# KerkDovan/univer-ocr

Measured on AMD Instinct MI355X. Metric: document-images/sec (fwd+bwd) on 256x512 synthetic pages, higher is better.
Workload: dtype f32; 1 GPU; BASELINE configs[2]: my_model train step (fwd+loss+bwd+L2+SGD) of Monochrome+Paragraph+Line on (32,256,512,1) pages and Char on (32,32,64,1) line strips per GPU; batch_per_gpu=32, global_batch=32, optimizer=sgd, parallelism=dp1, h2d_inclusive=False, input_grads=True, hip_graphs=True, pipelined_lanes=True, hw_queues=4

## Files before the change

### include/univer_hip.h

```cpp
#ifndef UNIVER_HIP_H
#define UNIVER_HIP_H

#include <stddef.h>
#include <stdint.h>

#ifdef __cplusplus
extern "C" {
#endif

#define UOCR_ABI_VERSION 4

typedef struct uocr_ctx uocr_ctx;

enum { UOCR_F32 = 0, UOCR_F64 = 1, UOCR_F16 = 2 };
#define UOCR_F16_SCALED(k) (UOCR_F16 | ((k) << 8))
#define UOCR_DTYPE_BASE(dtype) ((dtype) & 0xff)
#define UOCR_DTYPE_GRAD_SCALE_LOG2(dtype) (((dtype) >> 8) & 0xff)
enum { UOCR_ACT_NONE = 0, UOCR_ACT_RELU = 1, UOCR_ACT_LEAKY = 2, UOCR_ACT_SIGMOID = 3 };
enum { UOCR_LOSS_DICE = 0, UOCR_LOSS_JACCARD = 1 };
enum {
    UOCR_OK = 0,
    UOCR_ERR_ARG = -1,
    UOCR_ERR_DTYPE = -2,
    UOCR_ERR_HIP = -3,
    UOCR_ERR_WORKSPACE = -4,
    UOCR_ERR_UNSUPPORTED = -5,
    UOCR_ERR_RCCL = -6
};

int uocr_abi_version(void);
int uocr_ctx_create(int device, size_t workspace_bytes, uocr_ctx** out);
int uocr_ctx_create_cu_mask(int device, size_t workspace_bytes, const uint32_t* cu_mask, int mask_words, uocr_ctx** out);
int uocr_ctx_destroy(uocr_ctx* ctx);
int uocr_ctx_set_stream(uocr_ctx* ctx, void* hip_stream);
void* uocr_ctx_get_stream(uocr_ctx* ctx);
int uocr_ctx_set_option(uocr_ctx* ctx, const char* key, int value);
int uocr_ctx_last_split(uocr_ctx* ctx, int* blocks, long long* items);
int uocr_ctx_last_gemm(uocr_ctx* ctx, int* bm, int* gm, int* gn, int* nsplit);
int uocr_ctx_last_gemm_group(uocr_ctx* ctx, int* problems, int* split_problems);
int uocr_ctx_last_pair(uocr_ctx* ctx, int* kernel, int* g, int* mode, int* pf, int* nw, int* blocks_x, int* bands,
                       int* band_h);
enum {
    UOCR_CONV_NONE = 0,
    UOCR_CONV_GENERIC = 1,
    UOCR_CONV_MFMA = 2,
    UOCR_CONV_H16 = 3,
    UOCR_CONV_H16_WGRAD = 4,
    UOCR_CONV_H16_WGRAD_S2 = 5,
    UOCR_CONV_T32 = 6,
    UOCR_CONV_T32_WGRAD = 7,
    UOCR_CONV_H3 = 8,
    UOCR_CONV_TILED = 9,
    UOCR_CONV_C16_EXPAND = 10,
    UOCR_CONV_C16_REDUCE = 11,
    UOCR_CONV_C16_WGRAD = 12,
    UOCR_CONV_DGRAD_S2 = 13,
    UOCR_CONV_DGRAD_C64S2 = 14,
    UOCR_CONV_WGRAD_T542 = 15,
    UOCR_CONV_WGRAD_S2_TILED = 16,
    UOCR_CONV_TABLE_FAST = 17,
    UOCR_CONV_TABLE_PX = 18
};
int uocr_ctx_last_conv(uocr_ctx* ctx, int* entry, int* kernel);
int uocr_ctx_reserve_workspace(uocr_ctx* ctx, size_t bytes);
const char* uocr_last_error(uocr_ctx* ctx);
int uocr_malloc(uocr_ctx* ctx, size_t bytes, void** out);
int uocr_free(uocr_ctx* ctx, void* ptr);
int uocr_memset_zero(uocr_ctx* ctx, void* ptr, size_t bytes);
int uocr_h2d(uocr_ctx* ctx, void* dst, const void* src_host, size_t bytes);
int uocr_d2h_sync(uocr_ctx* ctx, void* dst_host, const void* src, size_t bytes);
int uocr_d2d(uocr_ctx* ctx, void* dst, const void* src, size_t bytes);
int uocr_stream_sync(uocr_ctx* ctx);
int uocr_event_create(void** out_event);
int uocr_event_destroy(void* event);
int uocr_event_record(uocr_ctx* ctx, void* event);
int uocr_stream_wait_event(uocr_ctx* ctx, void* event);
int uocr_event_elapsed_ms_sync(void* start, void* stop, float* out_ms);
int uocr_event_synchronize(void* event);
int uocr_graph_begin_capture(uocr_ctx* ctx);
int uocr_graph_end_capture(uocr_ctx* ctx, void** out_graph_exec);
int uocr_graph_launch(uocr_ctx* ctx, void* graph_exec);
int uocr_graph_destroy(void* graph_exec);
int uocr_ctx_set_loss_snapshot(uocr_ctx* ctx, const double* slots, int count, double* ring, int ring_len,
                               unsigned* counter);
int uocr_wgrad_defer_begin(uocr_ctx* ctx);
int uocr_wgrad_defer_flush(uocr_ctx* ctx, int keep_open);
int uocr_device_info(uocr_ctx* ctx, char* name_out, size_t name_cap, int* cu_count, size_t* hbm_bytes);

int uocr_conv2d_fwd(uocr_ctx* ctx, int dtype, const void* x, const void* w, const void* b, void* y,
                    int n, int h, int wd, int cin, int cout, int kh, int kw, int sh, int sw,
                    int ph, int pw, int oh, int ow, double pad_value, int use_bias,
                    int act, double act_alpha);
int uocr_conv2d_bwd_data(uocr_ctx* ctx, int dtype, const void* dy, const void* w, void* dx,
                         int n, int h, int wd, int cin, int cout, int kh, int kw, int sh, int sw,
                         int ph, int pw, int oh, int ow,
                         const void* x_act, int act, double act_alpha);
int uocr_conv2d_bwd_weight(uocr_ctx* ctx, int dtype, const void* x, const void* dy, void* dw, void* db,
                           int n, int h, int wd, int cin, int cout, int kh, int kw, int sh, int sw,
                           int ph, int pw, int oh, int ow, double pad_value, int use_bias,
                           int accumulate);

int uocr_conv_pair_fwd(uocr_ctx* ctx, int dtype, const void* x, const void* w1, const void* b1,
                       const void* w2, const void* b2, void* y, int n, int h, int wd, int cmid,
                       double pad_value1, int use_bias1, int use_bias2, double alpha1, int act2);
int uocr_conv_pair_bwd(uocr_ctx* ctx, int dtype, const void* x, const void* y, const void* dy,
                       const void* w1, const void* b1, const void* w2, void* dw1, void* db1, void* dw2,
                       void* db2, void* dx, int n, int h, int wd, int cmid, double pad_value1,
                       int use_bias1, int use_bias2, double alpha1, int act2, int accumulate);

int uocr_upconv2x_fwd(uocr_ctx* ctx, int dtype, const void* x_low, const void* w, const void* b, void* y,
                      int n, int hl, int wl, int cin, int cout, int kh, int kw, int ph, int pw,
                      int use_bias, int act, double act_alpha, void* weff);
int uocr_upconv2x_bwd_data(uocr_ctx* ctx, int dtype, const void* dy, const void* w, void* dx_low,
                           int n, int hl, int wl, int cin, int cout, int kh, int kw, int ph, int pw,
                           const void* x_act, int act, double act_alpha, const void* weff);
int uocr_upconv2x_bwd_weight(uocr_ctx* ctx, int dtype, const void* x_low, const void* dy, void* dw, void* db,
                             int n, int hl, int wl, int cin, int cout, int kh, int kw, int ph, int pw,
                             int use_bias, int accumulate);

int uocr_maxpool2d_fwd(uocr_ctx* ctx, int dtype, const void* x, void* y, uint8_t* mask,
                       int n, int h, int wd, int c, int kh, int kw, int sh, int sw, int ph, int pw,
                       int oh, int ow);
int uocr_maxpool2d_bwd(uocr_ctx* ctx, int dtype, const void* dy, const uint8_t* mask, void* dx,
                       int n, int h, int wd, int c, int kh, int kw, int sh, int sw, int ph, int pw,
                       int oh, int ow);

int uocr_upsample2d_fwd(uocr_ctx* ctx, int dtype, const void* x, void* y,
                        int n, int h, int wd, int c, int sy, int sx);
int uocr_upsample2d_bwd(uocr_ctx* ctx, int dtype, const void* dy, void* dx,
                        int n, int h, int wd, int c, int sy, int sx);

int uocr_act_fwd(uocr_ctx* ctx, int dtype, int kind, double alpha, const void* x, void* y, size_t count);
int uocr_act_bwd(uocr_ctx* ctx, int dtype, int kind, double alpha, const void* x, const void* dy,
                 void* dx, size_t count);

int uocr_act_bwd_from_output(uocr_ctx* ctx, int dtype, int kind, double alpha, const void* y, const void* dy,
                             void* dx, size_t count);

int uocr_dense_fwd(uocr_ctx* ctx, int dtype, const void* x, const void* w, void* y,
                   int m, int n_in, int n_out);
int uocr_dense_bwd(uocr_ctx* ctx, int dtype, const void* x, const void* w, const void* dy,
                   void* dx, void* dw, int m, int n_in, int n_out, int accumulate);
int uocr_dense_fwd_act(uocr_ctx* ctx, int dtype, const void* x, const void* w, void* y,
                       int m, int n_in, int n_out, int act, double act_alpha);
int uocr_dense_bwd_act(uocr_ctx* ctx, int dtype, const void* x, const void* w, const void* dy,
                       void* dx, void* dw, int m, int n_in, int n_out, int accumulate,
// ... 118 lines not shown
```

### univer-ocr_amd/csrc/conv_api.hip

```cpp
#include "conv_dims.h"

namespace {

int check_dims(uocr_ctx* ctx, const ConvDims& d) {
    UOCR_REQUIRE(ctx, d.n > 0 && d.h > 0 && d.w > 0 && d.cin > 0 && d.cout > 0);
    UOCR_REQUIRE(ctx, d.kh > 0 && d.kw > 0 && d.sh > 0 && d.sw > 0 && d.ph >= 0 && d.pw >= 0);
    UOCR_REQUIRE(ctx, d.oh > 0 && d.ow > 0);
    UOCR_REQUIRE(ctx, (d.oh - 1) * d.sh + d.kh <= d.h + 2 * d.ph);
    UOCR_REQUIRE(ctx, (d.ow - 1) * d.sw + d.kw <= d.w + 2 * d.pw);
    return UOCR_OK;
}

constexpr ConvRow<ConvFwd> FWD_ROWS[] = {
    {UOCR_CONV_H16, uocr_conv_h16_takes, uocr_conv_h16_run},
    {UOCR_CONV_T32, uocr_conv_t32_takes, uocr_conv_t32_run},
    {UOCR_CONV_H3, uocr_conv_h3_takes, uocr_conv_h3_run},
    {UOCR_CONV_TILED, uocr_conv_tiled_takes, uocr_conv_tiled_run},
    {CONV_NOT_NOTED, uocr_conv_fast_takes, uocr_conv_fast_run},
    {UOCR_CONV_MFMA, uocr_conv_mfma_takes, uocr_conv_mfma_run},
    {UOCR_CONV_GENERIC, uocr_conv_any_takes, uocr_conv_generic_run},
};
constexpr ConvRow<ConvDgrad> DGRAD_ROWS[] = {
    {UOCR_CONV_H16, uocr_conv_h16_takes, uocr_conv_h16_run},
    {UOCR_CONV_T32, uocr_conv_t32_takes, uocr_conv_t32_run},
    {CONV_NOT_NOTED, uocr_conv_fast_takes, uocr_conv_fast_run},
    {UOCR_CONV_MFMA, uocr_conv_mfma_takes, uocr_conv_mfma_run},
    {UOCR_CONV_GENERIC, uocr_conv_any_takes, uocr_conv_generic_run},
};
constexpr ConvRow<ConvWgrad> WGRAD_ROWS[] = {
    {UOCR_CONV_H16_WGRAD, uocr_conv_h16_takes, uocr_conv_h16_run},
    {UOCR_CONV_T32_WGRAD, uocr_conv_t32_takes, uocr_conv_t32_run},
    {UOCR_CONV_H16_WGRAD_S2, uocr_conv_h16_s2_takes, uocr_conv_h16_s2_run},
    {CONV_NOT_NOTED, uocr_conv_fast_takes, uocr_conv_fast_run},
    {UOCR_CONV_MFMA, uocr_conv_mfma_takes, uocr_conv_mfma_run},
    {UOCR_CONV_GENERIC, uocr_conv_any_takes, uocr_conv_generic_run},
};

}

extern "C" {

int uocr_conv2d_fwd(uocr_ctx* ctx, int dtype, const void* x, const void* w, const void* b, void* y, int n, int h,
                    int wd, int cin, int cout, int kh, int kw, int sh, int sw, int ph, int pw, int oh, int ow,
                    double pad_value, int use_bias, int act, double act_alpha) {
    UOCR_CHECK_CTX(ctx);
    const ConvDims d{n, h, wd, cin, cout, kh, kw, sh, sw, ph, pw, oh, ow};
    int rc = check_dims(ctx, d);
    if (rc) return rc;
    UOCR_REQUIRE(ctx, x && w && y && (b || !use_bias));
    UOCR_REQUIRE(ctx, act >= UOCR_ACT_NONE && act <= UOCR_ACT_SIGMOID);
    return uocr_conv_dispatch(ctx, 0, FWD_ROWS, ConvFwd{dtype, d, x, w, b, y, pad_value, use_bias, act, act_alpha});
}

int uocr_conv2d_bwd_data(uocr_ctx* ctx, int dtype, const void* dy, const void* w, void* dx, int n, int h, int wd,
                         int cin, int cout, int kh, int kw, int sh, int sw, int ph, int pw, int oh, int ow,
                         const void* x_act, int act, double act_alpha) {
    UOCR_CHECK_CTX(ctx);
    const ConvDims d{n, h, wd, cin, cout, kh, kw, sh, sw, ph, pw, oh, ow};
    int rc = check_dims(ctx, d);
    if (rc) return rc;
    UOCR_REQUIRE(ctx, dy && w && dx);
    UOCR_REQUIRE(ctx, act == UOCR_ACT_NONE || (x_act && (act == UOCR_ACT_SIGMOID || (act == UOCR_ACT_LEAKY && act_alpha > 0))));
    const ActMask mask{act == UOCR_ACT_NONE ? nullptr : x_act, act, act_alpha};
    return uocr_conv_dispatch(ctx, 1, DGRAD_ROWS, ConvDgrad{dtype, d, dy, w, dx, mask});
}

int uocr_conv2d_bwd_weight(uocr_ctx* ctx, int dtype, const void* x, const void* dy, void* dw, void* db, int n, int h,
                           int wd, int cin, int cout, int kh, int kw, int sh, int sw, int ph, int pw, int oh, int ow,
                           double pad_value, int use_bias, int accumulate) {
    UOCR_CHECK_CTX(ctx);
    const ConvDims d{n, h, wd, cin, cout, kh, kw, sh, sw, ph, pw, oh, ow};
    int rc = check_dims(ctx, d);
    if (rc) return rc;
    UOCR_REQUIRE(ctx, x && dy && dw && db);
    return uocr_conv_dispatch(ctx, 2, WGRAD_ROWS, ConvWgrad{dtype, d, x, dy, dw, db, pad_value, use_bias, accumulate});
}

}
```

### univer-ocr_amd/csrc/conv_dims.h

```cpp
#pragma once
#include "uocr_common.h"

struct ConvDims { int n, h, w, cin, cout, kh, kw, sh, sw, ph, pw, oh, ow; };

inline bool conv_is5x5_pad2(const ConvDims& d, int stride) {
    return d.kh == 5 && d.kw == 5 && d.sh == stride && d.sw == stride && d.ph == 2 && d.pw == 2 &&
           d.oh == (d.h + stride - 1) / stride && d.ow == (d.w + stride - 1) / stride;
}

struct ActMask { const void* y; int act; double alpha; };

struct ConvFwd { int dtype; ConvDims d; const void *x, *w, *b; void* y; double pad_value; int use_bias, act; double act_alpha; };
struct ConvDgrad { int dtype; ConvDims d; const void *dy, *w; void* dx; ActMask mask; };
struct ConvWgrad { int dtype; ConvDims d; const void *x, *dy; void *dw, *db; double pad_value; int use_bias, accumulate; };

template <class Call>
struct ConvRow { int kernel; bool (*takes)(uocr_ctx*, const Call&); int (*run)(uocr_ctx*, const Call&); };
constexpr int CONV_NOT_NOTED = UOCR_CONV_NONE;
template <class Call> bool uocr_conv_any_takes(uocr_ctx*, const Call&) { return true; }

template <class Call, size_t N>
int uocr_conv_dispatch(uocr_ctx* ctx, int entry, const ConvRow<Call> (&rows)[N], const Call& c) {
    for (const ConvRow<Call>& r : rows)
        if (r.takes(ctx, c))
            return r.kernel == CONV_NOT_NOTED ? r.run(ctx, c) : uocr_noted_conv(ctx, entry, r.kernel, r.run(ctx, c));
    UOCR_FAIL(ctx, UOCR_ERR_UNSUPPORTED, "no conv kernel takes this call");
}

bool uocr_conv_mfma_takes(uocr_ctx*, const ConvFwd&);       int uocr_conv_mfma_run(uocr_ctx*, const ConvFwd&);
bool uocr_conv_mfma_takes(uocr_ctx*, const ConvDgrad&);     int uocr_conv_mfma_run(uocr_ctx*, const ConvDgrad&);
bool uocr_conv_mfma_takes(uocr_ctx*, const ConvWgrad&);     int uocr_conv_mfma_run(uocr_ctx*, const ConvWgrad&);
bool uocr_conv_h16_takes(uocr_ctx*, const ConvFwd&);        int uocr_conv_h16_run(uocr_ctx*, const ConvFwd&);
bool uocr_conv_h16_takes(uocr_ctx*, const ConvDgrad&);      int uocr_conv_h16_run(uocr_ctx*, const ConvDgrad&);
bool uocr_conv_h16_takes(uocr_ctx*, const ConvWgrad&);      int uocr_conv_h16_run(uocr_ctx*, const ConvWgrad&);
bool uocr_conv_h16_s2_takes(uocr_ctx*, const ConvWgrad&);   int uocr_conv_h16_s2_run(uocr_ctx*, const ConvWgrad&);
bool uocr_upconv_h16_takes(uocr_ctx*, const ConvFwd&);      int uocr_upconv_h16_run(uocr_ctx*, const ConvFwd&);
bool uocr_upconv_h16_takes(uocr_ctx*, const ConvDgrad&);    int uocr_upconv_h16_run(uocr_ctx*, const ConvDgrad&);
bool uocr_upconv_wgrad_h16_takes(uocr_ctx*, const ConvWgrad&);
int uocr_upconv_wgrad_h16(uocr_ctx* ctx, const ConvWgrad& c, float* partial, size_t partial_floats, int* nblocks);
bool uocr_conv_t32_takes(uocr_ctx*, const ConvFwd&);        int uocr_conv_t32_run(uocr_ctx*, const ConvFwd&);
bool uocr_conv_t32_takes(uocr_ctx*, const ConvDgrad&);      int uocr_conv_t32_run(uocr_ctx*, const ConvDgrad&);
bool uocr_conv_t32_takes(uocr_ctx*, const ConvWgrad&);      int uocr_conv_t32_run(uocr_ctx*, const ConvWgrad&);
bool uocr_upconv_t32_takes(uocr_ctx*, const ConvDgrad&);    int uocr_upconv_t32_run(uocr_ctx*, const ConvDgrad&);
bool uocr_conv_h3_takes(uocr_ctx*, const ConvFwd&);         int uocr_conv_h3_run(uocr_ctx*, const ConvFwd&);
bool uocr_conv_tiled_takes(uocr_ctx*, const ConvFwd&);      int uocr_conv_tiled_run(uocr_ctx*, const ConvFwd&);
bool uocr_conv_fast_takes(uocr_ctx*, const ConvFwd&);       int uocr_conv_fast_run(uocr_ctx*, const ConvFwd&);
bool uocr_conv_fast_takes(uocr_ctx*, const ConvDgrad&);     int uocr_conv_fast_run(uocr_ctx*, const ConvDgrad&);
bool uocr_conv_fast_takes(uocr_ctx*, const ConvWgrad&);     int uocr_conv_fast_run(uocr_ctx*, const ConvWgrad&);
int uocr_conv_generic_run(uocr_ctx*, const ConvFwd&);       int uocr_conv_generic_run(uocr_ctx*, const ConvDgrad&);
int uocr_conv_generic_run(uocr_ctx*, const ConvWgrad&);
```

### univer-ocr_amd/csrc/conv_fast.hip

```cpp
#include "finish_group.h"
#include "conv_dims.h"

namespace {

template <int C, typename TA>
__device__ __forceinline__ void load_vec(const TA* __restrict__ p, float (&v)[C]) {
    if constexpr (C == 1) {
        v[0] = ld1(p);
    } else if constexpr (C == 2) {
        const float2 t = ld2(p);
        v[0] = t.x;
        v[1] = t.y;
    } else {
        static_assert(C % 4 == 0, "channel count must be 1, 2 or a multiple of 4");
#pragma unroll
        for (int q = 0; q < C / 4; ++q) {
            const float4 t = ld4(p + 4 * q);
            v[4 * q] = t.x;
            v[4 * q + 1] = t.y;
            v[4 * q + 2] = t.z;
            v[4 * q + 3] = t.w;
        }
    }
}

template <int C, typename TA>
__device__ __forceinline__ void store_vec(TA* __restrict__ p, const float (&v)[C]) {
    if constexpr (C == 1) {
        st1(p, v[0]);
    } else if constexpr (C == 2) {
        st2(p, make_float2(v[0], v[1]));
    } else {
#pragma unroll
        for (int q = 0; q < C / 4; ++q) st4(p + 4 * q, make_float4(v[4 * q], v[4 * q + 1], v[4 * q + 2], v[4 * q + 3]));
    }
}

struct FastDims {
    int n, h, w, oh, ow, ph, pw;
};

inline bool is_c16_same(const ConvDims& d, int cin, int cout) {
    return d.kh == 3 && d.kw == 3 && d.cin == cin && d.cout == cout && d.sh == 1 && d.sw == 1 && d.oh == d.h &&
           d.ow == d.w;
}
inline bool is_5x5_s2_pad2(const ConvDims& d) {
    return d.kh == 5 && d.kw == 5 && d.sh == 2 && d.sw == 2 && d.ph == 2 && d.pw == 2;
}
inline bool is_5x5_s1_pad2(const ConvDims& d) {
    return d.kh == 5 && d.kw == 5 && d.sh == 1 && d.sw == 1 && d.ph == 2 && d.pw == 2;
}

template <int C, typename TA>
__device__ __forceinline__ void apply_mask(float (&v)[C], const TA* __restrict__ mask_y, size_t off, int act,
                                           float alpha) {
    if (act == UOCR_ACT_NONE) return;
    float m[C];
    load_vec<C>(mask_y + off, m);
#pragma unroll
    for (int c = 0; c < C; ++c) v[c] *= act_grad_from_output<float>(m[c], act, alpha);
}

template <int KH, int KW, int CIN, int COUT, int SH, int SW, int COB, int PY, typename TA>
__global__ __launch_bounds__(256) void conv_fwd_fast(const TA* __restrict__ x, const float* __restrict__ w,
                                                     const float* __restrict__ bias, TA* __restrict__ y,
                                                     FastDims d, float pad, int use_bias, int act, float alpha) {
    constexpr int NQ = COUT / COB;
    constexpr int PXW = 64 / NQ;
    constexpr int ROWS = (PY - 1) * SH + KH;
    const int ox = blockIdx.x * PXW + threadIdx.x / NQ;
    const int oy0 = (blockIdx.y * 4 + threadIdx.y) * PY;
    const int oc0 = (threadIdx.x % NQ) * COB;
    const int b = blockIdx.z;
    const float* __restrict__ wl = w;
    const bool valid = ox < d.ow && oy0 < d.oh;
    if (!valid) return;
    float acc[PY][COB];
#pragma unroll
    for (int p = 0; p < PY; ++p)
#pragma unroll
        for (int o = 0; o < COB; ++o) acc[p][o] = 0.f;
    const int iy0 = oy0 * SH - d.ph, ix0 = ox * SW - d.pw;
    const TA* xb = x + (size_t)b * d.h * d.w * CIN;
#pragma unroll
// ... 35 lines not shown
        }
        store_vec<COB>(y + (((size_t)b * d.oh + oy0 + p) * d.ow + ox) * COUT + oc0, out);
    }
}

template <int KH, int KW, int CIN, int COUT, int SH, int SW, int PY, typename TA>
__global__ __launch_bounds__(256) void conv_dgrad_fast(const TA* __restrict__ dy, const float* __restrict__ w,
                                                       TA* __restrict__ dx, FastDims d,
                                                       const TA* __restrict__ mask_y, int mask_act, float mask_alpha) {
    static_assert(PY == 1 || (SH == 1 && SW == 1), "row tiling of dgrad needs stride 1");
    const int ix = blockIdx.x * 64 + threadIdx.x;
    const int iy0 = (blockIdx.y * 4 + threadIdx.y) * PY;
    const int b = blockIdx.z;
    const float* __restrict__ wl = w;
    const bool valid = ix < d.w && iy0 < d.h;
    if (!valid) return;
    float acc[PY][CIN];
#pragma unroll
    for (int p = 0; p < PY; ++p)
#pragma unroll
        for (int c = 0; c < CIN; ++c) acc[p][c] = 0.f;
    const TA* gb = dy + (size_t)b * d.oh * d.ow * COUT;
    if constexpr (SH == 1 && SW == 1) {
        constexpr int ROWS = PY + KH - 1;
        const int gy0 = iy0 + d.ph - (KH - 1);
#pragma unroll
        for (int r = 0; r < ROWS; ++r) {
            const int gy = gy0 + r;
            const bool row_ok = gy >= 0 && gy < d.oh;
            const int gyc = min(max(gy, 0), d.oh - 1);
#pragma unroll
            for (int kx = KW - 1; kx >= 0; --kx) {
                const int gx = ix + d.pw - kx;
                float g[COUT];
                load_vec<COUT>(gb + ((size_t)gyc * d.ow + min(max(gx, 0), d.ow - 1)) * COUT, g);
                if (!(row_ok && gx >= 0 && gx < d.ow)) {
#pragma unroll
                    for (int o = 0; o < COUT; ++o) g[o] = 0.f;
                }
#pragma unroll
                for (int p = 0; p < PY; ++p) {
                    const int ky = p + (KH - 1) - r;
                    if (ky >= 0 && ky < KH) {
#pragma unroll
                        for (int c = 0; c < CIN; ++c)
#pragma unroll
                            for (int o = 0; o < COUT; ++o)
                                acc[p][c] += g[o] * wl[((ky * KW + kx) * CIN + c) * COUT + o];
                    }
                }
            }
        }
    } else {
#pragma unroll
        for (int ky = KH - 1; ky >= 0; --ky) {
            const int ty = iy0 + d.ph - ky;
            const int gy = ty / SH;
            const bool row_ok = ty >= 0 && gy < d.oh && gy * SH == ty;
#pragma unroll
            for (int kx = KW - 1; kx >= 0; --kx) {
                const int tx = ix + d.pw - kx;
                const int gx = tx / SW;
                if (row_ok && tx >= 0 && gx < d.ow && gx * SW == tx) {
                    float g[COUT];
                    load_vec<COUT>(gb + ((size_t)gy * d.ow + gx) * COUT, g);
#pragma unroll
                    for (int c = 0; c < CIN; ++c)
#pragma unroll
                        for (int o = 0; o < COUT; ++o) acc[0][c] += g[o] * wl[((ky * KW + kx) * CIN + c) * COUT + o];
                }
            }
        }
    }
#pragma unroll
    for (int p = 0; p < PY; ++p) {
        if (!valid || iy0 + p >= d.h) break;
        const size_t off = (((size_t)b * d.h + iy0 + p) * d.w + ix) * CIN;
        apply_mask<CIN>(acc[p], mask_y, off, mask_act, mask_alpha);
        store_vec<CIN>(dx + off, acc[p]);
    }
}

template <int CIN, int COUT, typename TA, class K>
__global__ __launch_bounds__(256) void conv_dgrad_s2(const TA* __restrict__ dy, const float* __restrict__ w,
                                                     TA* __restrict__ dx, FastDims d,
                                                     const TA* __restrict__ mask_y, int mask_act,
                                                     float mask_alpha) {
    mask_act = act_kind<K::mask>(mask_act);
    const int i = blockIdx.x * 64 + threadIdx.x, j = blockIdx.y * 4 + threadIdx.y, b = blockIdx.z;
    if (2 * i >= d.w || 2 * j >= d.h) return;
    const TA* gb = dy + (size_t)b * d.oh * d.ow * COUT;
    float g[3][3][COUT];
#pragma unroll
    for (int r = 0; r < 3; ++r) {
        const int gy = j - 1 + r;
        const bool row_ok = gy >= 0 && gy < d.oh;
        const int gyc = min(max(gy, 0), d.oh - 1);
#pragma unroll
        for (int c = 0; c < 3; ++c) {
            const int gx = i - 1 + c;
            load_vec<COUT>(gb + ((size_t)gyc * d.ow + min(max(gx, 0), d.ow - 1)) * COUT, g[r][c]);
            if (!(row_ok && gx >= 0 && gx < d.ow)) {
#pragma unroll
                for (int o = 0; o < COUT; ++o) g[r][c][o] = 0.f;
            }
        }
    }
    float out[2][2][CIN];
#pragma unroll
    for (int q = 0; q < 4; ++q)
#pragma unroll
        for (int ci = 0; ci < CIN; ++ci) out[q >> 1][q & 1][ci] = 0.f;
#pragma unroll
    for (int ky = 0; ky < 5; ++ky)
#pragma unroll
        for (int kx = 0; kx < 5; ++kx) {
            const int py = ky & 1, px = kx & 1;
            const int r = (py ? (3 - ky) / 2 : 1 - ky / 2) + 1, c = (px ? (3 - kx) / 2 : 1 - kx / 2) + 1;
#pragma unroll
            for (int ci = 0; ci < CIN; ++ci)
#pragma unroll
                for (int o = 0; o < COUT; ++o)
                    out[py][px][ci] += g[r][c][o] * w[((ky * 5 + kx) * CIN + ci) * COUT + o];
        }
#pragma unroll
    for (int py = 0; py < 2; ++py) {
        const int y = 2 * j + py;
        if (y >= d.h) break;
        const size_t off = (((size_t)b * d.h + y) * d.w + 2 * i) * CIN;
        if (CIN == 1 && (d.w & 1) == 0) {
            float v[2] = {out[py][0][0], out[py][1][0]};
            apply_mask<2>(v, mask_y, off, mask_act, mask_alpha);
            store_vec<2>(dx + off, v);
        } else {
#pragma unroll
            for (int px = 0; px < 2; ++px) {
                if (2 * i + px >= d.w) break;
                apply_mask<CIN>(out[py][px], mask_y, off + px * CIN, mask_act, mask_alpha);
                store_vec<CIN>(dx + off + px * CIN, out[py][px]);
            }
        }
    }
}

__global__ __launch_bounds__(256) void conv_dgrad_c64s2(const float* __restrict__ dy, const float* __restrict__ w,
                                                        float* __restrict__ dx, int n, int h, int wd, int oh, int ow,
                                                        const float* __restrict__ mask_y, int mask_act,
                                                        float mask_alpha) {
    constexpr int KH = 5, KW = 3, CO = 64;
    const int q = threadIdx.x & 15;
    const int b = blockIdx.z, y = blockIdx.y;
    const bool live = (int)(blockIdx.x * 16 + (threadIdx.x >> 4)) < wd;
    const int x = live ? blockIdx.x * 16 + (threadIdx.x >> 4) : wd - 1;
    const size_t pix = ((size_t)b * h + y) * wd + x;
    const float* gb = dy + (size_t)b * oh * ow * CO + 4 * q;
    float acc = 0.f;
#pragma unroll
    for (int t = 0; t < 3; ++t) {
        const int ky = (y & 1) + 2 * t, gy = (y - ky) / 2;
        if (ky >= KH || y - ky < 0 || gy >= oh) continue;
#pragma unroll
        for (int kx = 0; kx < KW; ++kx) {
            const int gx = x + 1 - kx;
            if (gx < 0 || gx >= ow) continue;
            const float4 g = *reinterpret_cast<const float4*>(gb + ((size_t)gy * ow + gx) * CO);
            const float4 wv = *reinterpret_cast<const float4*>(w + (ky * KW + kx) * CO + 4 * q);
            acc += g.x * wv.x + g.y * wv.y + g.z * wv.z + g.w * wv.w;
        }
    }
    acc += __shfl_xor(acc, 8, 64);
    acc += __shfl_xor(acc, 4, 64);
    acc += __shfl_xor(acc, 2, 64);
    acc += __shfl_xor(acc, 1, 64);
    if (!live || q != 0) return;
    if (mask_act != UOCR_ACT_NONE) acc *= act_grad_from_output<float>(mask_y[pix], mask_act, mask_alpha);
    dx[pix] = acc;
}

template <int N, int OFFS, typename TA>
__device__ __forceinline__ void load_row_c1(const TA* __restrict__ row, int a4, int width, bool row_ok,
                                            float fill, float (&seg)[N][1]) {
    constexpr int NV4 = (OFFS + N + 3) / 4;
    float buf[NV4 * 4];
#pragma unroll
    for (int k = 0; k < NV4; ++k) {
        const int col = a4 + 4 * k;
        float4 v = ld4(row + min(max(col, 0), width - 4));
        if (!(row_ok && col >= 0 && col < width)) v = make_float4(fill, fill, fill, fill);
        buf[4 * k] = v.x;
        buf[4 * k + 1] = v.y;
        buf[4 * k + 2] = v.z;
        buf[4 * k + 3] = v.w;
    }
#pragma unroll
    for (int j = 0; j < N; ++j) seg[j][0] = buf[OFFS + j];
}

template <int KH, int KW, int CIN, int COUT, int SH, int SW, int PX, typename TA, class K>
__global__ __launch_bounds__(256) void conv_fwd_px(const TA* __restrict__ x, const float* __restrict__ w,
                                                   const float* __restrict__ bias, TA* __restrict__ y,
                                                   FastDims d, float pad, int use_bias, int act, float alpha) {
    act = act_kind<K::act>(act);
    constexpr int NXV = (PX - 1) * SW + KW;
    const int ox0 = (blockIdx.x * 64 + threadIdx.x) * PX;
    const int oy = blockIdx.y * 4 + threadIdx.y;
    const int b = blockIdx.z;
    if (ox0 >= d.ow || oy >= d.oh) return;
    float acc[PX][COUT];
#pragma unroll
    for (int p = 0; p < PX; ++p)
#pragma unroll
        for (int o = 0; o < COUT; ++o) acc[p][o] = 0.f;
    const int ix0 = ox0 * SW - d.pw;
    const TA* xb = x + (size_t)b * d.h * d.w * CIN;
#pragma unroll 1
    for (int ky = 0; ky < KH; ++ky) {
        const int iy = oy * SH - d.ph + ky;
        const bool row_ok = iy >= 0 && iy < d.h;
        const TA* xr = xb + (size_t)min(max(iy, 0), d.h - 1) * d.w * CIN;
        const float* wr = w + ky * (KW * CIN * COUT);
        float xv[NXV][CIN];
        bool vec_done = false;
        if constexpr (CIN == 1 && PX % 4 == 0) {
            constexpr int PWC = KW / 2, OFFS = (4 - PWC % 4) % 4;
            if (d.pw == PWC && d.w % 4 == 0) {
                load_row_c1<NXV, OFFS>(xr, ix0 - OFFS, d.w, row_ok, pad, xv);
                vec_done = true;
            }
        }
        if (!vec_done) {
#pragma unroll
            for (int j = 0; j < NXV; ++j) {
                const int ix = ix0 + j;
                load_vec<CIN>(xr + (size_t)min(max(ix, 0), d.w - 1) * CIN, xv[j]);
                if (!(row_ok && ix >= 0 && ix < d.w)) {
#pragma unroll
                    for (int c = 0; c < CIN; ++c) xv[j][c] = pad;
                }
            }
        }
#pragma unroll
        for (int kx = 0; kx < KW; ++kx)
#pragma unroll
            for (int c = 0; c < CIN; ++c)
#pragma unroll
                for (int o = 0; o < COUT; ++o) {
                    const float wv = wr[(kx * CIN + c) * COUT + o];
#pragma unroll
                    for (int p = 0; p < PX; ++p) acc[p][o] += xv[p * SW + kx][c] * wv;
                }
    }
    if constexpr (COUT == 1 && PX % 4 == 0) {
        if (d.ow % PX == 0) {
            float out[PX];
#pragma unroll
            for (int p = 0; p < PX; ++p) out[p] = act_apply(acc[p][0] + (use_bias ? bias[0] : 0.f), act, alpha);
            store_vec<PX>(y + ((size_t)b * d.oh + oy) * d.ow + ox0, out);
            return;
        }
    }
#pragma unroll
    for (int p = 0; p < PX; ++p) {
        if (ox0 + p >= d.ow) break;
        float out[COUT];
#pragma unroll
        for (int o = 0; o < COUT; ++o) {
            float v = acc[p][o];
            if (use_bias) v += bias[o];
            out[o] = act_apply(v, act, alpha);
        }
        store_vec<COUT>(y + (((size_t)b * d.oh + oy) * d.ow + ox0 + p) * COUT, out);
    }
}

template <int KH, int KW, int CIN, int COUT, int PX, typename TA>
__global__ __launch_bounds__(256) void conv_dgrad_px(const TA* __restrict__ dy, const float* __restrict__ w,
                                                     TA* __restrict__ dx, FastDims d,
                                                     const TA* __restrict__ mask_y, int mask_act, float mask_alpha) {
    constexpr int NG = PX + KW - 1;
    const int ix0 = (blockIdx.x * 64 + threadIdx.x) * PX;
    const int iy = blockIdx.y * 4 + threadIdx.y;
    const int b = blockIdx.z;
    if (ix0 >= d.w || iy >= d.h) return;
    float acc[PX][CIN];
#pragma unroll
    for (int p = 0; p < PX; ++p)
#pragma unroll
        for (int c = 0; c < CIN; ++c) acc[p][c] = 0.f;
    const TA* gb = dy + (size_t)b * d.oh * d.ow * COUT;
    const int gx0 = ix0 + d.pw - (KW - 1);
#pragma unroll 1
    for (int ky = KH - 1; ky >= 0; --ky) {
        const int gy = iy + d.ph - ky;
        const bool row_ok = gy >= 0 && gy < d.oh;
        const TA* gr = gb + (size_t)min(max(gy, 0), d.oh - 1) * d.ow * COUT;
        const float* wr = w + ky * (KW * CIN * COUT);
        float g[NG][COUT];
        bool vec_done = false;
        if constexpr (COUT == 1 && PX % 4 == 0) {
            constexpr int PWC = KW / 2, OFFS = (((KW - 1 - PWC) % 4) + 4) % 4;
            if (d.pw == PWC && d.ow % 4 == 0) {
                load_row_c1<NG, OFFS>(gr, gx0 - OFFS, d.ow, row_ok, 0.f, g);
                vec_done = true;
            }
        }
        if (!vec_done) {
#pragma unroll
            for (int j = 0; j < NG; ++j) {
                const int gx = gx0 + j;
                load_vec<COUT>(gr + (size_t)min(max(gx, 0), d.ow - 1) * COUT, g[j]);
                if (!(row_ok && gx >= 0 && gx < d.ow)) {
#pragma unroll
                    for (int o = 0; o < COUT; ++o) g[j][o] = 0.f;
                }
            }
        }
#pragma unroll
        for (int kx = 0; kx < KW; ++kx)
#pragma unroll
            for (int c = 0; c < CIN; ++c)
#pragma unroll
                for (int o = 0; o < COUT; ++o) {
                    const float wv = wr[(kx * CIN + c) * COUT + o];
#pragma unroll
                    for (int p = 0; p < PX; ++p) acc[p][c] += g[p + (KW - 1) - kx][o] * wv;
                }
    }
    if constexpr (CIN == 1 && PX % 4 == 0) {
        if (d.w % PX == 0) {
            float out[PX];
#pragma unroll
            for (int p = 0; p < PX; ++p) out[p] = acc[p][0];
            const size_t off = ((size_t)b * d.h + iy) * d.w + ix0;
            apply_mask<PX>(out, mask_y, off, mask_act, mask_alpha);
            store_vec<PX>(dx + off, out);
            return;
        }
    }
#pragma unroll
    for (int p = 0; p < PX; ++p) {
        if (ix0 + p >= d.w) break;
        const size_t off = (((size_t)b * d.h + iy) * d.w + ix0 + p) * CIN;
        apply_mask<CIN>(acc[p], mask_y, off, mask_act, mask_alpha);
        store_vec<CIN>(dx + off, acc[p]);
    }
}

template <int KH, int KW, int PY, bool FLIP>
__global__ __launch_bounds__(256) void conv_c16_reduce(const float* __restrict__ src, const float* __restrict__ w,
                                                       const float* __restrict__ bias, float* __restrict__ dst,
                                                       int n, int h, int wd, int ph, int pw, float pad, int use_bias,
                                                       int act, float alpha, const float* __restrict__ mask_y,
                                                       int mask_act, float mask_alpha) {
    constexpr int C = 16, ROWS = PY + KH - 1;
    const int q = threadIdx.x & 3;
    const int ox = blockIdx.x * 16 + (threadIdx.x >> 2);
    const int oy0 = (blockIdx.y * 4 + threadIdx.y) * PY;
    const int b = blockIdx.z;
    float wreg[KH][KW][4];
#pragma unroll
    for (int ky = 0; ky < KH; ++ky)
#pragma unroll
        for (int kx = 0; kx < KW; ++kx) {
            const int sky = FLIP ? KH - 1 - ky : ky, skx = FLIP ? KW - 1 - kx : kx;
            const float4 t = *reinterpret_cast<const float4*>(w + (sky * KW + skx) * C + q * 4);
            wreg[ky][kx][0] = t.x;
            wreg[ky][kx][1] = t.y;
            wreg[ky][kx][2] = t.z;
            wreg[ky][kx][3] = t.w;
        }
    const int PH = FLIP ? KH - 1 - ph : ph, PW = FLIP ? KW - 1 - pw : pw;
    float acc[PY];
#pragma unroll
    for (int p = 0; p < PY; ++p) acc[p] = 0.f;
    const float* sb = src + (size_t)b * h * wd * C + q * 4;
    const int oxc = min(ox, wd - 1);
#pragma unroll
    for (int r = 0; r < ROWS; ++r) {
        const int iy = oy0 - PH + r;
        const bool row_ok = iy >= 0 && iy < h;
        const float* sr = sb + (size_t)min(max(iy, 0), h - 1) * wd * C;
#pragma unroll
        for (int kx = 0; kx < KW; ++kx) {
            const int ix = oxc - PW + kx;
            float4 v = *reinterpret_cast<const float4*>(sr + (size_t)min(max(ix, 0), wd - 1) * C);
            if (!(row_ok && ix >= 0 && ix < wd)) v = make_float4(pad, pad, pad, pad);
#pragma unroll
            for (int p = 0; p < PY; ++p) {
                const int ky = r - p;
                if (ky >= 0 && ky < KH)
                    acc[p] += v.x * wreg[ky][kx][0] + v.y * wreg[ky][kx][1] + v.z * wreg[ky][kx][2] +
                              v.w * wreg[ky][kx][3];
            }
        }
    }
#pragma unroll
    for (int p = 0; p < PY; ++p) {
        float v = acc[p];
        v += __shfl_xor(v, 1, 64);
        v += __shfl_xor(v, 2, 64);
        if (q == 0 && ox < wd && oy0 + p < h) {
            if (use_bias) v += bias[0];
            const size_t off = ((size_t)b * h + oy0 + p) * wd + ox;
            v = act_apply(v, act, alpha);
            if (mask_act != UOCR_ACT_NONE) v *= act_grad_from_output<float>(mask_y[off], mask_act, mask_alpha);
            dst[off] = v;
        }
    }
}

template <int KH, int KW, int PY, bool FLIP>
__global__ __launch_bounds__(256) void conv_c16_expand(const float* __restrict__ src, const float* __restrict__ w,
                                                       const float* __restrict__ bias, float* __restrict__ dst,
                                                       int n, int h, int wd, int ph, int pw, float pad, int use_bias,
                                                       int act, float alpha, const float* __restrict__ mask_y,
                                                       int mask_act, float mask_alpha) {
    constexpr int C = 16, ROWS = PY + KH - 1;
    const int q = threadIdx.x & 3;
    const int ox = blockIdx.x * 16 + (threadIdx.x >> 2);
    const int oy0 = (blockIdx.y * 4 + threadIdx.y) * PY;
    const int b = blockIdx.z;
    float wreg[KH][KW][4];
#pragma unroll
    for (int ky = 0; ky < KH; ++ky)
#pragma unroll
        for (int kx = 0; kx < KW; ++kx) {
            const int sky = FLIP ? KH - 1 - ky : ky, skx = FLIP ? KW - 1 - kx : kx;
            const float4 t = *reinterpret_cast<const float4*>(w + (sky * KW + skx) * C + q * 4);
            wreg[ky][kx][0] = t.x;
// ... 92 lines not shown
        for (int kx = 0; kx < KW; ++kx)
#pragma unroll
            for (int j = 0; j < 4; ++j) {
                float t = acc[ky][kx][j];
#pragma unroll
                for (int m = 4; m < 64; m <<= 1) t += __shfl_xor(t, m, 64);
                acc[ky][kx][j] = t;
            }
#pragma unroll
    for (int m = 4; m < 64; m <<= 1) accb += __shfl_xor(accb, m, 64);
    if (pl == 0) {
#pragma unroll
        for (int ky = 0; ky < KH; ++ky)
#pragma unroll
            for (int kx = 0; kx < KW; ++kx)
#pragma unroll
                for (int j = 0; j < 4; ++j) red[wv][q][(ky * KW + kx) * 4 + j] = acc[ky][kx][j];
        red[wv][q][NA - 1] = accb;
    }
    __syncthreads();
    const int tid = wv * 64 + threadIdx.x;
    float* out = partial + (size_t)blockIdx.x * 4 * NA;
    for (int a = tid; a < 4 * NA; a += 256) {
        const int qq = a / NA, i = a % NA;
        out[a] = red[0][qq][i] + red[1][qq][i] + red[2][qq][i] + red[3][qq][i];
    }
}

template <int KH, int KW>
__global__ __launch_bounds__(256) void conv_c16_wgrad_finish(const float* __restrict__ partial, float* __restrict__ dw,
                                                             float* __restrict__ db, int nblocks, int use_bias,
                                                             int accumulate) {
    constexpr int NA = KH * KW * 4 + 1;
    __shared__ double smem[16];
    const int i = blockIdx.x, q = blockIdx.y;
    double s = 0.0;
    for (int blk = threadIdx.x; blk < nblocks; blk += blockDim.x) s += (double)partial[((size_t)blk * 4 + q) * NA + i];
    s = block_reduce_sum(s, smem);
    if (threadIdx.x != 0) return;
    float* dst;
    if (i < NA - 1) {
        dst = dw + (i / 4) * 16 + q * 4 + (i % 4);
    } else {
        if (q != 0) return;
        dst = db;
        if (!use_bias) s = 0.0;
    }
    *dst = accumulate ? (float)((double)*dst + s) : (float)s;
}

template <int NP, int S>
__device__ __forceinline__ void reduce_scatter_step(float (&acc)[NP], int lane) {
    constexpr int bit = 32 >> S;
    constexpr int half = NP >> (S + 1);
    const bool up = lane & bit;
#pragma unroll
    for (int i = 0; i < half; ++i) {
        const float send = up ? acc[i] : acc[i + half];
        const float keep = up ? acc[i + half] : acc[i];
        acc[i] = keep + __shfl_xor(send, bit, 64);
    }
}

template <int NP>
__device__ __forceinline__ void lane_reduce_scatter(float (&acc)[NP], int lane) {
    reduce_scatter_step<NP, 0>(acc, lane);
    reduce_scatter_step<NP, 1>(acc, lane);
    reduce_scatter_step<NP, 2>(acc, lane);
    reduce_scatter_step<NP, 3>(acc, lane);
    reduce_scatter_step<NP, 4>(acc, lane);
    reduce_scatter_step<NP, 5>(acc, lane);
}

template <int KH, int KW, int CIN, int COUT, int SH, int SW, int KYR, int COB>
struct WgradCfg {
    static constexpr int NW = KYR * KW * CIN * COB;
    static constexpr int NACC = NW + COB;
    static constexpr int NP = ((NACC + 63) / 64) * 64;
    static constexpr int KYG = KH / KYR;
    static constexpr int OCG = COUT / COB;
};

template <int KH, int KW, int CIN, int COUT, int SH, int SW, int KYR, int COB, int PX, bool CLAMP, typename TA>
__global__ __launch_bounds__(256) void conv_wgrad_fast(const TA* __restrict__ x, const TA* __restrict__ dy,
                                                       float* __restrict__ partial, FastDims d, float pad,
                                                       int rows_per_block, int nbands) {
    using C = WgradCfg<KH, KW, CIN, COUT, SH, SW, KYR, COB>;
    constexpr int NXV = (PX - 1) * SW + KW;
    __shared__ float red[4][C::NP];
    const int lane = threadIdx.x, wv = threadIdx.y;
    const int band = blockIdx.x % nbands, b = blockIdx.x / nbands;
    const int kyg = blockIdx.y / C::OCG, ocg = blockIdx.y % C::OCG;
    const int ky0 = kyg * KYR, oc0 = ocg * COB;
    const int row0 = band * rows_per_block;
    const int row1 = min(d.oh, row0 + rows_per_block);
    float acc[C::NP];
#pragma unroll
    for (int a = 0; a < C::NP; ++a) acc[a] = 0.f;
    const TA* xb = x + (size_t)b * d.h * d.w * CIN;
    const TA* gb = dy + (size_t)b * d.oh * d.ow * COUT + oc0;
    for (int oy = row0 + wv; oy < row1; oy += 4) {
        for (int ox0 = lane * PX; ox0 < d.ow; ox0 += 64 * PX) {
            float g[PX][COB];
#pragma unroll
            for (int p = 0; p < PX; ++p) {
                if (ox0 + p < d.ow) {
                    load_vec<COB>(gb + ((size_t)oy * d.ow + ox0 + p) * COUT, g[p]);
                } else {
#pragma unroll
                    for (int o = 0; o < COB; ++o) g[p][o] = 0.f;
                }
                if (kyg == 0) {
#pragma unroll
                    for (int o = 0; o < COB; ++o) acc[C::NW + o] += g[p][o];
                }
            }
            const int iy0 = oy * SH - d.ph + ky0, ix0 = ox0 * SW - d.pw;
#pragma unroll
            for (int kyl = 0; kyl < KYR; ++kyl) {
                const int iy = iy0 + kyl;
                const bool row_ok = iy >= 0 && iy < d.h;
                const int iyc = min(max(iy, 0), d.h - 1);
                float xv[NXV][CIN];
                bool vec_done = false;
                if constexpr (CIN == 1 && PX % 4 == 0) {
                    constexpr int PWC = KW / 2, OFFS = (4 - PWC % 4) % 4;
                    if (d.pw == PWC && d.w % 4 == 0) {
                        load_row_c1<NXV, OFFS>(xb + (size_t)iyc * d.w, ix0 - OFFS, d.w, row_ok, pad, xv);
                        vec_done = true;
                    }
                }
                if (!vec_done) {
#pragma unroll
                    for (int j = 0; j < NXV; ++j) {
                        const int ix = ix0 + j;
                        if constexpr (CLAMP) {
                            load_vec<CIN>(xb + ((size_t)iyc * d.w + min(max(ix, 0), d.w - 1)) * CIN, xv[j]);
                            if (!(row_ok && ix >= 0 && ix < d.w)) {
#pragma unroll
                                for (int c = 0; c < CIN; ++c) xv[j][c] = pad;
                            }
                        } else {
                            if (row_ok && ix >= 0 && ix < d.w) {
                                load_vec<CIN>(xb + ((size_t)iy * d.w + ix) * CIN, xv[j]);
                            } else {
#pragma unroll
                                for (int c = 0; c < CIN; ++c) xv[j][c] = pad;
                            }
                        }
                    }
                }
#pragma unroll
                for (int kx = 0; kx < KW; ++kx)
#pragma unroll
                    for (int c = 0; c < CIN; ++c)
#pragma unroll
                        for (int o = 0; o < COB; ++o)
#pragma unroll
                            for (int p = 0; p < PX; ++p)
                                acc[((kyl * KW + kx) * CIN + c) * COB + o] += xv[p * SW + kx][c] * g[p][o];
            }
        }
    }
    lane_reduce_scatter<C::NP>(acc, lane);
    int base = 0;
#pragma unroll
    for (int s = 0; s < 6; ++s)
        if (lane & (32 >> s)) base += C::NP >> (s + 1);
#pragma unroll
    for (int r = 0; r < C::NP / 64; ++r) red[wv][base + r] = acc[r];
    __syncthreads();
    const int tid = wv * 64 + lane;
    float* out = partial + ((size_t)blockIdx.y * gridDim.x + blockIdx.x) * C::NP;
    for (int a = tid; a < C::NP; a += 256) out[a] = red[0][a] + red[1][a] + red[2][a] + red[3][a];
}

template <int KH, int KW, int CIN, int COUT, int KYR, int COB, int NW, int NP>
__global__ __launch_bounds__(256) void conv_wgrad_fast_finish(const float* __restrict__ partial, float* __restrict__ dw,
                                                              float* __restrict__ db, int nblocks, int use_bias,
                                                              int accumulate, float unscale) {
    __shared__ double smem[16];
    const int a = blockIdx.x, grp = blockIdx.y;
    constexpr int OCG = COUT / COB;
    const int kyg = grp / OCG, ocg = grp % OCG;
    const float* src = partial + (size_t)grp * nblocks * NP + a;
    double s = 0.0;
    for (int i = threadIdx.x; i < nblocks; i += blockDim.x) s += (double)src[(size_t)i * NP];
    s = block_reduce_sum(s, smem);
    if (threadIdx.x != 0) return;
    float* dst;
    if (a < NW) {
        const int o = a % COB, t = a / COB;
        const int c = t % CIN, tap = t / CIN;
        const int kx = tap % KW, kyl = tap / KW;
        dst = dw + (((size_t)(kyg * KYR + kyl) * KW + kx) * CIN + c) * COUT + ocg * COB + o;
    } else {
        if (kyg != 0) return;
        dst = db + ocg * COB + (a - NW);
        if (!use_bias) s = 0.0;
    }
    s *= (double)unscale;
    *dst = accumulate ? (float)((double)*dst + s) : (float)s;
}

namespace t542 {
constexpr int TH = 16, TW = 64, WH = TH + 4, WW = TW + 4, NW = 40, NB = 2, NACC = NW + NB, NP = 64;
__device__ __forceinline__ int swz(int row, int c) { return row * WW + (c & 3) * (WW / 4) + (c >> 2); }
struct Taprows {
    static constexpr int TH = t542::TH, TW = t542::TW, NW = t542::NW, NB = t542::NB, ROW = NACC;
};
}

template <typename TA>
__global__ __launch_bounds__(320) void conv_wgrad_t542(const TA* __restrict__ x, const TA* __restrict__ dy,
                                                       float* __restrict__ partial, int h, int wd, float pad,
                                                       int tiles_per_block) {
    using namespace t542;
    __shared__ float4 xs[WH * WW];
    __shared__ float2 gs[TH * TW];
    const int tid = threadIdx.x, lane = tid & 63, ky = tid >> 6;
    const int x0 = blockIdx.x * TW, b = blockIdx.z;
    const int tile0 = blockIdx.y * tiles_per_block, tiles_y = (h + TH - 1) / TH;
    const TA* xb = x + (size_t)b * h * wd * 4;
    const TA* gb = dy + (size_t)b * h * wd * 2;
    float acc[NP];
#pragma unroll
    for (int a = 0; a < NP; ++a) acc[a] = 0.f;
    const int cg = lane & 15, rsub = lane >> 4;
    const int t_end = min(tiles_y, tile0 + tiles_per_block);
    for (int t = tile0; t < t_end; ++t) {
        const int y0 = t * TH;
        __syncthreads();
        for (int e = tid; e < WH * WW; e += 320) {
            const int r = e / WW, c = e - r * WW;
            const int gy = y0 - 2 + r, gx = x0 - 2 + c;
            float4 v = ld4(xb + ((size_t)min(max(gy, 0), h - 1) * wd + min(max(gx, 0), wd - 1)) * 4);
            if (gy < 0 || gy >= h || gx < 0 || gx >= wd) v = make_float4(pad, pad, pad, pad);
            xs[swz(r, c)] = v;
        }
        for (int e = tid; e < TH * TW; e += 320) {
            const int r = e / TW, c = e - r * TW;
            const int gy = y0 + r, gx = x0 + c;
            float2 v = ld2(gb + ((size_t)min(gy, h - 1) * wd + min(gx, wd - 1)) * 2);
            if (gy >= h || gx >= wd) v = make_float2(0.f, 0.f);
            gs[e] = v;
        }
        __syncthreads();
#pragma unroll 1
        for (int it = 0; it < TH / 4; ++it) {
            const int r = it * 4 + rsub;
            float g[4][2];
            {
                const float4* gp = reinterpret_cast<const float4*>(gs + r * TW + 4 * cg);
                const float4 g01 = gp[0], g23 = gp[1];
                g[0][0] = g01.x, g[0][1] = g01.y, g[1][0] = g01.z, g[1][1] = g01.w;
                g[2][0] = g23.x, g[2][1] = g23.y, g[3][0] = g23.z, g[3][1] = g23.w;
            }
            float xv[8][4];
// ... 82 lines not shown
            float v[COUT];
            load_vec<COUT>(gb + ((size_t)min(gy, oh - 1) * ow + min(gx, ow - 1)) * COUT, v);
            const bool in = gy < oh && gx < ow;
#pragma unroll
            for (int co = 0; co < COUT; ++co) gs[e * COUT + co] = in ? v[co] : 0.f;
        }
        __syncthreads();
#pragma unroll 1
        for (int it = 0; it < C::TH * C::TW / 64; ++it) {
            const int e = it * 64 + lane, r = e / C::TW, c = e - r * C::TW;
            float g[COUT];
#pragma unroll
            for (int co = 0; co < COUT; ++co) g[co] = gs[e * COUT + co];
            const float* xr = xs + ((2 * r + ky) * C::WW + 2 * c) * CIN;
#pragma unroll
            for (int kx = 0; kx < 5; ++kx)
#pragma unroll
                for (int ci = 0; ci < CIN; ++ci) {
                    const float xv = xr[kx * CIN + ci];
#pragma unroll
                    for (int co = 0; co < COUT; ++co) acc[(kx * CIN + ci) * COUT + co] += xv * g[co];
                }
            if (ky == 0) {
#pragma unroll
                for (int co = 0; co < COUT; ++co) acc[C::NW + co] += g[co];
            }
        }
    }
    lane_reduce_scatter<C::NP>(acc, lane);
    int base = 0;
#pragma unroll
    for (int sft = 0; sft < 6; ++sft)
        if (lane & (32 >> sft)) base += C::NP >> (sft + 1);
    const size_t blk = ((size_t)blockIdx.z * gridDim.y + blockIdx.y) * gridDim.x + blockIdx.x;
    float* out = partial + (blk * 5 + ky) * C::NP;
#pragma unroll
    for (int q = 0; q < C::NP / 64; ++q) out[base + q] = acc[q];
}

template <int ROW, int NW>
__global__ __launch_bounds__(256) void conv_wgrad_taprows_finish(const float* __restrict__ partial, float* __restrict__ dw,
                                                                 float* __restrict__ db, int nblocks, int use_bias,
                                                                 int accumulate, float unscale) {
    __shared__ double smem[16];
    const int a = blockIdx.x, ndw = 5 * NW;
    const int ky = a < ndw ? a / NW : 0, idx = a < ndw ? a % NW : NW + (a - ndw);
    double s = 0.0;
    for (int i = threadIdx.x; i < nblocks; i += blockDim.x) s += (double)partial[((size_t)i * 5 + ky) * ROW + idx];
    s = block_reduce_sum(s, smem);
    if (threadIdx.x != 0) return;
    float* dst = a < ndw ? dw + a : db + (a - ndw);
    if (a >= ndw && !use_bias) s = 0.0;
    s *= (double)unscale;
    *dst = accumulate ? (float)((double)*dst + s) : (float)s;
}

template <class C, class Producer>
int launch_wgrad_taprows(uocr_ctx* ctx, const ConvWgrad& c, int kernel_id, int rows, int cols, Producer&& producer) {
    const int n = c.d.n;
    const int tiles_x = (cols + C::TW - 1) / C::TW, tiles_y = (rows + C::TH - 1) / C::TH;
    const int per_block = uocr_tiles_per_block(tiles_x, tiles_y, n, uocr_budget(ctx, 1024));
    const dim3 grid(tiles_x, (tiles_y + per_block - 1) / per_block, n);
    const int nblocks = (int)(grid.x * grid.y * grid.z);
    uocr_note_split(ctx, nblocks, (long long)tiles_x * tiles_y * n);
    int rc = UOCR_OK;
    float* partial = uocr_partial_buffer(ctx, (size_t)nblocks * 5 * C::ROW * sizeof(float), &rc);
    if (rc) return rc;
    UOCR_DISPATCH_TA(ctx, c.dtype, { producer(TA{}, grid, partial, per_block); });
    UOCR_LAUNCH_CHECK(ctx);
    const float unscale = (float)uocr_grad_unscale(c.dtype);
    const FinishDesc fd = finish_taprows(partial, nblocks, C::ROW, C::NW, C::NB, (float*)c.dw, (float*)c.db, c.use_bias,
                                         c.accumulate, unscale);
    return uocr_noted_conv(ctx, 2, kernel_id, uocr_finish(ctx, fd, [&] {
        hipLaunchKernelGGL((conv_wgrad_taprows_finish<C::ROW, C::NW>), dim3(5 * C::NW + C::NB), dim3(256), 0, ctx->stream,
                           (const float*)partial, (float*)c.dw, (float*)c.db, nblocks, c.use_bias, c.accumulate, unscale);
    }));
}

struct FastRow {
    int kh, kw, cin, cout, sh, sw;
    struct Fwd { int px = 0, cob = 0, py = 0; } fwd;
    struct Dx { int px = 0, py = 0; } dx;
    struct Dw { int kyr = 0, cob = 0, px = 0; } dw;
};

constexpr FastRow FAST_CONVS[] = {
    {.kh = 3, .kw = 3, .cin = 1, .cout = 16, .sh = 1, .sw = 1,
     .fwd = {.cob = 4, .py = 2}, .dx = {.px = 4}, .dw = {.kyr = 3, .cob = 16, .px = 1}},
    {.kh = 3, .kw = 3, .cin = 16, .cout = 1, .sh = 1, .sw = 1,
     .fwd = {.px = 4}, .dx = {.px = 2}, .dw = {.kyr = 1, .cob = 1, .px = 1}},
    {.kh = 5, .kw = 5, .cin = 1, .cout = 1, .sh = 2, .sw = 2,
     .fwd = {.px = 4}, .dx = {.py = 1}, .dw = {.kyr = 5, .cob = 1, .px = 4}},
    {.kh = 5, .kw = 5, .cin = 1, .cout = 1, .sh = 1, .sw = 1,
     .fwd = {.px = 4}, .dx = {.px = 8}, .dw = {.kyr = 5, .cob = 1, .px = 8}},
    {.kh = 5, .kw = 5, .cin = 1, .cout = 4, .sh = 2, .sw = 2,
     .fwd = {.px = 4}, .dx = {.py = 1}, .dw = {.kyr = 5, .cob = 4, .px = 1}},
    {.kh = 5, .kw = 5, .cin = 4, .cout = 4, .sh = 2, .sw = 2,
     .fwd = {.px = 4}, .dx = {.py = 1}, .dw = {.kyr = 1, .cob = 4, .px = 2}},
    {.kh = 5, .kw = 5, .cin = 4, .cout = 4, .sh = 1, .sw = 1,
     .fwd = {.px = 4}, .dx = {.px = 4}, .dw = {.kyr = 1, .cob = 4, .px = 4}},
    {.kh = 5, .kw = 5, .cin = 4, .cout = 2, .sh = 1, .sw = 1,
     .fwd = {.px = 4}, .dx = {.px = 4}, .dw = {.kyr = 1, .cob = 2, .px = 4}},
    {.kh = 5, .kw = 3, .cin = 1, .cout = 64, .sh = 2, .sw = 1,
     .fwd = {.cob = 4, .py = 1}, .dx = {.py = 1}, .dw = {.kyr = 5, .cob = 8, .px = 1}},
};

template <int I>
struct FastConv {
    static constexpr FastRow R = FAST_CONVS[I];
    static constexpr int KH = R.kh, KW = R.kw, CIN = R.cin, COUT = R.cout, SH = R.sh, SW = R.sw;
    static_assert(R.fwd.px > 0 ? !R.fwd.cob && !R.fwd.py : R.fwd.cob > 0 && R.fwd.py > 0, "forward: px, or cob and py");
    static_assert(R.dx.px > 0 ? !R.dx.py && SH == 1 && SW == 1 : R.dx.py > 0, "dx: px (stride 1 only), or py");
    static_assert(R.dw.kyr > 0 && R.dw.cob > 0 && R.dw.px > 0, "dw: kyr, cob and px");
    static constexpr int FWD_KERNEL = R.fwd.px > 0 ? UOCR_CONV_TABLE_PX : UOCR_CONV_TABLE_FAST;
    static constexpr int DX_KERNEL = R.dx.px > 0 ? UOCR_CONV_TABLE_PX : UOCR_CONV_TABLE_FAST;

    static bool match(const ConvDims& d) {
        return d.kh == KH && d.kw == KW && d.cin == CIN && d.cout == COUT && d.sh == SH && d.sw == SW;
    }
    static FastDims dims(const ConvDims& d) { return FastDims{d.n, d.h, d.w, d.oh, d.ow, d.ph, d.pw}; }

    static int run(uocr_ctx* ctx, const ConvFwd& c) {
        const ConvDims& d = c.d;
        return uocr_act_tags<0>(ctx, c.act, UOCR_ACT_NONE, [&](auto kinds) -> int {
        using K = ActKindsIf<COUT == 4, decltype(kinds)>;
        UOCR_DISPATCH_TA(ctx, c.dtype, {
            if constexpr (R.fwd.px > 0) {
                const int groups = (d.ow + R.fwd.px - 1) / R.fwd.px;
                const dim3 grid((groups + 63) / 64, (d.oh + 3) / 4, d.n), block(64, 4);
                hipLaunchKernelGGL((conv_fwd_px<KH, KW, CIN, COUT, SH, SW, R.fwd.px, TA, K>), grid, block, 0, ctx->stream,
                                   (const TA*)c.x, (const float*)c.w, (const float*)c.b, (TA*)c.y, dims(d),
                                   (float)c.pad_value, c.use_bias, c.act, (float)c.act_alpha);
            } else {
                constexpr int PXW = 64 / (COUT / R.fwd.cob);
                const dim3 grid((d.ow + PXW - 1) / PXW, (d.oh + 4 * R.fwd.py - 1) / (4 * R.fwd.py), d.n), block(64, 4);
                hipLaunchKernelGGL((conv_fwd_fast<KH, KW, CIN, COUT, SH, SW, R.fwd.cob, R.fwd.py, TA>), grid, block, 0, ctx->stream,
                                   (const TA*)c.x, (const float*)c.w, (const float*)c.b, (TA*)c.y, dims(d),
                                   (float)c.pad_value, c.use_bias, c.act, (float)c.act_alpha);
            }
        });
        UOCR_LAUNCH_CHECK(ctx);
        return UOCR_OK;
        });
    }

    static int run(uocr_ctx* ctx, const ConvDgrad& c) {
        const ConvDims& d = c.d;
        UOCR_DISPATCH_TA(ctx, c.dtype, {
            if constexpr (R.dx.px > 0) {
                const int groups = (d.w + R.dx.px - 1) / R.dx.px;
                const dim3 grid((groups + 63) / 64, (d.h + 3) / 4, d.n), block(64, 4);
                hipLaunchKernelGGL((conv_dgrad_px<KH, KW, CIN, COUT, R.dx.px, TA>), grid, block, 0, ctx->stream,
                                   (const TA*)c.dy, (const float*)c.w, (TA*)c.dx, dims(d), (const TA*)c.mask.y,
                                   c.mask.act, (float)c.mask.alpha);
            } else {
                const dim3 grid((d.w + 63) / 64, (d.h + 4 * R.dx.py - 1) / (4 * R.dx.py), d.n), block(64, 4);
                hipLaunchKernelGGL((conv_dgrad_fast<KH, KW, CIN, COUT, SH, SW, R.dx.py, TA>), grid, block, 0, ctx->stream,
                                   (const TA*)c.dy, (const float*)c.w, (TA*)c.dx, dims(d), (const TA*)c.mask.y,
                                   c.mask.act, (float)c.mask.alpha);
            }
        });
        UOCR_LAUNCH_CHECK(ctx);
        return UOCR_OK;
    }

    static int run(uocr_ctx* ctx, const ConvWgrad& c) {
        const ConvDims& d = c.d;
        using C = WgradCfg<KH, KW, CIN, COUT, SH, SW, R.dw.kyr, R.dw.cob>;
        constexpr int RQ = 4;
        const int bands = ctx->opt_wgrad_bands > 0 ? ctx->opt_wgrad_bands : (C::NP >= 128 ? 64 : 512);
        int rows = (d.n * d.oh + bands - 1) / bands;
        rows = ((rows + RQ - 1) / RQ) * RQ;
        if (rows > d.oh) rows = ((d.oh + RQ - 1) / RQ) * RQ;
        const int nbands = (d.oh + rows - 1) / rows;
        const int nblocks = nbands * d.n, ngroups = C::KYG * C::OCG;
        const size_t bytes = (size_t)nblocks * ngroups * C::NP * sizeof(float);
        int rc = UOCR_OK;
        float* partial = uocr_partial_buffer(ctx, bytes, &rc);
        if (rc) return rc;
        UOCR_DISPATCH_TA(ctx, c.dtype, {
            hipLaunchKernelGGL((conv_wgrad_fast<KH, KW, CIN, COUT, SH, SW, R.dw.kyr, R.dw.cob, R.dw.px, (CIN >= 4), TA>),
                               dim3(nblocks, ngroups), dim3(64, 4), 0, ctx->stream, (const TA*)c.x, (const TA*)c.dy,
                               partial, dims(d), (float)c.pad_value, rows, nbands);
        });
        UOCR_LAUNCH_CHECK(ctx);
        const float unscale = (float)uocr_grad_unscale(c.dtype);
        const FinishDesc fd = finish_fast(partial, nblocks, ngroups, {C::NP, C::NW, KW, CIN, COUT, R.dw.kyr, R.dw.cob},
                                          (float*)c.dw, (float*)c.db, c.use_bias, c.accumulate, unscale);
        return uocr_finish(ctx, fd, [&] {
            hipLaunchKernelGGL((conv_wgrad_fast_finish<KH, KW, CIN, COUT, R.dw.kyr, R.dw.cob, C::NW, C::NP>),
                               dim3(C::NACC, ngroups), dim3(256), 0, ctx->stream, (const float*)partial, (float*)c.dw,
                               (float*)c.db, nblocks, c.use_bias, c.accumulate, unscale);
        });
    }
};

template <class F>
bool with_fast_conv(const ConvDims& d, F&& f) {
    return [&]<size_t... I>(std::index_sequence<I...>) {
        return ((FastConv<I>::match(d) && (f(FastConv<I>{}), true)) || ...);
    }(std::make_index_sequence<std::size(FAST_CONVS)>{});
}

struct C16Args { const void *src, *w, *bias; void* dst; float pad; int use_bias, act; float alpha; ActMask mask; };
template <class Kernel>
int launch_c16(uocr_ctx* ctx, Kernel kernel, int py, const C16Args& a, const ConvDims& d, int entry, int kernel_id) {
    const dim3 grid((d.w + 15) / 16, (d.h + 4 * py - 1) / (4 * py), d.n), block(64, 4);
    hipLaunchKernelGGL(kernel, grid, block, 0, ctx->stream, (const float*)a.src, (const float*)a.w, (const float*)a.bias,
                       (float*)a.dst, d.n, d.h, d.w, d.ph, d.pw, a.pad, a.use_bias, a.act, a.alpha,
                       (const float*)a.mask.y, a.mask.act, (float)a.mask.alpha);
    UOCR_LAUNCH_CHECK(ctx);
    uocr_note_conv(ctx, entry, kernel_id);
    return UOCR_OK;
}

bool fast_takes(uocr_ctx* ctx, int dtype, const ConvDims& d, const void* p0, const void* p1, const void* p2) {
    const int base = UOCR_DTYPE_BASE(dtype);
    if ((base != UOCR_F32 && base != UOCR_F16) || !ctx->opt_fast) return false;
    if (!uocr_aligned_act(p0, dtype) || !uocr_aligned_act(p1, dtype) || !uocr_aligned_act(p2, UOCR_F32)) return false;
    return with_fast_conv(d, [](auto) {});
}

}

bool uocr_conv_fast_takes(uocr_ctx* ctx, const ConvFwd& c) { return fast_takes(ctx, c.dtype, c.d, c.x, c.y, c.w); }
bool uocr_conv_fast_takes(uocr_ctx* ctx, const ConvDgrad& c) { return fast_takes(ctx, c.dtype, c.d, c.dy, c.dx, c.w); }
bool uocr_conv_fast_takes(uocr_ctx* ctx, const ConvWgrad& c) { return fast_takes(ctx, c.dtype, c.d, c.x, c.dy, c.dw); }

int uocr_conv_fast_run(uocr_ctx* ctx, const ConvFwd& c) {
    const ConvDims& d = c.d;
    const bool f32 = UOCR_DTYPE_BASE(c.dtype) == UOCR_F32;
    const C16Args c16{c.x, c.w, c.b, c.y, (float)c.pad_value, c.use_bias, c.act, (float)c.act_alpha, ActMask{nullptr, UOCR_ACT_NONE, 0.0}};
    if (f32 && is_c16_same(d, 1, 16))
        return launch_c16(ctx, conv_c16_expand<3, 3, 2, false>, 2, c16, d, 0, UOCR_CONV_C16_EXPAND);
    if (f32 && is_c16_same(d, 16, 1))
        return launch_c16(ctx, conv_c16_reduce<3, 3, 4, false>, 4, c16, d, 0, UOCR_CONV_C16_REDUCE);
    int rc = UOCR_OK;
    if (with_fast_conv(d, [&](auto fc) { rc = uocr_noted_conv(ctx, 0, fc.FWD_KERNEL, fc.run(ctx, c)); })) return rc;
    UOCR_FAIL(ctx, UOCR_ERR_UNSUPPORTED, "no fast conv kernel for this shape");
}

int uocr_conv_fast_run(uocr_ctx* ctx, const ConvDgrad& c) {
    const ConvDims& d = c.d;
    const bool f32 = UOCR_DTYPE_BASE(c.dtype) == UOCR_F32;
    const C16Args c16{c.dy, c.w, nullptr, c.dx, 0.f, 0, UOCR_ACT_NONE, 0.f, c.mask};
    if (f32 && is_c16_same(d, 16, 1))
        return launch_c16(ctx, conv_c16_expand<3, 3, 2, true>, 2, c16, d, 1, UOCR_CONV_C16_EXPAND);
    if (f32 && is_c16_same(d, 1, 16))
        return launch_c16(ctx, conv_c16_reduce<3, 3, 4, true>, 4, c16, d, 1, UOCR_CONV_C16_REDUCE);
    if (f32 && d.kh == 5 && d.kw == 3 && d.sh == 2 && d.sw == 1 && d.ph == 0 && d.pw == 1 && d.cin == 1 && d.cout == 64 &&
        d.h <= 65535 && d.n <= 65535) {
        hipLaunchKernelGGL(conv_dgrad_c64s2, dim3((unsigned)((d.w + 15) / 16), d.h, d.n), dim3(256), 0, ctx->stream,
                           (const float*)c.dy, (const float*)c.w, (float*)c.dx, d.n, d.h, d.w, d.oh, d.ow,
                           (const float*)c.mask.y, c.mask.act, (float)c.mask.alpha);
        UOCR_LAUNCH_CHECK(ctx);
        uocr_note_conv(ctx, 1, UOCR_CONV_DGRAD_C64S2);
        return UOCR_OK;
    }
    if (is_5x5_s2_pad2(d) && ((d.cin == 1 && (d.cout == 1 || d.cout == 4)) || (d.cin == 4 && d.cout == 4))) {
        const dim3 grid(((d.w + 1) / 2 + 63) / 64, ((d.h + 1) / 2 + 3) / 4, d.n), block(64, 4);
        const FastDims fd{d.n, d.h, d.w, d.oh, d.ow, d.ph, d.pw};
        const int rc = uocr_act_tags<1>(ctx, UOCR_ACT_NONE, c.mask.act, [&](auto kinds) -> int {
            using K = decltype(kinds);
            using D = ActKinds<UOCR_ACT_DYN, UOCR_ACT_DYN>;
            UOCR_DISPATCH_TA(ctx, c.dtype, {
                auto launch = [&](auto kernel) {
                    hipLaunchKernelGGL(kernel, grid, block, 0, ctx->stream, (const TA*)c.dy, (const float*)c.w, (TA*)c.dx, fd,
                                       (const TA*)c.mask.y, c.mask.act, (float)c.mask.alpha);
                };
                if (d.cin == 4) launch(conv_dgrad_s2<4, 4, TA, K>);
                else if (d.cout == 1) launch(conv_dgrad_s2<1, 1, TA, D>);
                else launch(conv_dgrad_s2<1, 4, TA, D>);
            });
            UOCR_LAUNCH_CHECK(ctx);
            return UOCR_OK;
        });
        if (rc != UOCR_OK) return rc;
        uocr_note_conv(ctx, 1, UOCR_CONV_DGRAD_S2);
        return UOCR_OK;
    }
    int rc = UOCR_OK;
    if (with_fast_conv(d, [&](auto fc) { rc = uocr_noted_conv(ctx, 1, fc.DX_KERNEL, fc.run(ctx, c)); })) return rc;
    UOCR_FAIL(ctx, UOCR_ERR_UNSUPPORTED, "no fast conv kernel for this shape");
}

int uocr_conv_fast_run(uocr_ctx* ctx, const ConvWgrad& c) {
    const ConvDims& d = c.d;
    const bool f32 = UOCR_DTYPE_BASE(c.dtype) == UOCR_F32;
    if (f32 && is_c16_same(d, 16, 1) && c.pad_value == 0.0) {
        constexpr int NA = 3 * 3 * 4 + 1;
        const long budget = uocr_budget(ctx, 2048);
        int rows = (int)((d.n * d.h + budget - 1) / budget);
        rows = ((rows + 3) / 4) * 4;
        if (rows > d.h) rows = ((d.h + 3) / 4) * 4;
        const int nbands = (d.h + rows - 1) / rows, nblocks = nbands * d.n;
        uocr_note_split(ctx, nblocks, (long long)((d.h + 3) / 4) * d.n);
        int rc = uocr_need_workspace(ctx, (size_t)nblocks * 4 * NA * sizeof(float));
        if (rc) return rc;
        float* partial = (float*)ctx->workspace;
        hipLaunchKernelGGL((conv_c16_wgrad<3, 3>), dim3(nblocks), dim3(64, 4), 0, ctx->stream, (const float*)c.x,
                           (const float*)c.dy, partial, d.h, d.w, d.ph, d.pw, rows, nbands);
        UOCR_LAUNCH_CHECK(ctx);
        hipLaunchKernelGGL((conv_c16_wgrad_finish<3, 3>), dim3(NA, 4), dim3(256), 0, ctx->stream,
                           (const float*)partial, (float*)c.dw, (float*)c.db, nblocks, c.use_bias, c.accumulate);
        UOCR_LAUNCH_CHECK(ctx);
        uocr_note_conv(ctx, 2, UOCR_CONV_C16_WGRAD);
        return UOCR_OK;
    }
    if (is_5x5_s2_pad2(d) && ctx->opt_tiled == 1 && d.cin == 1 && d.cout == 4)
        return launch_wgrad_taprows<S2Cfg<1, 4>>(
            ctx, c, UOCR_CONV_WGRAD_S2_TILED, d.oh, d.ow, [&](auto ta, dim3 grid, float* partial, int per_block) {
                using TA = decltype(ta);
                hipLaunchKernelGGL((conv_wgrad_s2_tiled<1, 4, TA>), grid, dim3(320), 0, ctx->stream, (const TA*)c.x,
                                   (const TA*)c.dy, partial, d.h, d.w, d.oh, d.ow, (float)c.pad_value, per_block);
            });
    if (is_5x5_s1_pad2(d) && d.cin == 4 && d.cout == 2)
        return launch_wgrad_taprows<t542::Taprows>(
            ctx, c, UOCR_CONV_WGRAD_T542, d.h, d.w, [&](auto ta, dim3 grid, float* partial, int per_block) {
                using TA = decltype(ta);
                hipLaunchKernelGGL((conv_wgrad_t542<TA>), grid, dim3(320), 0, ctx->stream, (const TA*)c.x, (const TA*)c.dy,
                                   partial, d.h, d.w, (float)c.pad_value, per_block);
            });
    int rc = UOCR_OK;
    if (with_fast_conv(d, [&](auto fc) { rc = uocr_noted_conv(ctx, 2, UOCR_CONV_TABLE_FAST, fc.run(ctx, c)); })) return rc;
    UOCR_FAIL(ctx, UOCR_ERR_UNSUPPORTED, "no fast conv kernel for this shape");
}
```

### univer-ocr_amd/csrc/conv_up.hip

```cpp
#include "up_phase.h"
#include "finish_group.h"
#include "conv_toeplitz.h"

namespace {

constexpr int CH = 4;
constexpr int RH = 16, RW = 32;
constexpr int XH = RH + 2, XW = RW + 2;
constexpr int XPLANE = 624;
constexpr int NWEFF = 9 * CH * 16;

__device__ __forceinline__ float weff_entry(const float* __restrict__ w, int i) {
    const int o = i & 3, phase = (i >> 2) & 3, c = (i >> 4) & 3, m = i >> 6;
    int ylo, yhi, xlo, xhi;
    tap_group(phase >> 1, m / 3, ylo, yhi);
    tap_group(phase & 1, m % 3, xlo, xhi);
    float v[2][2];
#pragma unroll
    for (int a = 0; a < 2; ++a)
#pragma unroll
        for (int b = 0; b < 2; ++b) v[a][b] = w[((min(ylo + a, 4) * 5 + min(xlo + b, 4)) * CH + c) * CH + o];
    float s = 0.f;
#pragma unroll
    for (int a = 0; a < 2; ++a)
#pragma unroll
        for (int b = 0; b < 2; ++b) s += (ylo + a < yhi && xlo + b < xhi) ? v[a][b] : 0.f;
    return s;
}
constexpr int NW = 25 * CH * CH;

__global__ __launch_bounds__(256) void upconv_weff_kernel(const float* __restrict__ w, float* __restrict__ weff) {
    for (int i = threadIdx.x; i < NWEFF; i += blockDim.x) weff[i] = weff_entry(w, i);
}

template <typename TA>
__device__ __forceinline__ void xl_tile_load(float4 (&v)[3], bool (&in)[3], const TA* __restrict__ xb, int ry, int rx,
                                             int hl, int wl, int tid) {
#pragma unroll
    for (int k = 0; k < 3; ++k) {
        const int i = min(tid + 256 * k, XH * XW - 1);
        const int r = i / XW, c = i - r * XW;
        const int gy = ry - 1 + r, gx = rx - 1 + c;
        in[k] = gy >= 0 && gy < hl && gx >= 0 && gx < wl;
        v[k] = ld4(xb + ((size_t)min(max(gy, 0), hl - 1) * wl + min(max(gx, 0), wl - 1)) * CH);
    }
}
__device__ __forceinline__ void xl_tile_put(float* __restrict__ xs, const float4 (&v)[3], const bool (&in)[3], int tid) {
#pragma unroll
    for (int k = 0; k < 3; ++k) {
        const int i = tid + 256 * k;
        if (i >= XH * XW) continue;
        const float4 u = in[k] ? v[k] : make_float4(0.f, 0.f, 0.f, 0.f);
        xs[i] = u.x;
        xs[XPLANE + i] = u.y;
        xs[2 * XPLANE + i] = u.z;
        xs[3 * XPLANE + i] = u.w;
    }
}

template <typename TA, class K>
__global__ __launch_bounds__(256, 8) void upconv_fwd_kernel(const TA* __restrict__ xl, const float* __restrict__ w,
                                                         const float* __restrict__ bias, TA* __restrict__ y,
                                                         int hl, int wl, int rows_per_block, int use_bias, int act,
                                                         float alpha, float* __restrict__ weff_out) {
    act = act_kind<K::act>(act);
    __shared__ float xs[CH * XPLANE];
    __shared__ float ws[512];
    const int tid = threadIdx.x, lane = tid & 63, wv = tid >> 6, n = lane & 15, kq = lane >> 4;
    const int rx = blockIdx.x * RW;
    const int row_begin = blockIdx.y * rows_per_block, row_end = min(hl, row_begin + rows_per_block);
    const TA* xb = xl + (size_t)blockIdx.z * hl * wl * CH;
    const int W = 2 * wl;
    TA* yb = y + (size_t)blockIdx.z * (2 * hl) * W * CH;
    float wr[2];
#pragma unroll
    for (int k = 0; k < 2; ++k) wr[k] = w[min(tid + 256 * k, NW - 1)];
    float4 xv[3];
    bool xin[3];
    xl_tile_load(xv, xin, xb, row_begin, rx, hl, wl, tid);
#pragma unroll
    for (int k = 0; k < 2; ++k) ws[tid + 256 * k] = wr[k];
    xl_tile_put(xs, xv, xin, tid);
    __syncthreads();
    if (weff_out && blockIdx.x == 0 && blockIdx.y == 0 && blockIdx.z == 0)
        for (int i = tid; i < NWEFF; i += 256) weff_out[i] = weff_entry(ws, i);
// ... 222 lines not shown
#pragma unroll
            for (int ch = 0; ch < 4; ++ch)
#pragma unroll
                for (int phase = 0; phase < 4; ++phase) {
                    const float* wv = wt + ch * 16 + phase * 4;
                    acc[p][ch] += wv[0] * g[phase].x + wv[1] * g[phase].y + wv[2] * g[phase].z + wv[3] * g[phase].w;
                }
        }
    }
#pragma unroll
    for (int p = 0; p < 2; ++p) {
        const int qy = ry + r0 + 8 * p, qx = rx + c;
        if (qy >= hl || qx >= wl) continue;
        const size_t off = (((size_t)blockIdx.z * hl + qy) * wl + qx) * CH;
        float4 out = make_float4(acc[p][0], acc[p][1], acc[p][2], acc[p][3]);
        if (mask_act != UOCR_ACT_NONE) {
            out.x *= act_grad_from_output<float>(yv[p].x, mask_act, mask_alpha);
            out.y *= act_grad_from_output<float>(yv[p].y, mask_act, mask_alpha);
            out.z *= act_grad_from_output<float>(yv[p].z, mask_act, mask_alpha);
            out.w *= act_grad_from_output<float>(yv[p].w, mask_act, mask_alpha);
        }
        st4(dxl + off, out);
    }
}

__device__ __forceinline__ void weff1_build(float (&we)[36], const float* __restrict__ w) {
#pragma unroll
    for (int m = 0; m < 9; ++m)
#pragma unroll
        for (int phase = 0; phase < 4; ++phase) {
            int ylo, yhi, xlo, xhi;
            tap_group(phase >> 1, m / 3, ylo, yhi);
            tap_group(phase & 1, m % 3, xlo, xhi);
            float s = 0.f;
            for (int ky = ylo; ky < yhi; ++ky)
                for (int kx = xlo; kx < xhi; ++kx) s += w[ky * 5 + kx];
            we[m * 4 + phase] = s;
        }
}

template <typename TA>
__global__ __launch_bounds__(256) void up1_fwd_kernel(const TA* __restrict__ xl, const float* __restrict__ w,
                                                      const float* __restrict__ bias, TA* __restrict__ y, int hl,
                                                      int wl, int use_bias, int act, float alpha) {
    __shared__ float xs[XH * XW];
    const int tid = threadIdx.x;
    const int rx = blockIdx.x * RW, ry = blockIdx.y * RH;
    const TA* xb = xl + (size_t)blockIdx.z * hl * wl;
    stage_batched<XH * XW, 256, 3, TA>(
        tid,
        [&](int i, bool& inside) {
            const int r = i / XW, c = i - r * XW;
            const int gy = ry - 1 + r, gx = rx - 1 + c;
            inside = gy >= 0 && gy < hl && gx >= 0 && gx < wl;
            return xb + (size_t)min(max(gy, 0), hl - 1) * wl + min(max(gx, 0), wl - 1);
        },
        [&](int i, TA v, bool inside) { xs[i] = inside ? (float)v : 0.f; });
    float we[36];
    weff1_build(we, w);
    const float b0 = use_bias ? bias[0] : 0.f;
    __syncthreads();
    const int c = tid & 31, r0 = tid >> 5;
    const int W = 2 * wl;
    TA* yb = y + (size_t)blockIdx.z * (2 * hl) * W;
#pragma unroll
    for (int p = 0; p < 2; ++p) {
        const int r = r0 + 8 * p, py = ry + r, pxl = rx + c;
        float acc[4] = {b0, b0, b0, b0};
#pragma unroll
        for (int m = 0; m < 9; ++m) {
            const float xv = xs[(r + m / 3) * XW + c + m % 3];
#pragma unroll
            for (int phase = 0; phase < 4; ++phase) acc[phase] += xv * we[m * 4 + phase];
        }
        if (py < hl && pxl < wl) {
            TA* o = yb + (size_t)(2 * py) * W + 2 * pxl;
            st2(o, make_float2(act_apply(acc[0], act, alpha), act_apply(acc[1], act, alpha)));
            st2(o + W, make_float2(act_apply(acc[2], act, alpha), act_apply(acc[3], act, alpha)));
        }
    }
}

template <typename TA>
__global__ __launch_bounds__(256) void up1_dgrad_kernel(const TA* __restrict__ dy, const float* __restrict__ w,
                                                        TA* __restrict__ dxl, int hl, int wl,
                                                        const TA* __restrict__ mask_y, int mask_act,
                                                        float mask_alpha) {
    __shared__ float gs[GH * GW];
    const int tid = threadIdx.x;
    const int rx = blockIdx.x * RW, ry = blockIdx.y * RH;
    const int H = 2 * hl, W = 2 * wl;
    const TA* gb = dy + (size_t)blockIdx.z * H * W;
    stage_batched<GH * GW, 256, 10, TA>(
        tid,
        [&](int i, bool& inside) {
            const int r = i / GW, c = i - r * GW;
            const int gy = 2 * (ry - 1) + r, gx = 2 * (rx - 1) + c;
            inside = gy >= 0 && gy < H && gx >= 0 && gx < W;
            return gb + (size_t)min(max(gy, 0), H - 1) * W + min(max(gx, 0), W - 1);
        },
        [&](int i, TA v, bool inside) { gs[i] = inside ? (float)v : 0.f; });
    float we[36];
    weff1_build(we, w);
    __syncthreads();
    const int c = tid & 31, r0 = tid >> 5;
#pragma unroll
    for (int p = 0; p < 2; ++p) {
        const int r = r0 + 8 * p;
        float acc = 0.f;
#pragma unroll
        for (int m = 0; m < 9; ++m) {
            const int my = m / 3 - 1, mx = m % 3 - 1;
            const float* g0 = gs + (2 * (r - my + 1)) * GW + 2 * (c - mx + 1);
            acc += we[m * 4] * g0[0] + we[m * 4 + 1] * g0[1] + we[m * 4 + 2] * g0[GW] + we[m * 4 + 3] * g0[GW + 1];
        }
        const int qy = ry + r, qx = rx + c;
        if (qy >= hl || qx >= wl) continue;
        const size_t off = ((size_t)blockIdx.z * hl + qy) * wl + qx;
        if (mask_act != UOCR_ACT_NONE) acc *= act_grad_from_output<float>(ld1(mask_y + off), mask_act, mask_alpha);
        st1(dxl + off, acc);
    }
}

template <typename TA>
__global__ __launch_bounds__(256) void up1_wgrad_kernel(const TA* __restrict__ xl, const TA* __restrict__ dy,
                                                        float* __restrict__ partial, int hl, int wl,
                                                        int rows_per_block) {
    __shared__ float xs[XH * XW];
    __shared__ float red[4][37];
    const int tid = threadIdx.x;
    const int rx = blockIdx.x * RW;
    const int row_begin = blockIdx.y * rows_per_block, row_end = min(hl, row_begin + rows_per_block);
    const TA* xb = xl + (size_t)blockIdx.z * hl * wl;
    const int W = 2 * wl;
    const TA* gb = dy + (size_t)blockIdx.z * (2 * hl) * W;
    const int c = tid & 31, r0 = tid >> 5;
    float acc[36], dbacc = 0.f;
#pragma unroll
    for (int i = 0; i < 36; ++i) acc[i] = 0.f;
    for (int ry = row_begin; ry < row_end; ry += RH) {
        __syncthreads();
        stage_batched<XH * XW, 256, 3, TA>(
            tid,
            [&](int i, bool& inside) {
                const int r = i / XW, cc = i - r * XW;
                const int gy = ry - 1 + r, gx = rx - 1 + cc;
                inside = gy >= 0 && gy < hl && gx >= 0 && gx < wl;
                return xb + (size_t)min(max(gy, 0), hl - 1) * wl + min(max(gx, 0), wl - 1);
            },
            [&](int i, TA v, bool inside) { xs[i] = inside ? (float)v : 0.f; });
        __syncthreads();
#pragma unroll
        for (int p = 0; p < 2; ++p) {
            const int r = r0 + 8 * p, py = ry + r, pxl = rx + c;
            if (py >= row_end || pxl >= wl) continue;
            const TA* g0 = gb + (size_t)(2 * py) * W + 2 * pxl;
            const float2 ga = ld2(g0), gbv = ld2(g0 + W);
            const float g[4] = {ga.x, ga.y, gbv.x, gbv.y};
            dbacc += (g[0] + g[1]) + (g[2] + g[3]);
#pragma unroll
            for (int m = 0; m < 9; ++m) {
                const float xv = xs[(r + m / 3) * XW + c + m % 3];
#pragma unroll
                for (int phase = 0; phase < 4; ++phase) acc[m * 4 + phase] += xv * g[phase];
            }
        }
    }
    const int lane = tid & 63, wv = tid >> 6;
#pragma unroll
    for (int i = 0; i < 36; ++i) {
        const float v = wave_reduce_sum(acc[i]);
        if (lane == 0) red[wv][i] = v;
    }
    dbacc = wave_reduce_sum(dbacc);
    if (lane == 0) red[wv][36] = dbacc;
    __syncthreads();
    const int blk = (blockIdx.z * gridDim.y + blockIdx.y) * gridDim.x + blockIdx.x;
    up1_write_row(partial + (size_t)blk * UP1_NOUT, [&](int i) { return red[0][i] + red[1][i] + red[2][i] + red[3][i]; }, tid);
}


int up_rows_per_block(int strips, int hl, int n, unsigned max_blocks = 2048u) {
    int rows = RH;
    while (rows < hl && (size_t)strips * ((hl + rows - 1) / rows) * n > max_blocks) rows += RH;
    return rows;
}

int check_up(uocr_ctx* ctx, int dtype, int n, int hl, int wl, int cin, int cout, int kh, int kw, int ph, int pw) {
    if (UOCR_DTYPE_BASE(dtype) != UOCR_F32 && UOCR_DTYPE_BASE(dtype) != UOCR_F16)
        UOCR_FAIL(ctx, UOCR_ERR_UNSUPPORTED, "upconv2x: float32 / float16 only");
    if (!((cin == CH && cout == CH) || (cin == 1 && cout == 1)) || kh != 5 || kw != 5 || ph != 2 || pw != 2)
        UOCR_FAIL(ctx, UOCR_ERR_UNSUPPORTED,
                  "upconv2x: 5x5 / padding 2 / 4 -> 4 or 1 -> 1 channels only (got %dx%d pad %d,%d %d -> %d)", kh, kw, ph,
                  pw, cin, cout);
    UOCR_REQUIRE(ctx, n > 0 && hl > 0 && wl > 0 && n <= 65535);
    return UOCR_OK;
}

ConvDims up_dims(int n, int hl, int wl, int cin, int cout) { return {n, hl, wl, cin, cout, 5, 5, 1, 1, 2, 2, 2 * hl, 2 * wl}; }
int up_ncols(const ConvWgrad& c) { return c.d.cin == 1 ? UP1_NOUT : UP4_NOUT; }

struct UpFwd { ConvFwd call; void* weff; };
struct UpDgrad { ConvDgrad call; const void* weff; };
template <class Up> bool up_h16_takes(uocr_ctx* ctx, const Up& u) { return uocr_upconv_h16_takes(ctx, u.call); }
template <class Up> int up_h16_run(uocr_ctx* ctx, const Up& u) { return uocr_upconv_h16_run(ctx, u.call); }
bool up_t32_takes(uocr_ctx* ctx, const UpDgrad& u) { return uocr_upconv_t32_takes(ctx, u.call); }
int up_t32_run(uocr_ctx* ctx, const UpDgrad& u) { return uocr_upconv_t32_run(ctx, u.call); }

int up_fwd_vector(uocr_ctx* ctx, const UpFwd& u) {
    const ConvFwd& c = u.call;
    const int n = c.d.n, hl = c.d.h, wl = c.d.w, cin = c.d.cin;
    const int strips = (wl + RW - 1) / RW, rows = up_rows_per_block(strips, hl, n, (unsigned)uocr_budget(ctx, 2048));
    if (cin != 1) uocr_note_split(ctx, (long long)strips * ((hl + rows - 1) / rows) * n, (long long)strips * ((hl + RH - 1) / RH) * n);
    return uocr_act_tags<0>(ctx, c.act, UOCR_ACT_NONE, [&](auto kinds) -> int {
    using K = decltype(kinds);
    UOCR_DISPATCH_TA(ctx, c.dtype, {
        if (cin == 1)
            hipLaunchKernelGGL((up1_fwd_kernel<TA>), dim3((wl + RW - 1) / RW, (hl + RH - 1) / RH, n), dim3(256), 0,
                               ctx->stream, (const TA*)c.x, (const float*)c.w, (const float*)c.b, (TA*)c.y, hl, wl,
                               c.use_bias, c.act, (float)c.act_alpha);
        else
            hipLaunchKernelGGL((upconv_fwd_kernel<TA, K>), dim3(strips, (hl + rows - 1) / rows, n), dim3(256), 0,
                               ctx->stream, (const TA*)c.x, (const float*)c.w, (const float*)c.b, (TA*)c.y, hl, wl, rows,
                               c.use_bias, c.act, (float)c.act_alpha, (float*)u.weff);
    });
    UOCR_LAUNCH_CHECK(ctx);
    return UOCR_OK;
    });
}

int up_dgrad_vector(uocr_ctx* ctx, const UpDgrad& u) {
    const ConvDgrad& c = u.call;
    const int n = c.d.n, hl = c.d.h, wl = c.d.w, cin = c.d.cin;
    const float* weff = (const float*)u.weff;
    if (cin != 1 && !weff) {
        const int rc = uocr_need_workspace(ctx, NWEFF * sizeof(float));
        if (rc != UOCR_OK) return rc;
        hipLaunchKernelGGL(upconv_weff_kernel, dim3(1), dim3(256), 0, ctx->stream, (const float*)c.w, (float*)ctx->workspace);
        weff = (const float*)ctx->workspace;
    }
    const dim3 grid((wl + RW - 1) / RW, (hl + RH - 1) / RH, n);
    return uocr_act_tags<1>(ctx, UOCR_ACT_NONE, c.mask.act, [&](auto kinds) -> int {
    using K = decltype(kinds);
    UOCR_DISPATCH_TA(ctx, c.dtype, {
        if (cin == 1)
            hipLaunchKernelGGL((up1_dgrad_kernel<TA>), grid, dim3(256), 0, ctx->stream, (const TA*)c.dy, (const float*)c.w,
                               (TA*)c.dx, hl, wl, (const TA*)c.mask.y, c.mask.act, (float)c.mask.alpha);
        else
            hipLaunchKernelGGL((upconv_dgrad_kernel<TA, K>), grid, dim3(256), 0, ctx->stream, (const TA*)c.dy,
                               weff, (TA*)c.dx, hl, wl, (const TA*)c.mask.y, c.mask.act, (float)c.mask.alpha);
    });
    UOCR_LAUNCH_CHECK(ctx);
    return UOCR_OK;
    });
}

int up_wgrad_finish(uocr_ctx* ctx, const ConvWgrad& c, const float* partial, int nblocks) {
    const float unscale = (float)uocr_grad_unscale(c.dtype);
    const int ncols = up_ncols(c), ndw = ncols - c.d.cin;
    const FinishDesc fd = finish_cols(partial, nblocks, ncols, ndw, (float*)c.dw, (float*)c.db, c.use_bias, c.accumulate, unscale);
    return uocr_finish(ctx, fd, [&] {
        hipLaunchKernelGGL(colsum_finish_kernel, dim3((ncols + 7) / 8), dim3(256), 0, ctx->stream, partial, nblocks,
                           ncols, ndw, (float*)c.dw, (float*)c.db, c.use_bias, c.accumulate, unscale);
    });
}

int up_wgrad_h16(uocr_ctx* ctx, const ConvWgrad& c) {
    const size_t floats = (size_t)ctx->cu_count * 8 * up_ncols(c);
    int rc = UOCR_OK, nblocks = 0;
    float* partial = uocr_partial_buffer(ctx, floats * sizeof(float), &rc);
    if (rc != UOCR_OK) return rc;
    rc = uocr_upconv_wgrad_h16(ctx, c, partial, floats, &nblocks);
    return rc != UOCR_OK ? rc : up_wgrad_finish(ctx, c, partial, nblocks);
}

int up_wgrad_vector(uocr_ctx* ctx, const ConvWgrad& c) {
    const int n = c.d.n, hl = c.d.h, wl = c.d.w, cin = c.d.cin;
    const int strips = (wl + RW - 1) / RW, rows = up_rows_per_block(strips, hl, n, (unsigned)uocr_budget(ctx, 1024));
    const int bands = (hl + rows - 1) / rows, nblocks = strips * bands * n;
    uocr_note_split(ctx, nblocks, (long long)strips * ((hl + RH - 1) / RH) * n);
    int rc = UOCR_OK;
    float* partial = uocr_partial_buffer(ctx, (size_t)nblocks * up_ncols(c) * sizeof(float), &rc);
    if (rc != UOCR_OK) return rc;
    UOCR_DISPATCH_TA(ctx, c.dtype, {
        if (cin == 1)
            hipLaunchKernelGGL((up1_wgrad_kernel<TA>), dim3(strips, bands, n), dim3(256), 0, ctx->stream,
                               (const TA*)c.x, (const TA*)c.dy, partial, hl, wl, rows);
        else
            hipLaunchKernelGGL((upconv_wgrad_kernel<TA>), dim3(strips, bands, n), dim3(256), 0, ctx->stream,
                               (const TA*)c.x, (const TA*)c.dy, partial, hl, wl, rows);
    });
    UOCR_LAUNCH_CHECK(ctx);
    return up_wgrad_finish(ctx, c, partial, nblocks);
}

constexpr ConvRow<UpFwd> UP_FWD_ROWS[] = {{CONV_NOT_NOTED, up_h16_takes, up_h16_run},
                                          {CONV_NOT_NOTED, uocr_conv_any_takes, up_fwd_vector}};
constexpr ConvRow<UpDgrad> UP_DGRAD_ROWS[] = {{CONV_NOT_NOTED, up_h16_takes, up_h16_run},
                                              {CONV_NOT_NOTED, up_t32_takes, up_t32_run},
                                              {CONV_NOT_NOTED, uocr_conv_any_takes, up_dgrad_vector}};
constexpr ConvRow<ConvWgrad> UP_WGRAD_ROWS[] = {{CONV_NOT_NOTED, uocr_upconv_wgrad_h16_takes, up_wgrad_h16},
                                                {CONV_NOT_NOTED, uocr_conv_any_takes, up_wgrad_vector}};

}

extern "C" int uocr_upconv2x_fwd(uocr_ctx* ctx, int dtype, const void* x_low, const void* w, const void* b, void* y,
                                 int n, int hl, int wl, int cin, int cout, int kh, int kw, int ph, int pw,
                                 int use_bias, int act, double act_alpha, void* weff) {
    UOCR_CHECK_CTX(ctx);
    UOCR_REQUIRE(ctx, x_low && w && b && y);
    int rc = check_up(ctx, dtype, n, hl, wl, cin, cout, kh, kw, ph, pw);
    if (rc != UOCR_OK) return rc;
    const ConvFwd call{dtype, up_dims(n, hl, wl, cin, cout), x_low, w, b, y, 0.0, use_bias, act, act_alpha};
    return uocr_conv_dispatch(ctx, 0, UP_FWD_ROWS, UpFwd{call, weff});
}

extern "C" int uocr_upconv2x_bwd_data(uocr_ctx* ctx, int dtype, const void* dy, const void* w, void* dx_low, int n,
                                      int hl, int wl, int cin, int cout, int kh, int kw, int ph, int pw,
                                      const void* x_act, int act, double act_alpha, const void* weff_in) {
    UOCR_CHECK_CTX(ctx);
    UOCR_REQUIRE(ctx, dy && w && dx_low);
    UOCR_REQUIRE(ctx, act == UOCR_ACT_NONE || x_act != nullptr);
    int rc = check_up(ctx, dtype, n, hl, wl, cin, cout, kh, kw, ph, pw);
    if (rc != UOCR_OK) return rc;
    const ActMask mask{act == UOCR_ACT_NONE ? nullptr : x_act, act, act_alpha};
    const ConvDgrad call{dtype, up_dims(n, hl, wl, cin, cout), dy, w, dx_low, mask};
    return uocr_conv_dispatch(ctx, 1, UP_DGRAD_ROWS, UpDgrad{call, weff_in});
}

extern "C" int uocr_upconv2x_bwd_weight(uocr_ctx* ctx, int dtype, const void* x_low, const void* dy, void* dw, void* db,
                                        int n, int hl, int wl, int cin, int cout, int kh, int kw, int ph, int pw,
                                        int use_bias, int accumulate) {
    UOCR_CHECK_CTX(ctx);
    UOCR_REQUIRE(ctx, x_low && dy && dw && db);
    int rc = check_up(ctx, dtype, n, hl, wl, cin, cout, kh, kw, ph, pw);
    if (rc != UOCR_OK) return rc;
    return uocr_conv_dispatch(ctx, 2, UP_WGRAD_ROWS,
                              ConvWgrad{dtype, up_dims(n, hl, wl, cin, cout), x_low, dy, dw, db, 0.0, use_bias, accumulate});
}
```

### univer-ocr_amd/csrc/ctx.hip

```cpp
#include <cstdlib>

#include "finish_group.h"
#include "gemm.h"
#include "uocr_common.h"

extern "C" {

int uocr_abi_version(void) { return UOCR_ABI_VERSION; }

int uocr_ctx_create(int device, size_t workspace_bytes, uocr_ctx** out) {
    if (!out || device < 0) return UOCR_ERR_ARG;
    *out = nullptr;
    int count = 0;
    if (hipGetDeviceCount(&count) != hipSuccess || device >= count) return UOCR_ERR_HIP;
    if (hipSetDevice(device) != hipSuccess) return UOCR_ERR_HIP;
    uocr_ctx* ctx = new uocr_ctx();
    ctx->device = device;
#ifdef UOCR_EXPERIMENTS
    if (const char* e = getenv("UOCR_H3")) ctx->opt_h3 = atoi(e);
#endif
    if (const char* e = getenv("UOCR_PAIR_PF")) ctx->opt_pair_pf = atoi(e);
    if (const char* e = getenv("UOCR_WGRAD_BANDS")) ctx->opt_wgrad_bands = atoi(e);
    if (hipStreamCreateWithFlags(&ctx->stream, hipStreamNonBlocking) != hipSuccess) {
        delete ctx;
// ... 8 lines not shown
            return UOCR_ERR_HIP;
        }
        ctx->workspace_bytes = workspace_bytes;
    }
    if (hipMalloc((void**)&ctx->sync, UOCR_SYNC_WORDS * sizeof(unsigned)) != hipSuccess ||
        hipMemsetAsync(ctx->sync, 0, UOCR_SYNC_WORDS * sizeof(unsigned), ctx->stream) != hipSuccess ||
        hipStreamSynchronize(ctx->stream) != hipSuccess) {
        if (ctx->sync) hipFree(ctx->sync);
        if (ctx->workspace) hipFree(ctx->workspace);
        hipStreamDestroy(ctx->stream);
        delete ctx;
        return UOCR_ERR_HIP;
    }
    *out = ctx;
    return UOCR_OK;
}

int uocr_ctx_create_cu_mask(int device, size_t workspace_bytes, const uint32_t* cu_mask, int mask_words, uocr_ctx** out) {
    if (!out || !cu_mask || mask_words <= 0) return UOCR_ERR_ARG;
    int rc = uocr_ctx_create(device, workspace_bytes, out);
    if (rc != UOCR_OK) return rc;
    uocr_ctx* ctx = *out;
    hipStream_t masked = nullptr;
    if (hipExtStreamCreateWithCUMask(&masked, (uint32_t)mask_words, cu_mask) != hipSuccess) {
        uocr_ctx_destroy(ctx);
        *out = nullptr;
        return UOCR_ERR_HIP;
    }
    hipStreamDestroy(ctx->stream);
    ctx->stream = masked;
    int cus = 0;
    for (int i = 0; i < mask_words; ++i) cus += __builtin_popcount(cu_mask[i]);
    if (cus > 0 && cus < ctx->cu_count) ctx->cu_count = cus;
    return UOCR_OK;
}

int uocr_ctx_destroy(uocr_ctx* ctx) {
    UOCR_CHECK_CTX(ctx);
    hipSetDevice(ctx->device);
    hipStreamSynchronize(ctx->stream);
    if (ctx->workspace) hipFree(ctx->workspace);
    if (ctx->sync) hipFree(ctx->sync);
    uocr_gemm_defer_free(ctx);
    uocr_finish_defer_free(ctx);
    if (ctx->owns_stream) hipStreamDestroy(ctx->stream);
    delete ctx;
    return UOCR_OK;
}

int uocr_ctx_set_stream(uocr_ctx* ctx, void* hip_stream) {
    UOCR_CHECK_CTX(ctx);
    if (ctx->owns_stream) {
        UOCR_HIP(ctx, hipStreamSynchronize(ctx->stream));
        UOCR_HIP(ctx, hipStreamDestroy(ctx->stream));
        ctx->owns_stream = false;
    }
    ctx->stream = (hipStream_t)hip_stream;
    return UOCR_OK;
}

int uocr_ctx_set_option(uocr_ctx* ctx, const char* key, int value) {
    UOCR_CHECK_CTX(ctx);
    UOCR_REQUIRE(ctx, key != nullptr);
    if (!strcmp(key, "mfma")) ctx->opt_mfma = value;
    else if (!strcmp(key, "fast_paths")) ctx->opt_fast = value;
    else if (!strcmp(key, "tiled")) ctx->opt_tiled = value;
    else if (!strcmp(key, "split_blocks")) ctx->opt_split = value;
    else if (!strcmp(key, "split_min")) ctx->opt_split_min = value;
    else if (!strcmp(key, "gemm_bm")) ctx->opt_bm = value;
    else if (!strcmp(key, "xcd_remap")) ctx->opt_xcd = value;
    else if (!strcmp(key, "h16")) ctx->opt_h16 = value;
    else if (!strcmp(key, "t32")) {
        if (value & ~UOCR_T32_BUILT)
            UOCR_FAIL(ctx, UOCR_ERR_UNSUPPORTED, "option t32 = %d asks for kernels this library was built without "
                      "(UOCR_BUILD_EXPERIMENTS=1 ./build.sh)", value);
        ctx->opt_t32 = value;
    }
    else if (!strcmp(key, "pair_band")) ctx->opt_pair_band = value;
    else if (!strcmp(key, "pair_g")) ctx->opt_pair_g = value;
    else if (!strcmp(key, "group_blocks")) ctx->opt_group_blocks = value;
    else if (!strcmp(key, "wgrad_bands") && value >= 0) ctx->opt_wgrad_bands = value;
    else if (!strcmp(key, "max_blocks") && value >= 0) ctx->opt_max_blocks = value;
    else if (!strcmp(key, "act_dispatch")) ctx->opt_act_dispatch = value != 0;
    else if (!strcmp(key, "h3")) {
#ifndef UOCR_EXPERIMENTS
        if (value) UOCR_FAIL(ctx, UOCR_ERR_UNSUPPORTED, "option h3: this library was built without conv_h3 "
                             "(UOCR_BUILD_EXPERIMENTS=1 ./build.sh)");
#endif
        ctx->opt_h3 = value;
    }
    else if (!strcmp(key, "pair_pf")) ctx->opt_pair_pf = value;
    else UOCR_FAIL(ctx, UOCR_ERR_ARG, "unknown option '%s'", key);
    return UOCR_OK;
}

int uocr_ctx_last_split(uocr_ctx* ctx, int* blocks, long long* items) {
    return uocr_report_read(ctx, UOCR_REPORT_SPLIT, blocks, items);
}

int uocr_ctx_last_gemm(uocr_ctx* ctx, int* bm, int* gm, int* gn, int* nsplit) {
    return uocr_report_read(ctx, UOCR_REPORT_GEMM, bm, gm, gn, nsplit);
}

int uocr_ctx_last_gemm_group(uocr_ctx* ctx, int* problems, int* split_problems) {
    return uocr_report_read(ctx, UOCR_REPORT_GEMM_GROUP, problems, split_problems);
}

int uocr_ctx_last_pair(uocr_ctx* ctx, int* kernel, int* g, int* mode, int* pf, int* nw, int* blocks_x, int* bands,
                       int* band_h) {
    return uocr_report_read(ctx, UOCR_REPORT_PAIR, kernel, g, mode, pf, nw, blocks_x, bands, band_h);
}

int uocr_ctx_last_conv(uocr_ctx* ctx, int* entry, int* kernel) {
    return uocr_report_read(ctx, UOCR_REPORT_CONV, entry, kernel);
}

void* uocr_ctx_get_stream(uocr_ctx* ctx) { return ctx ? (void*)ctx->stream : nullptr; }

int uocr_ctx_reserve_workspace(uocr_ctx* ctx, size_t bytes) {
    UOCR_CHECK_CTX(ctx);
    if (bytes <= ctx->workspace_bytes) return UOCR_OK;
    UOCR_HIP(ctx, hipSetDevice(ctx->device));
    UOCR_HIP(ctx, hipStreamSynchronize(ctx->stream));
    if (ctx->workspace) UOCR_HIP(ctx, hipFree(ctx->workspace));
    ctx->workspace = nullptr;
    ctx->workspace_bytes = 0;
    UOCR_HIP(ctx, hipMalloc(&ctx->workspace, bytes));
    ctx->workspace_bytes = bytes;
    return UOCR_OK;
}

const char* uocr_last_error(uocr_ctx* ctx) { return ctx ? ctx->err : "null context"; }

int uocr_malloc(uocr_ctx* ctx, size_t bytes, void** out) {
    UOCR_CHECK_CTX(ctx);
    UOCR_REQUIRE(ctx, out != nullptr);
    UOCR_HIP(ctx, hipSetDevice(ctx->device));
    UOCR_HIP(ctx, hipMalloc(out, bytes ? bytes : 1));
    return UOCR_OK;
}

int uocr_free(uocr_ctx* ctx, void* ptr) {
    UOCR_CHECK_CTX(ctx);
    if (ptr) UOCR_HIP(ctx, hipFree(ptr));
    return UOCR_OK;
}

int uocr_memset_zero(uocr_ctx* ctx, void* ptr, size_t bytes) {
    UOCR_CHECK_CTX(ctx);
    if (!bytes) return UOCR_OK;
    UOCR_REQUIRE(ctx, ptr != nullptr);
    UOCR_HIP(ctx, hipMemsetAsync(ptr, 0, bytes, ctx->stream));
    return UOCR_OK;
}

int uocr_h2d(uocr_ctx* ctx, void* dst, const void* src_host, size_t bytes) {
    UOCR_CHECK_CTX(ctx);
    if (!bytes) return UOCR_OK;
    UOCR_REQUIRE(ctx, dst && src_host);
    UOCR_HIP(ctx, hipMemcpyAsync(dst, src_host, bytes, hipMemcpyHostToDevice, ctx->stream));
    return UOCR_OK;
}

int uocr_d2h_sync(uocr_ctx* ctx, void* dst_host, const void* src, size_t bytes) {
    UOCR_CHECK_CTX(ctx);
    if (!bytes) return UOCR_OK;
    UOCR_REQUIRE(ctx, dst_host && src);
    UOCR_HIP(ctx, hipMemcpyAsync(dst_host, src, bytes, hipMemcpyDeviceToHost, ctx->stream));
    UOCR_HIP(ctx, hipStreamSynchronize(ctx->stream));
    return UOCR_OK;
}

int uocr_d2d(uocr_ctx* ctx, void* dst, const void* src, size_t bytes) {
    UOCR_CHECK_CTX(ctx);
    if (!bytes) return UOCR_OK;
    UOCR_REQUIRE(ctx, dst && src);
    UOCR_HIP(ctx, hipMemcpyAsync(dst, src, bytes, hipMemcpyDeviceToDevice, ctx->stream));
    return UOCR_OK;
}

int uocr_stream_sync(uocr_ctx* ctx) {
    UOCR_CHECK_CTX(ctx);
    UOCR_HIP(ctx, hipStreamSynchronize(ctx->stream));
    return UOCR_OK;
}

int uocr_event_create(void** out_event) {
    if (!out_event) return UOCR_ERR_ARG;
    hipEvent_t ev;
    if (hipEventCreate(&ev) != hipSuccess) return UOCR_ERR_HIP;
    *out_event = (void*)ev;
    return UOCR_OK;
}

int uocr_event_destroy(void* event) {
    if (!event) return UOCR_ERR_ARG;
    return hipEventDestroy((hipEvent_t)event) == hipSuccess ? UOCR_OK : UOCR_ERR_HIP;
// ... 75 lines not shown
```

### univer-ocr_amd/csrc/gemm_mfma.hip

```cpp
#include <array>
#include <type_traits>

#include "conv_dims.h"
#include "gemm.h"

namespace {

using f32x16 = __attribute__((ext_vector_type(16))) float;

constexpr int BN = 64;
constexpr int BD = 32;
constexpr int LDA = BD + 1;

struct alignas(16) F4 {
    float v[4];
};

__device__ __forceinline__ F4 f4_zero() { return F4{{0.f, 0.f, 0.f, 0.f}}; }
__device__ __forceinline__ F4 f4_fill(float x) { return F4{{x, x, x, x}}; }

enum : int { LD_KEEP = 0, LD_ZERO = 1, LD_E0 = 2, LD_PAD = 3 };

__device__ __forceinline__ F4 ld_resolve(F4 v, int code, float pad) {
    const float first = code == LD_PAD ? pad : (code == LD_E0 ? 1.f : 0.f);
    const float rest = code == LD_PAD ? pad : 0.f;
    F4 r;
    r.v[0] = code == LD_KEEP ? v.v[0] : first;
#pragma unroll
    for (int q = 1; q < 4; ++q) r.v[q] = code == LD_KEEP ? v.v[q] : rest;
    return r;
}

struct FastDiv {
    unsigned mul, shift;
    int d;
    FastDiv() = default;
    explicit FastDiv(int divisor) : mul(0), shift(0), d(divisor) {
        if (divisor > 1) {
            int lg = 0;
            while ((1ll << lg) < divisor) ++lg;
            const int p = 31 + lg;
            mul = (unsigned)(((1ull << p) + (unsigned)divisor - 1) / (unsigned)divisor);
            shift = (unsigned)(p - 32);
        }
    }
    __device__ __forceinline__ int div(int n) const { return d == 1 ? n : (int)(__umulhi((unsigned)n, mul) >> shift); }
};

struct Epilogue {
    float* c;
    long ldc;
    const float* bias;
    int act;
    float alpha;
    int accumulate;
    int split_row;
    float* c2;
    const float* mask_y;
    int mask_act;
    float mask_alpha;
};

__device__ __forceinline__ void epilogue_store(const Epilogue& e, int i, int j, float v) {
    if (e.bias) v += e.bias[j];
    v = act_apply(v, e.act, e.alpha);
    if (e.mask_act != UOCR_ACT_NONE) v *= act_grad_from_output<float>(e.mask_y[(long)i * e.ldc + j], e.mask_act, e.mask_alpha);
    float* dst = (e.split_row >= 0 && i >= e.split_row) ? e.c2 + j : e.c + (long)i * e.ldc + j;
    *dst = e.accumulate ? *dst + v : v;
}

struct BRowMajor {
    static constexpr bool DEPTH_CONTIG = false;
    const float* b;
    long ld;
    int rows, n;
    int vec_ok;
    __device__ __forceinline__ F4 load(int d, int j, int& code) const {
        const bool in = d < rows && j < n;
        code = in ? LD_KEEP : LD_ZERO;
        return *reinterpret_cast<const F4*>(in ? b + (long)d * ld + j : b);
    }
    struct Pos {
        const float* p;
        bool col_ok;
    };
    __device__ __forceinline__ Pos pos(int d, int j) const { return Pos{b + (long)d * ld + j, j < n}; }
    __device__ __forceinline__ F4 load_at(const Pos& c, long rows_on, int d, int& code) const {
        const bool in = c.col_ok && d < rows;
        code = in ? LD_KEEP : LD_ZERO;
        return *reinterpret_cast<const F4*>(in ? c.p + rows_on * ld : b);
    }
    __device__ __forceinline__ F4 load_slow(int d, int j) const {
        if (d >= rows || j >= n) return f4_zero();
        const float* p = b + (long)d * ld + j;
        if (vec_ok && j + 3 < n) return *reinterpret_cast<const F4*>(p);
        F4 r = f4_zero();
#pragma unroll
        for (int q = 0; q < 4; ++q)
            if (j + q < n) r.v[q] = p[q];
        return r;
    }
};

struct BDepthContig {
    static constexpr bool DEPTH_CONTIG = true;
    const float* b;
    long ld;
    int n, depth;
    int rows;
    FastDiv by_seg;
    int vec_ok;
    __device__ __forceinline__ const float* at(int d0, int j) const {
        const int kk = by_seg.div(d0);
        return b + ((long)kk * rows + j) * ld + (d0 - kk * by_seg.d);
    }
    __device__ __forceinline__ F4 load(int j, int d0, int& code) const {
        const bool in = j < n && d0 < depth;
        code = in ? LD_KEEP : LD_ZERO;
        return *reinterpret_cast<const F4*>(in ? at(d0, j) : b);
    }
    struct Pos {
        const float* p;
        bool col_ok;
    };
    __device__ __forceinline__ bool tiles_in_segments() const { return rows == 0 || by_seg.d % BD == 0; }
    __device__ __forceinline__ Pos pos(int j, int kq) const { return Pos{b + (long)j * ld + kq * 4, j < n}; }
    __device__ __forceinline__ F4 load_at(const Pos& c, int tile, int d0, int& code) const {
        const int kk = rows == 0 ? 0 : by_seg.div(tile * BD);
        const long on = (long)kk * rows * ld + (tile * BD - kk * by_seg.d);
        const bool in = c.col_ok && d0 < depth;
// ... 946 lines not shown
```

### univer-ocr_amd/csrc/uocr_common.h

```cpp
#pragma once
#include <hip/hip_runtime.h>
#include <stdint.h>
#include <stdio.h>
#include <string.h>

#include <type_traits>
#include <utility>

#include "univer_hip.h"

enum uocr_report_id {
    UOCR_REPORT_SPLIT,
    UOCR_REPORT_GEMM,
    UOCR_REPORT_GEMM_GROUP,
    UOCR_REPORT_PAIR,
    UOCR_REPORT_CONV,
    UOCR_REPORT_LABEL,
    UOCR_REPORT_LABEL_BATCH,
    UOCR_REPORT_CHAR_LABEL,
    UOCR_REPORT_LINE_CROP,
    UOCR_REPORT_ROTATE,
    UOCR_REPORT_ROTATION_SEARCH,
    UOCR_REPORT_PRED_TO_TEXT,
    UOCR_REPORT_PACK_LINES,
    UOCR_REPORT_PAGE_GEN,
    UOCR_REPORT_COUNT
};
constexpr int UOCR_REPORT_VALUES = 8;

struct uocr_ctx {
    int device = 0;
    hipStream_t stream = nullptr;
    bool owns_stream = true;
    void* workspace = nullptr;
    size_t workspace_bytes = 0;
    const double* snap_src = nullptr;
    int snap_count = 0;
    double* snap_ring = nullptr;
    int snap_ring_len = 0;
    unsigned* snap_counter = nullptr;
    void* gemm_defer = nullptr;
    void* finish_defer = nullptr;
    unsigned* sync = nullptr;
    int cu_count = 256;
    int opt_mfma = 1;
    int opt_fast = 1;
    int opt_tiled = 1;
    int opt_split = 1024;
    int opt_split_min = 3;
    int opt_xcd = 1;
    int opt_bm = 0;
    int opt_h16 = 1;
    int opt_t32 = 2;
    int opt_pair_band = 0;
    int opt_pair_pf = -1;
    int opt_h3 = 0;
    int opt_group_blocks = 0;
    int opt_wgrad_bands = 0;
    int opt_pair_g = 4;
    int opt_act_dispatch = 1;
    int opt_max_blocks = 0;
    long long report[UOCR_REPORT_COUNT][UOCR_REPORT_VALUES] = {};
    char err[512] = {};
};

#ifdef UOCR_EXPERIMENTS
constexpr int UOCR_T32_BUILT = 255;
#else
constexpr int UOCR_T32_BUILT = 2;
#endif

#define UOCR_FAIL(ctx, code, ...)                                   \
    do {                                                            \
        if (ctx) snprintf((ctx)->err, sizeof((ctx)->err), __VA_ARGS__); \
        return (code);                                              \
    } while (0)

#define UOCR_HIP(ctx, call)                                                              \
    do {                                                                                 \
        hipError_t e_ = (call);                                                          \
        if (e_ != hipSuccess)                                                            \
            UOCR_FAIL(ctx, UOCR_ERR_HIP, "%s failed: %s (%s:%d)", #call, hipGetErrorString(e_), \
                      __FILE__, __LINE__);                                               \
    } while (0)

#define UOCR_LAUNCH_CHECK(ctx)                                                           \
    do {                                                                                 \
        hipError_t e_ = hipGetLastError();                                               \
        if (e_ != hipSuccess)                                                            \
            UOCR_FAIL(ctx, UOCR_ERR_HIP, "kernel launch failed: %s (%s:%d)", hipGetErrorString(e_), \
                      __FILE__, __LINE__);                                               \
    } while (0)

#define UOCR_REQUIRE(ctx, cond)                                                          \
    do {                                                                                 \
        if (!(cond)) UOCR_FAIL(ctx, UOCR_ERR_ARG, "bad argument: %s (%s:%d)", #cond, __FILE__, __LINE__); \
    } while (0)

#define UOCR_CHECK_CTX(ctx) \
    do {                    \
        if (!(ctx)) return UOCR_ERR_ARG; \
    } while (0)

template <typename... V>
static inline void uocr_note(uocr_ctx* ctx, uocr_report_id id, V... v) {
    static_assert(sizeof...(V) >= 1 && sizeof...(V) <= UOCR_REPORT_VALUES, "a report holds 1 to UOCR_REPORT_VALUES values");
    long long* slot = ctx->report[id];
    ((*slot++ = (long long)v), ...);
}
template <typename... T>
static inline int uocr_report_read(uocr_ctx* ctx, uocr_report_id id, T*... out) {
    static_assert(sizeof...(T) >= 1 && sizeof...(T) <= UOCR_REPORT_VALUES, "a report holds 1 to UOCR_REPORT_VALUES values");
    UOCR_CHECK_CTX(ctx);
    if (!(out && ...)) UOCR_FAIL(ctx, UOCR_ERR_ARG, "bad argument: null out pointer of launch report %d", (int)id);
    const long long* slot = ctx->report[id];
    ((*out = (T)*slot++), ...);
    return UOCR_OK;
}

#define UOCR_DISPATCH(ctx, dtype, ...)                                   \
    do {                                                                 \
        if ((dtype) == UOCR_F32) { using T = float; __VA_ARGS__; }       \
        else if ((dtype) == UOCR_F64) { using T = double; __VA_ARGS__; } \
        else UOCR_FAIL(ctx, UOCR_ERR_DTYPE, "unknown dtype %d", (int)(dtype)); \
    } while (0)

#define UOCR_DISPATCH_ACT(ctx, dtype, ...)                                                        \
    do {                                                                                          \
        const int base_ = UOCR_DTYPE_BASE(dtype);                                                 \
        if (base_ == UOCR_F32) { using TS = float; using T = float; __VA_ARGS__; }                \
        else if (base_ == UOCR_F64) { using TS = double; using T = double; __VA_ARGS__; }         \
        else if (base_ == UOCR_F16) { using TS = _Float16; using T = float; __VA_ARGS__; }        \
        else UOCR_FAIL(ctx, UOCR_ERR_DTYPE, "unknown dtype %d", (int)(dtype));                    \
    } while (0)

#define UOCR_DISPATCH_STORAGE(ctx, dtype, ...)                                                    \
    do {                                                                                          \
        const int base_ = UOCR_DTYPE_BASE(dtype);                                                 \
        if (base_ == UOCR_F32) { using T = float; __VA_ARGS__; }                                  \
        else if (base_ == UOCR_F64) { using T = double; __VA_ARGS__; }                            \
        else if (base_ == UOCR_F16) { using T = _Float16; __VA_ARGS__; }                          \
        else UOCR_FAIL(ctx, UOCR_ERR_DTYPE, "unknown dtype %d", (int)(dtype));                    \
    } while (0)

static inline double uocr_grad_scale(int dtype) {
    return UOCR_DTYPE_BASE(dtype) == UOCR_F16 ? (double)(1u << (UOCR_DTYPE_GRAD_SCALE_LOG2(dtype) & 31)) : 1.0;
}
static inline double uocr_grad_unscale(int dtype) { return 1.0 / uocr_grad_scale(dtype); }

static inline int uocr_need_workspace(uocr_ctx* ctx, size_t bytes) {
    if (bytes > ctx->workspace_bytes)
        UOCR_FAIL(ctx, UOCR_ERR_WORKSPACE, "workspace too small: need %zu bytes, have %zu", bytes,
                  ctx->workspace_bytes);
    return UOCR_OK;
}

static inline unsigned uocr_blocks_for(size_t items, unsigned per_block, unsigned cap) {
    size_t b = (items + per_block - 1) / per_block;
    if (b < 1) b = 1;
    if (b > cap) b = cap;
    return (unsigned)b;
}

static inline long uocr_budget(const uocr_ctx* ctx, long budget) {
    return ctx->opt_max_blocks > 0 && ctx->opt_max_blocks < budget ? ctx->opt_max_blocks : budget;
}
static inline void uocr_note_split(uocr_ctx* ctx, long long blocks, long long items) {
    uocr_note(ctx, UOCR_REPORT_SPLIT, blocks, items);
}

template <typename K>
static inline int uocr_resident_blocks(uocr_ctx* ctx, K kernel, int threads, int* cache, int* out) {
    if (*cache == 0) {
        int nb = 0;
        UOCR_HIP(ctx, hipOccupancyMaxActiveBlocksPerMultiprocessor(&nb, kernel, threads, 0));
        *cache = nb > 0 ? nb : 1;
    }
    *out = *cache;
    return UOCR_OK;
}
template <typename K>
static inline int uocr_persistent_grid(uocr_ctx* ctx, K kernel, long ntiles, int slots_per_resident, int* cache,
                                       int* grid) {
    UOCR_REQUIRE(ctx, ntiles < (1l << 31));
// ... 170 lines not shown
__device__ __forceinline__ void st4(_Float16* p, float4 v) {
    uocr_h4 h;
    h.x = (_Float16)v.x;
    h.y = (_Float16)v.y;
    h.z = (_Float16)v.z;
    h.w = (_Float16)v.w;
    *reinterpret_cast<uocr_h4*>(p) = h;
}

#define UOCR_DISPATCH_TA(ctx, dtype, ...)                                                          \
    do {                                                                                           \
        const int base_ = UOCR_DTYPE_BASE(dtype);                                                  \
        if (base_ == UOCR_F32) { using TA = float; __VA_ARGS__; }                                  \
        else if (base_ == UOCR_F16) { using TA = _Float16; __VA_ARGS__; }                          \
        else UOCR_FAIL(ctx, UOCR_ERR_DTYPE, "dtype %d: this kernel exists for float32 / float16 only", (int)(dtype)); \
    } while (0)

static inline bool uocr_aligned_act(const void* p, int dtype) {
    return (reinterpret_cast<uintptr_t>(p) & (UOCR_DTYPE_BASE(dtype) == UOCR_F16 ? 7u : 15u)) == 0;
}
static inline bool uocr_aligned16(const void* p) { return (reinterpret_cast<uintptr_t>(p) & 15u) == 0; }

__device__ __forceinline__ float act_apply(float v, int act, float alpha) {
    switch (act) {
        case UOCR_ACT_RELU: return v * (v >= 0.f ? 1.f : 0.f);
        case UOCR_ACT_LEAKY: return v * ((v >= 0.f ? 1.f : 0.f) + alpha * (v < 0.f ? 1.f : 0.f));
        case UOCR_ACT_SIGMOID: return 1.f / (1.f + expf(-v));
        default: return v;
    }
}

template <typename T>
__device__ __forceinline__ T act_grad_from_output(T y, int act, T alpha) {
    if (act == UOCR_ACT_LEAKY) return y >= T(0) ? T(1) : alpha;
    if (act == UOCR_ACT_SIGMOID) return y * (T(1) - y);
    return T(1);
}

constexpr int UOCR_ACT_DYN = -1;
template <int ACT, int MASK>
struct ActKinds {
    static constexpr int act = ACT, mask = MASK;
    static constexpr bool dynamic = ACT == UOCR_ACT_DYN;
};
template <bool KEEP, class K>
using ActKindsIf = std::conditional_t<KEEP, K, ActKinds<UOCR_ACT_DYN, UOCR_ACT_DYN>>;
template <int KIND>
__host__ __device__ __forceinline__ int act_kind(int argument) {
    return KIND == UOCR_ACT_DYN ? argument : KIND;
}
template <int SIDE, class F>
static inline int uocr_act_tags(const uocr_ctx* ctx, int act, int mask_act, F&& f) {
    if (ctx->opt_act_dispatch) {
        if constexpr (SIDE == 0) {
            if (mask_act == UOCR_ACT_NONE && act == UOCR_ACT_NONE) return f(ActKinds<UOCR_ACT_NONE, UOCR_ACT_NONE>{});
            if (mask_act == UOCR_ACT_NONE && act == UOCR_ACT_LEAKY) return f(ActKinds<UOCR_ACT_LEAKY, UOCR_ACT_NONE>{});
            if (mask_act == UOCR_ACT_NONE && act == UOCR_ACT_SIGMOID) return f(ActKinds<UOCR_ACT_SIGMOID, UOCR_ACT_NONE>{});
        } else {
            if (act == UOCR_ACT_NONE && mask_act == UOCR_ACT_NONE) return f(ActKinds<UOCR_ACT_NONE, UOCR_ACT_NONE>{});
            if (act == UOCR_ACT_NONE && mask_act == UOCR_ACT_LEAKY) return f(ActKinds<UOCR_ACT_NONE, UOCR_ACT_LEAKY>{});
        }
    }
    return f(ActKinds<UOCR_ACT_DYN, UOCR_ACT_DYN>{});
}

template <int COUNT, int NT, int BATCH, typename V, typename Addr, typename Put>
__device__ __forceinline__ void stage_batched(int tid, Addr addr, Put put) {
    constexpr int K = (COUNT + NT - 1) / NT;
#pragma unroll
    for (int k0 = 0; k0 < K; k0 += BATCH) {
        V v[BATCH];
        bool in[BATCH];
#pragma unroll
        for (int k = 0; k < BATCH; ++k)
            if (k0 + k < K) v[k] = *addr(min(tid + NT * (k0 + k), COUNT - 1), in[k]);
#pragma unroll
        for (int k = 0; k < BATCH; ++k)
            if (k0 + k < K) {
                const int i = tid + NT * (k0 + k);
                if (i < COUNT) put(i, v[k], in[k]);
            }
    }
}

struct TileWalk {
    int strip, trow, img;
    int qx, qy, qz;
    __device__ __forceinline__ TileWalk(int first, int step, int tiles_x, int tiles_y) {
        strip = first % tiles_x;
        int r = first / tiles_x;
        trow = r % tiles_y;
        img = r / tiles_y;
        qx = step % tiles_x;
        r = step / tiles_x;
        qy = r % tiles_y;
        qz = r / tiles_y;
    }
    __device__ __forceinline__ void next(int tiles_x, int tiles_y) {
        strip += qx;
        int carry = strip >= tiles_x;
        strip -= carry ? tiles_x : 0;
        trow += qy + carry;
        carry = trow >= tiles_y;
        trow -= carry ? tiles_y : 0;
        img += qz + carry;
    }
};

int uocr_finish_sum(uocr_ctx* ctx, const double* partial, int count, double scale, double* out, int accumulate);
```

### univer-ocr_amd/hip/lib.py

```python
import ctypes as C
import os

_HERE = os.path.dirname(os.path.abspath(__file__))
_LIB_NAME = 'libuniver_hip.so'

F32, F64, F16 = 0, 1, 2
DP_UNIQUE_ID_BYTES = 128


def f16_scaled(k):
    return F16 | (int(k) << 8)
ACT_NONE, ACT_RELU, ACT_LEAKY, ACT_SIGMOID = 0, 1, 2, 3
LOSS_DICE, LOSS_JACCARD = 0, 1
THRESH_MEAN, THRESH_MEAN_MAX, THRESH_VALUE = 0, 1, 2
CONV_KERNELS = ('none', 'generic', 'mfma', 'h16', 'h16_wgrad', 'h16_wgrad_s2', 't32', 't32_wgrad', 'h3', 'tiled',
                'c16_expand', 'c16_reduce', 'c16_wgrad', 'dgrad_s2', 'dgrad_c64s2', 'wgrad_t542', 'wgrad_s2_tiled',
                'table_fast', 'table_px')


class HipError(RuntimeError):
    pass


def lib_path():
    return os.path.join(os.path.dirname(_HERE), _LIB_NAME)


def dtype_code(np_dtype):
    import numpy as np
    dt = np.dtype(np_dtype)
    if dt == np.float32:
        return F32
    if dt == np.float64:
        return F64
    if dt == np.float16:
        return F16
    raise HipError(f'unsupported dtype {dt}: the HIP backend stores float16 / float32 / float64')


_vp, _i, _d, _sz = C.c_void_p, C.c_int, C.c_double, C.c_size_t
_ctx = C.c_void_p

_PROTOS = {
    'uocr_ctx_create': [_i, _sz, C.POINTER(_ctx)],
    'uocr_ctx_create_cu_mask': [_i, _sz, C.POINTER(C.c_uint32), _i, C.POINTER(_ctx)],
    'uocr_ctx_destroy': [_ctx],
    'uocr_ctx_set_stream': [_ctx, _vp],
    'uocr_ctx_reserve_workspace': [_ctx, _sz],
    'uocr_ctx_set_option': [_ctx, C.c_char_p, _i],
    'uocr_ctx_last_split': [_ctx, C.POINTER(_i), C.POINTER(C.c_longlong)],
    'uocr_ctx_last_gemm': [_ctx, C.POINTER(_i), C.POINTER(_i), C.POINTER(_i), C.POINTER(_i)],
    'uocr_ctx_last_gemm_group': [_ctx, C.POINTER(_i), C.POINTER(_i)],
    'uocr_ctx_last_pair': [_ctx] + [C.POINTER(_i)] * 8,
    'uocr_ctx_last_conv': [_ctx, C.POINTER(_i), C.POINTER(_i)],
    'uocr_malloc': [_ctx, _sz, C.POINTER(_vp)],
    'uocr_free': [_ctx, _vp],
    'uocr_memset_zero': [_ctx, _vp, _sz],
    'uocr_h2d': [_ctx, _vp, _vp, _sz],
    'uocr_d2h_sync': [_ctx, _vp, _vp, _sz],
    'uocr_d2d': [_ctx, _vp, _vp, _sz],
    'uocr_stream_sync': [_ctx],
    'uocr_event_create': [C.POINTER(_vp)],
    'uocr_event_destroy': [_vp],
    'uocr_event_record': [_ctx, _vp],
    'uocr_stream_wait_event': [_ctx, _vp],
    'uocr_event_elapsed_ms_sync': [_vp, _vp, C.POINTER(C.c_float)],
    'uocr_event_synchronize': [_vp],
    'uocr_graph_begin_capture': [_ctx],
    'uocr_graph_end_capture': [_ctx, C.POINTER(_vp)],
    'uocr_graph_launch': [_ctx, _vp],
    'uocr_graph_destroy': [_vp],
    'uocr_ctx_set_loss_snapshot': [_ctx, _vp, _i, _vp, _i, _vp],
    'uocr_wgrad_defer_begin': [_ctx],
    'uocr_wgrad_defer_flush': [_ctx, _i],
    'uocr_device_info': [_ctx, C.c_char_p, _sz, C.POINTER(_i), C.POINTER(_sz)],
    'uocr_conv2d_fwd': [_ctx, _i, _vp, _vp, _vp, _vp] + [_i] * 13 + [_d, _i, _i, _d],
    'uocr_conv2d_bwd_data': [_ctx, _i, _vp, _vp, _vp] + [_i] * 13 + [_vp, _i, _d],
    'uocr_conv2d_bwd_weight': [_ctx, _i, _vp, _vp, _vp, _vp] + [_i] * 13 + [_d, _i, _i],
    'uocr_conv_pair_fwd': [_ctx, _i] + [_vp] * 6 + [_i] * 4 + [_d, _i, _i, _d, _i],
    'uocr_conv_pair_bwd': [_ctx, _i] + [_vp] * 11 + [_i] * 4 + [_d, _i, _i, _d, _i, _i],
    'uocr_upconv2x_fwd': [_ctx, _i, _vp, _vp, _vp, _vp] + [_i] * 9 + [_i, _i, _d, _vp],
    'uocr_upconv2x_bwd_data': [_ctx, _i, _vp, _vp, _vp] + [_i] * 9 + [_vp, _i, _d, _vp],
    'uocr_upconv2x_bwd_weight': [_ctx, _i, _vp, _vp, _vp, _vp] + [_i] * 9 + [_i, _i],
    'uocr_maxpool2d_fwd': [_ctx, _i, _vp, _vp, _vp] + [_i] * 12,
    'uocr_maxpool2d_bwd': [_ctx, _i, _vp, _vp, _vp] + [_i] * 12,
    'uocr_upsample2d_fwd': [_ctx, _i, _vp, _vp] + [_i] * 6,
    'uocr_upsample2d_bwd': [_ctx, _i, _vp, _vp] + [_i] * 6,
    'uocr_act_fwd': [_ctx, _i, _i, _d, _vp, _vp, _sz],
    'uocr_act_bwd': [_ctx, _i, _i, _d, _vp, _vp, _vp, _sz],
    'uocr_act_bwd_from_output': [_ctx, _i, _i, _d, _vp, _vp, _vp, _sz],
    'uocr_dense_fwd': [_ctx, _i, _vp, _vp, _vp, _i, _i, _i],
    'uocr_dense_bwd': [_ctx, _i, _vp, _vp, _vp, _vp, _vp, _i, _i, _i, _i],
    'uocr_dense_fwd_act': [_ctx, _i, _vp, _vp, _vp, _i, _i, _i, _i, _d],
    'uocr_dense_bwd_act': [_ctx, _i, _vp, _vp, _vp, _vp, _vp, _i, _i, _i, _i, _i, _d],
    'uocr_fixed_width_fwd': [_ctx, _i, _vp, _vp] + [_i] * 5,
    'uocr_fixed_width_bwd': [_ctx, _i, _vp, _vp] + [_i] * 5,
    'uocr_copy_2d': [_ctx, _i, _vp, _sz, _vp, _sz, _sz, _sz],
    'uocr_add': [_ctx, _i, _vp, _vp, _vp, _sz],
    'uocr_axpy': [_ctx, _i, _d, _vp, _vp, _sz],
    'uocr_scale': [_ctx, _i, _d, _vp, _sz],
    'uocr_fill': [_ctx, _i, _vp, _d, _sz],
    'uocr_convert': [_ctx, _i, _vp, _i, _vp, _sz],
    'uocr_u8_to_float': [_ctx, _i, _vp, _vp, _d, _sz],
    'uocr_seg_loss': [_ctx, _i, _i, _vp, _vp, _vp, _vp, _i, _i, _i, _i],
    'uocr_softmax_ce': [_ctx, _i, _vp, _vp, _vp, _vp, _i, _i],
    'uocr_sigmoid_ce': [_ctx, _i, _vp, _vp, _vp, _vp, _i, _sz],
    'uocr_l2_reg': [_ctx, _i, _vp, _vp, _sz, _d, _vp, _i],
    'uocr_l1_reg': [_ctx, _i, _vp, _vp, _sz, _d, _vp, _i],
    'uocr_adam_step': [_ctx, _i, _vp, _vp, _vp, _vp, _sz, _d, _d, _d, _d],
    'uocr_momentum_step': [_ctx, _i, _vp, _vp, _vp, _sz, _d, _d],
    'uocr_momentum_step_fused': [_ctx, _i, _vp, _vp, _vp, _sz, _d, _d, _i, C.POINTER(C.c_longlong), C.POINTER(C.c_longlong),
                                 C.POINTER(C.c_int), C.POINTER(C.c_double), _vp, _i, _vp],
    'uocr_adam_step_fused': [_ctx, _i, _vp, _vp, _vp, _vp, _sz, _d, _d, _d, _d, _i, C.POINTER(C.c_longlong),
                             C.POINTER(C.c_longlong), C.POINTER(C.c_int), C.POINTER(C.c_double), _vp, _i, _vp],
    'uocr_rmsprop_step': [_ctx, _i, _vp, _vp, _vp, _sz, _d, _d, _d],
    'uocr_has_nan': [_ctx, _i, _vp, _sz, _vp],
    'uocr_label_components': [_ctx, _i, _vp, _i, _i, _i, _i, _d, _vp, _vp, _i, _vp],
    'uocr_masked_crop': [_ctx, _i, _vp, _vp] + [_i] * 10 + [_vp, _i, _i],
    'uocr_ctx_last_label': [_ctx, C.POINTER(_i), C.POINTER(_i), C.POINTER(_i)],
    'uocr_label_batch': [_ctx, _i, _i, C.POINTER(_vp)] + [C.POINTER(_i)] * 4 + [_i, _d, C.POINTER(_vp), _vp, _i, _vp],
    'uocr_ctx_last_label_batch': [_ctx, C.POINTER(_i), C.POINTER(_i), C.POINTER(_i), C.POINTER(_i)],
    'uocr_char_label': [_ctx, _i, _i, C.POINTER(_vp), C.POINTER(_i), C.POINTER(_i), _i, _i, _i, C.POINTER(_vp),
                        C.POINTER(_vp)],
    'uocr_ctx_last_char_label': [_ctx, C.POINTER(_i), C.POINTER(_i), C.POINTER(_i), C.POINTER(_i)],
    'uocr_line_crop': [_ctx, _i, _i, C.POINTER(_vp)] + [C.POINTER(_i)] * 10 + [C.POINTER(_vp), C.POINTER(_i)],
    'uocr_ctx_last_line_crop': [_ctx, C.POINTER(_i), C.POINTER(_i), C.POINTER(_i), C.POINTER(_i)],
    'uocr_rotated_extent': [_ctx, _vp, _i, _i, _i, _i, _i, C.POINTER(_i), C.POINTER(_i), C.POINTER(_d), C.POINTER(_d),
                            C.POINTER(_i), _vp],
    'uocr_rotate_crop': [_ctx, _i, _i, C.POINTER(_vp), C.POINTER(_vp)] + [C.POINTER(_i)] * 4 + [C.POINTER(_d)] * 2 +
                        [C.POINTER(_i)] * 2 + [C.POINTER(_vp), C.POINTER(_i)],
    'uocr_ctx_last_rotate': [_ctx, C.POINTER(_i), C.POINTER(_i), C.POINTER(_i), C.POINTER(_i)],
    'uocr_rotation_search': [_ctx, _vp, _i, _i, _i, _i, _i, C.POINTER(_i), C.POINTER(_i), _i, _vp, _vp, _vp],
    'uocr_rotation_search_workspace': [_i, C.POINTER(_sz)],
    'uocr_ctx_last_rotation_search': [_ctx, C.POINTER(_i), C.POINTER(_i), C.POINTER(_i)],
    'uocr_pred_to_text': [_ctx, _i, _i, C.POINTER(_vp), C.POINTER(_i), _i, C.POINTER(_i), C.POINTER(_vp), C.POINTER(_i),
                          C.POINTER(_vp)],
    'uocr_ctx_last_pred_to_text': [_ctx, C.POINTER(_i), C.POINTER(_i), C.POINTER(_i)],
# ... 55 lines not shown
```

### univer-ocr_amd/nn/gpu.py

```python
import contextlib
import ctypes as C
import os

import numpy as np
os.environ.setdefault('GPU_MAX_HW_QUEUES', '8')

import torch

from ..hip import lib as hiplib
from ..hip.lib import HipError

_TORCH_DT = {np.dtype(np.float32): torch.float32, np.dtype(np.float64): torch.float64,
             np.dtype(np.float16): torch.float16,
             np.dtype(np.uint8): torch.uint8, np.dtype(np.int32): torch.int32, np.dtype(np.int64): torch.int64}
_CODE = {torch.float32: hiplib.F32, torch.float64: hiplib.F64, torch.float16: hiplib.F16}
_NP_DT = {v: k for k, v in _TORCH_DT.items()}


class Lane:

    __slots__ = ('handle', 'stream', 'side', 'held', 'fork_ev', 'join_ev', 'keep', 'dirty')

    def __init__(self, stream=None, handle=None):
        self.handle = C.c_void_p() if handle is None else handle
# ... 51 lines not shown
            if cu_mask is not None:
                lane.stream = self._stream(external=self.lib.uocr_ctx_get_stream(lane.handle))
            with self.on(lane):
                if cu_mask is None:
                    self.call('uocr_ctx_set_stream', C.c_void_p(lane.stream.cuda_stream))
                for key, value in self._options.items() if options else ():
                    self.call('uocr_ctx_set_option', key.encode(), value)
        except BaseException as error:
            self.lib.uocr_ctx_destroy(lane.handle)
            lane.handle = C.c_void_p()
            if isinstance(error, HipError):
                raise HipError(f'{what}: {error}') from error
            raise
        return lane

    @contextlib.contextmanager
    def on(self, lane):
        previous = self.current
        self.current = lane
        try:
            yield lane
        finally:
            self.current = previous

    def add_lane(self, workspace_mb=256, priority=0, xcds=None):
        if xcds is None:
            lane = self._open(Lane(self._stream(priority)), 'lane', int(workspace_mb) << 20)
        else:
            cus = self.device_info()['cu_count']
            mask = (C.c_uint32 * ((cus + 31) // 32))()
            for i in range(cus):
                if i % 8 in set(xcds):
                    mask[i // 32] |= 1 << (i % 32)
            lane = self._open(Lane(), f'lane on XCDs {sorted(set(xcds))}', int(workspace_mb) << 20, cu_mask=mask)
        self.lanes.append(lane)
        return len(self.lanes) - 1

    @contextlib.contextmanager
    def lane(self, index):
        lane, previous = self.lanes[index], torch.cuda.current_stream()
        with self.on(lane):
            torch.cuda.set_stream(lane.stream)
            try:
                yield lane.stream
            finally:
                torch.cuda.set_stream(previous)

    def call(self, name, *args):
        fn = self._fn.get(name)
        if fn is None:
            fn = self._fn[name] = getattr(self.lib, name)
        rc = fn(self.current.handle, *args)
        self.launches += 1
        if rc != 0:
            msg = self.lib.uocr_last_error(self.current.handle)
            raise HipError(f'{name} failed ({rc}): {msg.decode() if msg else "?"}')

    def set_option(self, key, value):
        for lane in self.lanes + [lane.side for lane in self.lanes if lane.side is not None]:
            with self.on(lane):
                self.call('uocr_ctx_set_option', key.encode(), int(value))
        self._options[key] = int(value)

    def _report(self, symbol):
        outs = [pointer._type_() for pointer in hiplib._PROTOS[symbol][1:]]
        self.call(symbol, *[C.byref(out) for out in outs])
        return tuple(out.value for out in outs)

    def last_split(self):
        return self._report('uocr_ctx_last_split')

    def last_gemm(self):
        return self._report('uocr_ctx_last_gemm')

    def last_gemm_group(self):
        return self._report('uocr_ctx_last_gemm_group')

    def last_pair(self):
        return self._report('uocr_ctx_last_pair')

    def last_conv(self):
        return self._report('uocr_ctx_last_conv')

    def last_label(self):
        return self._report('uocr_ctx_last_label')

    def last_label_batch(self):
        return self._report('uocr_ctx_last_label_batch')

    def last_char_label(self):
        return self._report('uocr_ctx_last_char_label')

    def last_line_crop(self):
        return self._report('uocr_ctx_last_line_crop')

    def last_rotate(self):
        return self._report('uocr_ctx_last_rotate')

    def last_rotation_search(self):
        return self._report('uocr_ctx_last_rotation_search')

    def last_pred_to_text(self):
        return self._report('uocr_ctx_last_pred_to_text')

    def last_pack_lines(self):
        return self._report('uocr_ctx_last_pack_lines')

    def last_page_gen(self):
        return self._report('uocr_ctx_last_page_gen')

    def set_loss_snapshot(self, arena):
        if arena is None:
            self.call('uocr_ctx_set_loss_snapshot', None, 0, None, 0, None)
        else:
            self.call('uocr_ctx_set_loss_snapshot', arena.array.ptr, arena.array.shape[0], arena.ring.ptr, arena.ring_len,
                      arena.counter.ptr)

    @contextlib.contextmanager
    def defer_wgrad(self):
        lane = self.current
        if lane.held is not None:
            raise HipError('defer_wgrad: a deferred group is already open on this lane')
        self.call('uocr_wgrad_defer_begin')
        lane.held = held = []
        failed = True
        try:
            yield
            failed = False
        finally:
            lane.held = None
            try:
                self.call('uocr_wgrad_defer_flush', 0)
            except HipError:
                if not failed:
                    raise
            finally:
                held.clear()

    def keep(self, *arrays):
        held = self.current.held
        if held is not None:
            held.extend(arrays)

    def flush_deferred(self):
        held = self.current.held
        if held is not None:
            self.call('uocr_wgrad_defer_flush', 1)
            held.clear()

    def side(self, *keep):
        return self._fork_side(keep) if self.side_on else _NO_SCOPE

    @contextlib.contextmanager
    def _fork_side(self, keep):
        lane = self.current
        if lane.side is None:
            side = Lane(self._stream())
            side.fork_ev, side.join_ev = Event(self), Event(self)
            lane.side = self._open(side, 'side stream', int(os.environ.get('UOCR_SIDE_WORKSPACE_MB', '128')) << 20,
                                   options=True)
        side = lane.side
        side.fork_ev.record()
        with self.on(side):
            side.fork_ev.wait()
            side.keep.extend(keep)
            side.dirty = True
# ... 421 lines not shown
```

Baseline: 34440 images/s.

## Defer wgrad launch and fuse it with following dgrad into one paired kernel

The weight-gradient kernel for selected small 5x5 convs is now held back instead of launched. When the matching data-gradient call on the same dy arrives, both run as a single combined grid whose blocks split between the two bodies. This cuts kernel launches and lets two small, under-filled grids share the GPU at once. Any other API call flushes the held launch alone, which adds host-side state and ordering risk.

Result: slower. 33940 images/s (-1.5%).

```diff
diff --git a/include/univer_hip.h b/include/univer_hip.h
--- a/include/univer_hip.h
+++ b/include/univer_hip.h
@@ -62,6 +62,7 @@
     UOCR_CONV_TABLE_PX = 18
 };
 int uocr_ctx_last_conv(uocr_ctx* ctx, int* entry, int* kernel);
+int uocr_ctx_pair_bwd_launches(uocr_ctx* ctx, long long* launches, int* w_blocks, int* d_blocks);
 int uocr_ctx_reserve_workspace(uocr_ctx* ctx, size_t bytes);
 const char* uocr_last_error(uocr_ctx* ctx);
 int uocr_malloc(uocr_ctx* ctx, size_t bytes, void** out);
diff --git a/univer-ocr_amd/csrc/conv_api.hip b/univer-ocr_amd/csrc/conv_api.hip
--- a/univer-ocr_amd/csrc/conv_api.hip
+++ b/univer-ocr_amd/csrc/conv_api.hip
@@ -1,4 +1,5 @@
 #include "conv_dims.h"
+#include "pair_bwd.h"
 
 namespace {
 
@@ -55,14 +56,28 @@
 int uocr_conv2d_bwd_data(uocr_ctx* ctx, int dtype, const void* dy, const void* w, void* dx, int n, int h, int wd,
                          int cin, int cout, int kh, int kw, int sh, int sw, int ph, int pw, int oh, int ow,
                          const void* x_act, int act, double act_alpha) {
-    UOCR_CHECK_CTX(ctx);
+    UOCR_CHECK_CTX_KEEP(ctx);
     const ConvDims d{n, h, wd, cin, cout, kh, kw, sh, sw, ph, pw, oh, ow};
-    int rc = check_dims(ctx, d);
+    const ConvDgrad call{dtype, d, dy, w, dx, ActMask{act == UOCR_ACT_NONE ? nullptr : x_act, act, act_alpha}};
+    const auto checked = [&]() -> int {
+        int rc = check_dims(ctx, d);
+        if (rc) return rc;
+        UOCR_REQUIRE(ctx, dy && w && dx);
+        UOCR_REQUIRE(ctx, act == UOCR_ACT_NONE || (x_act && (act == UOCR_ACT_SIGMOID || (act == UOCR_ACT_LEAKY && act_alpha > 0))));
+        return UOCR_OK;
+    };
+    int rc = checked();
+    const auto into_fast = [&] {
+        int (*const fast_run)(uocr_ctx*, const ConvDgrad&) = uocr_conv_fast_run;
+        const ConvRow<ConvDgrad>* taker = uocr_conv_taker(ctx, DGRAD_ROWS, call);
+        return taker && taker->run == fast_run;
+    };
+    if (rc != UOCR_OK || !uocr_held_matches(ctx, dtype, dy, d) || !into_fast()) {
+        const int held_rc = uocr_held_launch_alone(ctx);
+        if (rc == UOCR_OK) rc = held_rc;
+    }
     if (rc) return rc;
-    UOCR_REQUIRE(ctx, dy && w && dx);
-    UOCR_REQUIRE(ctx, act == UOCR_ACT_NONE || (x_act && (act == UOCR_ACT_SIGMOID || (act == UOCR_ACT_LEAKY && act_alpha > 0))));
-    const ActMask mask{act == UOCR_ACT_NONE ? nullptr : x_act, act, act_alpha};
-    return uocr_conv_dispatch(ctx, 1, DGRAD_ROWS, ConvDgrad{dtype, d, dy, w, dx, mask});
+    return uocr_conv_dispatch(ctx, 1, DGRAD_ROWS, call);
 }
 
 int uocr_conv2d_bwd_weight(uocr_ctx* ctx, int dtype, const void* x, const void* dy, void* dw, void* db, int n, int h,
diff --git a/univer-ocr_amd/csrc/conv_dims.h b/univer-ocr_amd/csrc/conv_dims.h
--- a/univer-ocr_amd/csrc/conv_dims.h
+++ b/univer-ocr_amd/csrc/conv_dims.h
@@ -20,10 +20,15 @@
 template <class Call> bool uocr_conv_any_takes(uocr_ctx*, const Call&) { return true; }
 
 template <class Call, size_t N>
+const ConvRow<Call>* uocr_conv_taker(uocr_ctx* ctx, const ConvRow<Call> (&rows)[N], const Call& c) {
+    for (const ConvRow<Call>& r : rows)
+        if (r.takes(ctx, c)) return &r;
+    return nullptr;
+}
+template <class Call, size_t N>
 int uocr_conv_dispatch(uocr_ctx* ctx, int entry, const ConvRow<Call> (&rows)[N], const Call& c) {
-    for (const ConvRow<Call>& r : rows)
-        if (r.takes(ctx, c))
-            return r.kernel == CONV_NOT_NOTED ? r.run(ctx, c) : uocr_noted_conv(ctx, entry, r.kernel, r.run(ctx, c));
+    if (const ConvRow<Call>* r = uocr_conv_taker(ctx, rows, c))
+        return r->kernel == CONV_NOT_NOTED ? r->run(ctx, c) : uocr_noted_conv(ctx, entry, r->kernel, r->run(ctx, c));
     UOCR_FAIL(ctx, UOCR_ERR_UNSUPPORTED, "no conv kernel takes this call");
 }
 
diff --git a/univer-ocr_amd/csrc/conv_fast.hip b/univer-ocr_amd/csrc/conv_fast.hip
--- a/univer-ocr_amd/csrc/conv_fast.hip
+++ b/univer-ocr_amd/csrc/conv_fast.hip
@@ -1,5 +1,6 @@
 #include "finish_group.h"
 #include "conv_dims.h"
+#include "pair_bwd.h"
 
 namespace {
 
@@ -201,12 +202,11 @@
 }
 
 template <int CIN, int COUT, typename TA, class K>
-__global__ __launch_bounds__(256) void conv_dgrad_s2(const TA* __restrict__ dy, const float* __restrict__ w,
-                                                     TA* __restrict__ dx, FastDims d,
-                                                     const TA* __restrict__ mask_y, int mask_act,
-                                                     float mask_alpha) {
+__device__ __forceinline__ void conv_dgrad_s2_body(const BlockAt& at, const TA* __restrict__ dy,
+                                                   const float* __restrict__ w, TA* __restrict__ dx, FastDims d,
+                                                   const TA* __restrict__ mask_y, int mask_act, float mask_alpha) {
     mask_act = act_kind<K::mask>(mask_act);
-    const int i = blockIdx.x * 64 + threadIdx.x, j = blockIdx.y * 4 + threadIdx.y, b = blockIdx.z;
+    const int i = at.bx * 64 + at.tx, j = at.by * 4 + at.ty, b = at.bz;
     if (2 * i >= d.w || 2 * j >= d.h) return;
     const TA* gb = dy + (size_t)b * d.oh * d.ow * COUT;
     float g[3][3][COUT];
@@ -261,16 +261,37 @@
         }
     }
 }
-
-__global__ __launch_bounds__(256) void conv_dgrad_c64s2(const float* __restrict__ dy, const float* __restrict__ w,
-                                                        float* __restrict__ dx, int n, int h, int wd, int oh, int ow,
-                                                        const float* __restrict__ mask_y, int mask_act,
-                                                        float mask_alpha) {
+template <int CIN, int COUT, typename TA, class K>
+__global__ __launch_bounds__(256) void conv_dgrad_s2(const TA* __restrict__ dy, const float* __restrict__ w,
+                                                     TA* __restrict__ dx, FastDims d,
+                                                     const TA* __restrict__ mask_y, int mask_act,
+                                                     float mask_alpha) {
+    conv_dgrad_s2_body<CIN, COUT, TA, K>(block_at_launch(), dy, w, dx, d, mask_y, mask_act, mask_alpha);
+}
+template <typename TA>
+struct DgradArgs { const TA* dy; const float* w; TA* dx; FastDims d; const TA* mask_y; int mask_act; float mask_alpha; };
+template <int CIN, int COUT, typename TA, class K>
+struct DgradS2Body {
+    using Args = DgradArgs<TA>;
+    static constexpr size_t LDS = 0;
+    static __device__ __forceinline__ void run(const BlockAt& at, void*, const Args& a) {
+        conv_dgrad_s2_body<CIN, COUT, TA, K>(at, a.dy, a.w, a.dx, a.d, a.mask_y, a.mask_act, a.mask_alpha);
+    }
+    static void launch(hipStream_t stream, dim3 grid, const Args& a) {
+        hipLaunchKernelGGL((conv_dgrad_s2<CIN, COUT, TA, K>), grid, dim3(64, 4), 0, stream, a.dy, a.w, a.dx, a.d, a.mask_y,
+                           a.mask_act, a.mask_alpha);
+    }
+};
+
+__device__ __forceinline__ void conv_dgrad_c64s2_body(const BlockAt& at, const float* __restrict__ dy,
+                                                      const float* __restrict__ w, float* __restrict__ dx, int n, int h,
+                                                      int wd, int oh, int ow, const float* __restrict__ mask_y,
+                                                      int mask_act, float mask_alpha) {
     constexpr int KH = 5, KW = 3, CO = 64;
-    const int q = threadIdx.x & 15;
-    const int b = blockIdx.z, y = blockIdx.y;
-    const bool live = (int)(blockIdx.x * 16 + (threadIdx.x >> 4)) < wd;
-    const int x = live ? blockIdx.x * 16 + (threadIdx.x >> 4) : wd - 1;
+    const int q = at.tid & 15;
+    const int b = at.bz, y = at.by;
+    const bool live = (int)(at.bx * 16 + (at.tid >> 4)) < wd;
+    const int x = live ? at.bx * 16 + (at.tid >> 4) : wd - 1;
     const size_t pix = ((size_t)b * h + y) * wd + x;
     const float* gb = dy + (size_t)b * oh * ow * CO + 4 * q;
     float acc = 0.f;
@@ -294,6 +315,12 @@
     if (!live || q != 0) return;
     if (mask_act != UOCR_ACT_NONE) acc *= act_grad_from_output<float>(mask_y[pix], mask_act, mask_alpha);
     dx[pix] = acc;
+}
+__global__ __launch_bounds__(256) void conv_dgrad_c64s2(const float* __restrict__ dy, const float* __restrict__ w,
+                                                        float* __restrict__ dx, int n, int h, int wd, int oh, int ow,
+                                                        const float* __restrict__ mask_y, int mask_act,
+                                                        float mask_alpha) {
+    conv_dgrad_c64s2_body(block_at_launch(), dy, w, dx, n, h, wd, oh, ow, mask_y, mask_act, mask_alpha);
 }
 
 template <int N, int OFFS, typename TA>
@@ -393,13 +420,13 @@
 }
 
 template <int KH, int KW, int CIN, int COUT, int PX, typename TA>
-__global__ __launch_bounds__(256) void conv_dgrad_px(const TA* __restrict__ dy, const float* __restrict__ w,
-                                                     TA* __restrict__ dx, FastDims d,
-                                                     const TA* __restrict__ mask_y, int mask_act, float mask_alpha) {
+__device__ __forceinline__ void conv_dgrad_px_body(const BlockAt& at, const TA* __restrict__ dy,
+                                                   const float* __restrict__ w, TA* __restrict__ dx, FastDims d,
+                                                   const TA* __restrict__ mask_y, int mask_act, float mask_alpha) {
     constexpr int NG = PX + KW - 1;
-    const int ix0 = (blockIdx.x * 64 + threadIdx.x) * PX;
-    const int iy = blockIdx.y * 4 + threadIdx.y;
-    const int b = blockIdx.z;
+    const int ix0 = (at.bx * 64 + at.tx) * PX;
+    const int iy = at.by * 4 + at.ty;
+    const int b = at.bz;
     if (ix0 >= d.w || iy >= d.h) return;
     float acc[PX][CIN];
 #pragma unroll
@@ -464,6 +491,24 @@
         store_vec<CIN>(dx + off, acc[p]);
     }
 }
+template <int KH, int KW, int CIN, int COUT, int PX, typename TA>
+__global__ __launch_bounds__(256) void conv_dgrad_px(const TA* __restrict__ dy, const float* __restrict__ w,
+                                                     TA* __restrict__ dx, FastDims d,
+                                                     const TA* __restrict__ mask_y, int mask_act, float mask_alpha) {
+    conv_dgrad_px_body<KH, KW, CIN, COUT, PX, TA>(block_at_launch(), dy, w, dx, d, mask_y, mask_act, mask_alpha);
+}
+template <int KH, int KW, int CIN, int COUT, int PX, typename TA>
+struct DgradPxBody {
+    using Args = DgradArgs<TA>;
+    static constexpr size_t LDS = 0;
+    static __device__ __forceinline__ void run(const BlockAt& at, void*, const Args& a) {
+        conv_dgrad_px_body<KH, KW, CIN, COUT, PX, TA>(at, a.dy, a.w, a.dx, a.d, a.mask_y, a.mask_act, a.mask_alpha);
+    }
+    static void launch(hipStream_t stream, dim3 grid, const Args& a) {
+        hipLaunchKernelGGL((conv_dgrad_px<KH, KW, CIN, COUT, PX, TA>), grid, dim3(64, 4), 0, stream, a.dy, a.w, a.dx, a.d,
+                           a.mask_y, a.mask_act, a.mask_alpha);
+    }
+};
 
 template <int KH, int KW, int PY, bool FLIP>
 __global__ __launch_bounds__(256) void conv_c16_reduce(const float* __restrict__ src, const float* __restrict__ w,
@@ -722,15 +767,14 @@
 };
 
 template <int KH, int KW, int CIN, int COUT, int SH, int SW, int KYR, int COB, int PX, bool CLAMP, typename TA>
-__global__ __launch_bounds__(256) void conv_wgrad_fast(const TA* __restrict__ x, const TA* __restrict__ dy,
-                                                       float* __restrict__ partial, FastDims d, float pad,
-                                                       int rows_per_block, int nbands) {
+__device__ __forceinline__ void conv_wgrad_fast_body(
+    const BlockAt& at, float (*red)[WgradCfg<KH, KW, CIN, COUT, SH, SW, KYR, COB>::NP] , const TA* __restrict__ x,
+    const TA* __restrict__ dy, float* __restrict__ partial, FastDims d, float pad, int rows_per_block, int nbands) {
     using C = WgradCfg<KH, KW, CIN, COUT, SH, SW, KYR, COB>;
     constexpr int NXV = (PX - 1) * SW + KW;
-    __shared__ float red[4][C::NP];
-    const int lane = threadIdx.x, wv = threadIdx.y;
-    const int band = blockIdx.x % nbands, b = blockIdx.x / nbands;
-    const int kyg = blockIdx.y / C::OCG, ocg = blockIdx.y % C::OCG;
+    const int lane = at.tx, wv = at.ty;
+    const int band = at.bx % nbands, b = at.bx / nbands;
+    const int kyg = at.by / C::OCG, ocg = at.by % C::OCG;
     const int ky0 = kyg * KYR, oc0 = ocg * COB;
     const int row0 = band * rows_per_block;
     const int row1 = min(d.oh, row0 + rows_per_block);
@@ -811,9 +855,31 @@
     for (int r = 0; r < C::NP / 64; ++r) red[wv][base + r] = acc[r];
     __syncthreads();
     const int tid = wv * 64 + lane;
-    float* out = partial + ((size_t)blockIdx.y * gridDim.x + blockIdx.x) * C::NP;
+    float* out = partial + ((size_t)at.by * at.gx + at.bx) * C::NP;
     for (int a = tid; a < C::NP; a += 256) out[a] = red[0][a] + red[1][a] + red[2][a] + red[3][a];
 }
+template <int KH, int KW, int CIN, int COUT, int SH, int SW, int KYR, int COB, int PX, bool CLAMP, typename TA>
+__global__ __launch_bounds__(256) void conv_wgrad_fast(const TA* __restrict__ x, const TA* __restrict__ dy,
+                                                       float* __restrict__ partial, FastDims d, float pad,
+                                                       int rows_per_block, int nbands) {
+    __shared__ float red[4][WgradCfg<KH, KW, CIN, COUT, SH, SW, KYR, COB>::NP];
+    conv_wgrad_fast_body<KH, KW, CIN, COUT, SH, SW, KYR, COB, PX, CLAMP, TA>(block_at_launch(), red, x, dy, partial, d, pad,
+                                                                              rows_per_block, nbands);
+}
+template <int KH, int KW, int CIN, int COUT, int SH, int SW, int KYR, int COB, int PX, bool CLAMP, typename TA>
+struct WgradFastBody {
+    using C = WgradCfg<KH, KW, CIN, COUT, SH, SW, KYR, COB>;
+    struct Args { const TA *x, *dy; float* partial; FastDims d; float pad; int rows_per_block, nbands; };
+    static constexpr size_t LDS = sizeof(float) * 4 * C::NP;
+    static __device__ __forceinline__ void run(const BlockAt& at, void* lds, const Args& a) {
+        conv_wgrad_fast_body<KH, KW, CIN, COUT, SH, SW, KYR, COB, PX, CLAMP, TA>(
+            at, reinterpret_cast<float(*)[C::NP]>(lds), a.x, a.dy, a.partial, a.d, a.pad, a.rows_per_block, a.nbands);
+    }
+    static void launch(hipStream_t stream, dim3 grid, const Args& a) {
+        hipLaunchKernelGGL((conv_wgrad_fast<KH, KW, CIN, COUT, SH, SW, KYR, COB, PX, CLAMP, TA>), grid, dim3(64, 4), 0, stream,
+                           a.x, a.dy, a.partial, a.d, a.pad, a.rows_per_block, a.nbands);
+    }
+};
 
 template <int KH, int KW, int CIN, int COUT, int KYR, int COB, int NW, int NP>
 __global__ __launch_bounds__(256) void conv_wgrad_fast_finish(const float* __restrict__ partial, float* __restrict__ dw,
@@ -1062,6 +1128,8 @@
     struct Fwd { int px = 0, cob = 0, py = 0; } fwd;
     struct Dx { int px = 0, py = 0; } dx;
     struct Dw { int kyr = 0, cob = 0, px = 0; } dw;
+    bool pair = false;
+    int pair_max_out = 0;
 };
 
 constexpr FastRow FAST_CONVS[] = {
@@ -1070,13 +1138,13 @@
     {.kh = 3, .kw = 3, .cin = 16, .cout = 1, .sh = 1, .sw = 1,
      .fwd = {.px = 4}, .dx = {.px = 2}, .dw = {.kyr = 1, .cob = 1, .px = 1}},
     {.kh = 5, .kw = 5, .cin = 1, .cout = 1, .sh = 2, .sw = 2,
-     .fwd = {.px = 4}, .dx = {.py = 1}, .dw = {.kyr = 5, .cob = 1, .px = 4}},
+     .fwd = {.px = 4}, .dx = {.py = 1}, .dw = {.kyr = 5, .cob = 1, .px = 4}, .pair = true, .pair_max_out = 1 << 19},
     {.kh = 5, .kw = 5, .cin = 1, .cout = 1, .sh = 1, .sw = 1,
-     .fwd = {.px = 4}, .dx = {.px = 8}, .dw = {.kyr = 5, .cob = 1, .px = 8}},
+     .fwd = {.px = 4}, .dx = {.px = 8}, .dw = {.kyr = 5, .cob = 1, .px = 8}, .pair = true},
     {.kh = 5, .kw = 5, .cin = 1, .cout = 4, .sh = 2, .sw = 2,
      .fwd = {.px = 4}, .dx = {.py = 1}, .dw = {.kyr = 5, .cob = 4, .px = 1}},
     {.kh = 5, .kw = 5, .cin = 4, .cout = 4, .sh = 2, .sw = 2,
-     .fwd = {.px = 4}, .dx = {.py = 1}, .dw = {.kyr = 1, .cob = 4, .px = 2}},
+     .fwd = {.px = 4}, .dx = {.py = 1}, .dw = {.kyr = 1, .cob = 4, .px = 2}, .pair = true},
     {.kh = 5, .kw = 5, .cin = 4, .cout = 4, .sh = 1, .sw = 1,
      .fwd = {.px = 4}, .dx = {.px = 4}, .dw = {.kyr = 1, .cob = 4, .px = 4}},
     {.kh = 5, .kw = 5, .cin = 4, .cout = 2, .sh = 1, .sw = 1,
@@ -1084,6 +1152,13 @@
     {.kh = 5, .kw = 3, .cin = 1, .cout = 64, .sh = 2, .sw = 1,
      .fwd = {.cob = 4, .py = 1}, .dx = {.py = 1}, .dw = {.kyr = 5, .cob = 8, .px = 1}},
 };
+constexpr int fast_row(int kh, int kw, int cin, int cout, int sh, int sw) {
+    for (int i = 0; i < (int)std::size(FAST_CONVS); ++i) {
+        const FastRow& r = FAST_CONVS[i];
+        if (r.kh == kh && r.kw == kw && r.cin == cin && r.cout == cout && r.sh == sh && r.sw == sw) return i;
+    }
+    return -1;
+}
 
 template <int I>
 struct FastConv {
@@ -1124,16 +1199,35 @@
         });
     }
 
+    template <typename TA>
+    using WBody = WgradFastBody<KH, KW, CIN, COUT, SH, SW, R.dw.kyr, R.dw.cob, R.dw.px, (CIN >= 4), TA>;
+    template <typename TA>
+    static DgradArgs<TA> dgrad_args(const ConvDgrad& c) {
+        return {(const TA*)c.dy, (const float*)c.w, (TA*)c.dx, dims(c.d), (const TA*)c.mask.y, c.mask.act, (float)c.mask.alpha};
+    }
+    template <typename TA, class D>
+    static int dgrad_or_pair(uocr_ctx* ctx, const ConvDgrad& c, const typename D::Args& da, dim3 grid) {
+        if constexpr (R.pair) {
+            if (uocr_held_matches(ctx, c.dtype, c.dy, c.d) && ctx->held.kind == I && uocr_pair_fits(ctx, grid))
+                return uocr_launch_pair<WBody<TA>, D>(ctx, da, grid);
+        }
+        const int rc = uocr_held_launch_alone(ctx);
+        if (rc != UOCR_OK) return rc;
+        D::launch(ctx->stream, grid, da);
+        UOCR_LAUNCH_CHECK(ctx);
+        return UOCR_OK;
+    }
+
     static int run(uocr_ctx* ctx, const ConvDgrad& c) {
         const ConvDims& d = c.d;
         UOCR_DISPATCH_TA(ctx, c.dtype, {
             if constexpr (R.dx.px > 0) {
                 const int groups = (d.w + R.dx.px - 1) / R.dx.px;
-                const dim3 grid((groups + 63) / 64, (d.h + 3) / 4, d.n), block(64, 4);
-                hipLaunchKernelGGL((conv_dgrad_px<KH, KW, CIN, COUT, R.dx.px, TA>), grid, block, 0, ctx->stream,
-                                   (const TA*)c.dy, (const float*)c.w, (TA*)c.dx, dims(d), (const TA*)c.mask.y,
-                                   c.mask.act, (float)c.mask.alpha);
+                const dim3 grid((groups + 63) / 64, (d.h + 3) / 4, d.n);
+                return dgrad_or_pair<TA, DgradPxBody<KH, KW, CIN, COUT, R.dx.px, TA>>(ctx, c, dgrad_args<TA>(c), grid);
             } else {
+                const int rc = uocr_held_launch_alone(ctx);
+                if (rc != UOCR_OK) return rc;
                 const dim3 grid((d.w + 63) / 64, (d.h + 4 * R.dx.py - 1) / (4 * R.dx.py), d.n), block(64, 4);
                 hipLaunchKernelGGL((conv_dgrad_fast<KH, KW, CIN, COUT, SH, SW, R.dx.py, TA>), grid, block, 0, ctx->stream,
                                    (const TA*)c.dy, (const float*)c.w, (TA*)c.dx, dims(d), (const TA*)c.mask.y,
@@ -1158,15 +1252,21 @@
         int rc = UOCR_OK;
         float* partial = uocr_partial_buffer(ctx, bytes, &rc);
         if (rc) return rc;
-        UOCR_DISPATCH_TA(ctx, c.dtype, {
-            hipLaunchKernelGGL((conv_wgrad_fast<KH, KW, CIN, COUT, SH, SW, R.dw.kyr, R.dw.cob, R.dw.px, (CIN >= 4), TA>),
-                               dim3(nblocks, ngroups), dim3(64, 4), 0, ctx->stream, (const TA*)c.x, (const TA*)c.dy,
-                               partial, dims(d), (float)c.pad_value, rows, nbands);
-        });
-        UOCR_LAUNCH_CHECK(ctx);
         const float unscale = (float)uocr_grad_unscale(c.dtype);
         const FinishDesc fd = finish_fast(partial, nblocks, ngroups, {C::NP, C::NW, KW, CIN, COUT, R.dw.kyr, R.dw.cob},
                                           (float*)c.dw, (float*)c.db, c.use_bias, c.accumulate, unscale);
+        UOCR_DISPATCH_TA(ctx, c.dtype, {
+            const typename WBody<TA>::Args args{(const TA*)c.x, (const TA*)c.dy, partial, dims(d), (float)c.pad_value, rows, nbands};
+            if constexpr (R.pair) {
+                const bool pays = R.pair_max_out == 0 || (long long)d.n * d.oh * d.ow <= R.pair_max_out;
+                if (ctx->opt_pair_bwd && pays && uocr_finish_defer(ctx, fd)) {
+                    uocr_hold_wgrad(ctx, uocr_held_alone<WBody<TA>>, I, c, dim3(nblocks, ngroups), args);
+                    return UOCR_OK;
+                }
+            }
+            WBody<TA>::launch(ctx->stream, dim3(nblocks, ngroups), args);
+        });
+        UOCR_LAUNCH_CHECK(ctx);
         return uocr_finish(ctx, fd, [&] {
             hipLaunchKernelGGL((conv_wgrad_fast_finish<KH, KW, CIN, COUT, R.dw.kyr, R.dw.cob, C::NW, C::NP>),
                                dim3(C::NACC, ngroups), dim3(256), 0, ctx->stream, (const float*)partial, (float*)c.dw,
@@ -1185,6 +1285,8 @@
 struct C16Args { const void *src, *w, *bias; void* dst; float pad; int use_bias, act; float alpha; ActMask mask; };
 template <class Kernel>
 int launch_c16(uocr_ctx* ctx, Kernel kernel, int py, const C16Args& a, const ConvDims& d, int entry, int kernel_id) {
+    const int rc = uocr_held_launch_alone(ctx);
+    if (rc != UOCR_OK) return rc;
     const dim3 grid((d.w + 15) / 16, (d.h + 4 * py - 1) / (4 * py), d.n), block(64, 4);
     hipLaunchKernelGGL(kernel, grid, block, 0, ctx->stream, (const float*)a.src, (const float*)a.w, (const float*)a.bias,
                        (float*)a.dst, d.n, d.h, d.w, d.ph, d.pw, a.pad, a.use_bias, a.act, a.alpha,
@@ -1230,6 +1332,8 @@
         return launch_c16(ctx, conv_c16_reduce<3, 3, 4, true>, 4, c16, d, 1, UOCR_CONV_C16_REDUCE);
     if (f32 && d.kh == 5 && d.kw == 3 && d.sh == 2 && d.sw == 1 && d.ph == 0 && d.pw == 1 && d.cin == 1 && d.cout == 64 &&
         d.h <= 65535 && d.n <= 65535) {
+        const int rc = uocr_held_launch_alone(ctx);
+        if (rc != UOCR_OK) return rc;
         hipLaunchKernelGGL(conv_dgrad_c64s2, dim3((unsigned)((d.w + 15) / 16), d.h, d.n), dim3(256), 0, ctx->stream,
                            (const float*)c.dy, (const float*)c.w, (float*)c.dx, d.n, d.h, d.w, d.oh, d.ow,
                            (const float*)c.mask.y, c.mask.act, (float)c.mask.alpha);
@@ -1238,26 +1342,21 @@
         return UOCR_OK;
     }
     if (is_5x5_s2_pad2(d) && ((d.cin == 1 && (d.cout == 1 || d.cout == 4)) || (d.cin == 4 && d.cout == 4))) {
-        const dim3 grid(((d.w + 1) / 2 + 63) / 64, ((d.h + 1) / 2 + 3) / 4, d.n), block(64, 4);
-        const FastDims fd{d.n, d.h, d.w, d.oh, d.ow, d.ph, d.pw};
+        const dim3 grid(((d.w + 1) / 2 + 63) / 64, ((d.h + 1) / 2 + 3) / 4, d.n);
         const int rc = uocr_act_tags<1>(ctx, UOCR_ACT_NONE, c.mask.act, [&](auto kinds) -> int {
             using K = decltype(kinds);
             using D = ActKinds<UOCR_ACT_DYN, UOCR_ACT_DYN>;
             UOCR_DISPATCH_TA(ctx, c.dtype, {
-                auto launch = [&](auto kernel) {
-                    hipLaunchKernelGGL(kernel, grid, block, 0, ctx->stream, (const TA*)c.dy, (const float*)c.w, (TA*)c.dx, fd,
-                                       (const TA*)c.mask.y, c.mask.act, (float)c.mask.alpha);
+                auto launch = [&](auto row, auto body) {
+                    return decltype(row)::template dgrad_or_pair<TA, decltype(body)>(ctx, c, row.template dgrad_args<TA>(c), grid);
                 };
-                if (d.cin == 4) launch(conv_dgrad_s2<4, 4, TA, K>);
-                else if (d.cout == 1) launch(conv_dgrad_s2<1, 1, TA, D>);
-                else launch(conv_dgrad_s2<1, 4, TA, D>);
+                if (d.cin == 4) return launch(FastConv<fast_row(5, 5, 4, 4, 2, 2)>{}, DgradS2Body<4, 4, TA, K>{});
+                if (d.cout == 1) return launch(FastConv<fast_row(5, 5, 1, 1, 2, 2)>{}, DgradS2Body<1, 1, TA, D>{});
+                return launch(FastConv<fast_row(5, 5, 1, 4, 2, 2)>{}, DgradS2Body<1, 4, TA, D>{});
             });
-            UOCR_LAUNCH_CHECK(ctx);
             return UOCR_OK;
         });
-        if (rc != UOCR_OK) return rc;
-        uocr_note_conv(ctx, 1, UOCR_CONV_DGRAD_S2);
-        return UOCR_OK;
+        return uocr_noted_conv(ctx, 1, UOCR_CONV_DGRAD_S2, rc);
     }
     int rc = UOCR_OK;
     if (with_fast_conv(d, [&](auto fc) { rc = uocr_noted_conv(ctx, 1, fc.DX_KERNEL, fc.run(ctx, c)); })) return rc;
diff --git a/univer-ocr_amd/csrc/conv_up.hip b/univer-ocr_amd/csrc/conv_up.hip
--- a/univer-ocr_amd/csrc/conv_up.hip
+++ b/univer-ocr_amd/csrc/conv_up.hip
@@ -1,6 +1,7 @@
 #include "up_phase.h"
 #include "finish_group.h"
 #include "conv_toeplitz.h"
+#include "pair_bwd.h"
 
 namespace {
 
@@ -389,15 +390,18 @@
 }
 
 template <typename TA>
-__global__ __launch_bounds__(256) void up1_dgrad_kernel(const TA* __restrict__ dy, const float* __restrict__ w,
-                                                        TA* __restrict__ dxl, int hl, int wl,
-                                                        const TA* __restrict__ mask_y, int mask_act,
-                                                        float mask_alpha) {
-    __shared__ float gs[GH * GW];
-    const int tid = threadIdx.x;
-    const int rx = blockIdx.x * RW, ry = blockIdx.y * RH;
+struct UpWgradArgs { const TA *xl, *dy; float* partial; int hl, wl, rows_per_block; };
+template <typename TA>
+struct UpDgradArgs { const TA* dy; const float* w; TA* dxl; int hl, wl; const TA* mask_y; int mask_act; float mask_alpha; };
+
+template <typename TA>
+__device__ __forceinline__ void up1_dgrad_body(const BlockAt& at, float* gs , const TA* __restrict__ dy,
+                                               const float* __restrict__ w, TA* __restrict__ dxl, int hl, int wl,
+                                               const TA* __restrict__ mask_y, int mask_act, float mask_alpha) {
+    const int tid = at.tid;
+    const int rx = at.bx * RW, ry = at.by * RH;
     const int H = 2 * hl, W = 2 * wl;
-    const TA* gb = dy + (size_t)blockIdx.z * H * W;
+    const TA* gb = dy + (size_t)at.bz * H * W;
     stage_batched<GH * GW, 256, 10, TA>(
         tid,
         [&](int i, bool& inside) {
@@ -423,24 +427,42 @@
         }
         const int qy = ry + r, qx = rx + c;
         if (qy >= hl || qx >= wl) continue;
-        const size_t off = ((size_t)blockIdx.z * hl + qy) * wl + qx;
+        const size_t off = ((size_t)at.bz * hl + qy) * wl + qx;
         if (mask_act != UOCR_ACT_NONE) acc *= act_grad_from_output<float>(ld1(mask_y + off), mask_act, mask_alpha);
         st1(dxl + off, acc);
     }
 }
-
-template <typename TA>
-__global__ __launch_bounds__(256) void up1_wgrad_kernel(const TA* __restrict__ xl, const TA* __restrict__ dy,
-                                                        float* __restrict__ partial, int hl, int wl,
-                                                        int rows_per_block) {
-    __shared__ float xs[XH * XW];
-    __shared__ float red[4][37];
-    const int tid = threadIdx.x;
-    const int rx = blockIdx.x * RW;
-    const int row_begin = blockIdx.y * rows_per_block, row_end = min(hl, row_begin + rows_per_block);
-    const TA* xb = xl + (size_t)blockIdx.z * hl * wl;
+template <typename TA>
+__global__ __launch_bounds__(256) void up1_dgrad_kernel(const TA* __restrict__ dy, const float* __restrict__ w,
+                                                        TA* __restrict__ dxl, int hl, int wl,
+                                                        const TA* __restrict__ mask_y, int mask_act,
+                                                        float mask_alpha) {
+    __shared__ float gs[GH * GW];
+    up1_dgrad_body<TA>(block_at_launch(), gs, dy, w, dxl, hl, wl, mask_y, mask_act, mask_alpha);
+}
+template <typename TA>
+struct Up1DgradBody {
+    using Args = UpDgradArgs<TA>;
+    static constexpr size_t LDS = sizeof(float) * GH * GW;
+    static __device__ __forceinline__ void run(const BlockAt& at, void* lds, const Args& a) {
+        up1_dgrad_body<TA>(at, (float*)lds, a.dy, a.w, a.dxl, a.hl, a.wl, a.mask_y, a.mask_act, a.mask_alpha);
+    }
+    static void launch(hipStream_t stream, dim3 grid, const Args& a) {
+        hipLaunchKernelGGL((up1_dgrad_kernel<TA>), grid, dim3(256), 0, stream, a.dy, a.w, a.dxl, a.hl, a.wl, a.mask_y,
+                           a.mask_act, a.mask_alpha);
+    }
+};
+
+template <typename TA>
+__device__ __forceinline__ void up1_wgrad_body(const BlockAt& at, float* xs , float (*red)[37] ,
+                                               const TA* __restrict__ xl, const TA* __restrict__ dy,
+                                               float* __restrict__ partial, int hl, int wl, int rows_per_block) {
+    const int tid = at.tid;
+    const int rx = at.bx * RW;
+    const int row_begin = at.by * rows_per_block, row_end = min(hl, row_begin + rows_per_block);
+    const TA* xb = xl + (size_t)at.bz * hl * wl;
     const int W = 2 * wl;
-    const TA* gb = dy + (size_t)blockIdx.z * (2 * hl) * W;
+    const TA* gb = dy + (size_t)at.bz * (2 * hl) * W;
     const int c = tid & 31, r0 = tid >> 5;
     float acc[36], dbacc = 0.f;
 #pragma unroll
@@ -482,9 +504,31 @@
     dbacc = wave_reduce_sum(dbacc);
     if (lane == 0) red[wv][36] = dbacc;
     __syncthreads();
-    const int blk = (blockIdx.z * gridDim.y + blockIdx.y) * gridDim.x + blockIdx.x;
+    const int blk = (at.bz * at.gy + at.by) * at.gx + at.bx;
     up1_write_row(partial + (size_t)blk * UP1_NOUT, [&](int i) { return red[0][i] + red[1][i] + red[2][i] + red[3][i]; }, tid);
 }
+template <typename TA>
+__global__ __launch_bounds__(256) void up1_wgrad_kernel(const TA* __restrict__ xl, const TA* __restrict__ dy,
+                                                        float* __restrict__ partial, int hl, int wl,
+                                                        int rows_per_block) {
+    __shared__ float xs[XH * XW];
+    __shared__ float red[4][37];
+    up1_wgrad_body<TA>(block_at_launch(), xs, red, xl, dy, partial, hl, wl, rows_per_block);
+}
+template <typename TA>
+struct Up1WgradBody {
+    using Args = UpWgradArgs<TA>;
+    static constexpr size_t LDS = sizeof(float) * (XH * XW + 4 * 37);
+    static __device__ __forceinline__ void run(const BlockAt& at, void* lds, const Args& a) {
+        float* xs = (float*)lds;
+        up1_wgrad_body<TA>(at, xs, reinterpret_cast<float(*)[37]>(xs + XH * XW), a.xl, a.dy, a.partial, a.hl, a.wl,
+                           a.rows_per_block);
+    }
+    static void launch(hipStream_t stream, dim3 grid, const Args& a) {
+        hipLaunchKernelGGL((up1_wgrad_kernel<TA>), grid, dim3(256), 0, stream, a.xl, a.dy, a.partial, a.hl, a.wl,
+                           a.rows_per_block);
+    }
+};
 
 
 int up_rows_per_block(int strips, int hl, int n, unsigned max_blocks = 2048u) {
@@ -504,6 +548,7 @@
     return UOCR_OK;
 }
 
+constexpr int HELD_UP_VECTOR = 100;
 ConvDims up_dims(int n, int hl, int wl, int cin, int cout) { return {n, hl, wl, cin, cout, 5, 5, 1, 1, 2, 2, 2 * hl, 2 * wl}; }
 int up_ncols(const ConvWgrad& c) { return c.d.cin == 1 ? UP1_NOUT : UP4_NOUT; }
 
@@ -536,6 +581,17 @@
     });
 }
 
+template <class W, class D>
+int up_dgrad_or_pair(uocr_ctx* ctx, const ConvDgrad& c, const typename D::Args& da, dim3 grid) {
+    if (uocr_held_matches(ctx, c.dtype, c.dy, c.d) && ctx->held.kind == HELD_UP_VECTOR && uocr_pair_fits(ctx, grid))
+        return uocr_launch_pair<W, D>(ctx, da, grid);
+    const int rc = uocr_held_launch_alone(ctx);
+    if (rc != UOCR_OK) return rc;
+    D::launch(ctx->stream, grid, da);
+    UOCR_LAUNCH_CHECK(ctx);
+    return UOCR_OK;
+}
+
 int up_dgrad_vector(uocr_ctx* ctx, const UpDgrad& u) {
     const ConvDgrad& c = u.call;
     const int n = c.d.n, hl = c.d.h, wl = c.d.w, cin = c.d.cin;
@@ -550,22 +606,30 @@
     return uocr_act_tags<1>(ctx, UOCR_ACT_NONE, c.mask.act, [&](auto kinds) -> int {
     using K = decltype(kinds);
     UOCR_DISPATCH_TA(ctx, c.dtype, {
-        if (cin == 1)
-            hipLaunchKernelGGL((up1_dgrad_kernel<TA>), grid, dim3(256), 0, ctx->stream, (const TA*)c.dy, (const float*)c.w,
-                               (TA*)c.dx, hl, wl, (const TA*)c.mask.y, c.mask.act, (float)c.mask.alpha);
-        else
-            hipLaunchKernelGGL((upconv_dgrad_kernel<TA, K>), grid, dim3(256), 0, ctx->stream, (const TA*)c.dy,
-                               weff, (TA*)c.dx, hl, wl, (const TA*)c.mask.y, c.mask.act, (float)c.mask.alpha);
+        if (cin == 1) {
+            const UpDgradArgs<TA> args{(const TA*)c.dy, (const float*)c.w, (TA*)c.dx, hl, wl, (const TA*)c.mask.y, c.mask.act,
+                                       (float)c.mask.alpha};
+            return up_dgrad_or_pair<Up1WgradBody<TA>, Up1DgradBody<TA>>(ctx, c, args, grid);
+        }
+        const int rc = uocr_held_launch_alone(ctx);
+        if (rc != UOCR_OK) return rc;
+        hipLaunchKernelGGL((upconv_dgrad_kernel<TA, K>), grid, dim3(256), 0, ctx->stream, (const TA*)c.dy,
+                           weff, (TA*)c.dx, hl, wl, (const TA*)c.mask.y, c.mask.act, (float)c.mask.alpha);
     });
     UOCR_LAUNCH_CHECK(ctx);
     return UOCR_OK;
     });
 }
 
+FinishDesc up_finish_desc(const ConvWgrad& c, const float* partial, int nblocks) {
+    const int ncols = up_ncols(c);
+    return finish_cols(partial, nblocks, ncols, ncols - c.d.cin, (float*)c.dw, (float*)c.db, c.use_bias, c.accumulate,
+                       (float)uocr_grad_unscale(c.dtype));
+}
 int up_wgrad_finish(uocr_ctx* ctx, const ConvWgrad& c, const float* partial, int nblocks) {
     const float unscale = (float)uocr_grad_unscale(c.dtype);
     const int ncols = up_ncols(c), ndw = ncols - c.d.cin;
-    const FinishDesc fd = finish_cols(partial, nblocks, ncols, ndw, (float*)c.dw, (float*)c.db, c.use_bias, c.accumulate, unscale);
+    const FinishDesc fd = up_finish_desc(c, partial, nblocks);
     return uocr_finish(ctx, fd, [&] {
         hipLaunchKernelGGL(colsum_finish_kernel, dim3((ncols + 7) / 8), dim3(256), 0, ctx->stream, partial, nblocks,
                            ncols, ndw, (float*)c.dw, (float*)c.db, c.use_bias, c.accumulate, unscale);
@@ -589,13 +653,19 @@
     int rc = UOCR_OK;
     float* partial = uocr_partial_buffer(ctx, (size_t)nblocks * up_ncols(c) * sizeof(float), &rc);
     if (rc != UOCR_OK) return rc;
+    const dim3 grid(strips, bands, n);
     UOCR_DISPATCH_TA(ctx, c.dtype, {
-        if (cin == 1)
-            hipLaunchKernelGGL((up1_wgrad_kernel<TA>), dim3(strips, bands, n), dim3(256), 0, ctx->stream,
-                               (const TA*)c.x, (const TA*)c.dy, partial, hl, wl, rows);
-        else
-            hipLaunchKernelGGL((upconv_wgrad_kernel<TA>), dim3(strips, bands, n), dim3(256), 0, ctx->stream,
-                               (const TA*)c.x, (const TA*)c.dy, partial, hl, wl, rows);
+        if (cin == 1) {
+            const UpWgradArgs<TA> args{(const TA*)c.x, (const TA*)c.dy, partial, hl, wl, rows};
+            if (ctx->opt_pair_bwd && uocr_finish_defer(ctx, up_finish_desc(c, partial, nblocks))) {
+                uocr_hold_wgrad(ctx, uocr_held_alone<Up1WgradBody<TA>>, HELD_UP_VECTOR, c, grid, args);
+                return UOCR_OK;
+            }
+            Up1WgradBody<TA>::launch(ctx->stream, grid, args);
+        } else {
+            hipLaunchKernelGGL((upconv_wgrad_kernel<TA>), grid, dim3(256), 0, ctx->stream, (const TA*)c.x, (const TA*)c.dy,
+                               partial, hl, wl, rows);
+        }
     });
     UOCR_LAUNCH_CHECK(ctx);
     return up_wgrad_finish(ctx, c, partial, nblocks);
@@ -625,14 +695,25 @@
 extern "C" int uocr_upconv2x_bwd_data(uocr_ctx* ctx, int dtype, const void* dy, const void* w, void* dx_low, int n,
                                       int hl, int wl, int cin, int cout, int kh, int kw, int ph, int pw,
                                       const void* x_act, int act, double act_alpha, const void* weff_in) {
-    UOCR_CHECK_CTX(ctx);
-    UOCR_REQUIRE(ctx, dy && w && dx_low);
-    UOCR_REQUIRE(ctx, act == UOCR_ACT_NONE || x_act != nullptr);
-    int rc = check_up(ctx, dtype, n, hl, wl, cin, cout, kh, kw, ph, pw);
+    UOCR_CHECK_CTX_KEEP(ctx);
+    const ActMask mask{act == UOCR_ACT_NONE ? nullptr : x_act, act, act_alpha};
+    const UpDgrad up{ConvDgrad{dtype, up_dims(n, hl, wl, cin, cout), dy, w, dx_low, mask}, weff_in};
+    const auto checked = [&]() -> int {
+        UOCR_REQUIRE(ctx, dy && w && dx_low);
+        UOCR_REQUIRE(ctx, act == UOCR_ACT_NONE || x_act != nullptr);
+        return check_up(ctx, dtype, n, hl, wl, cin, cout, kh, kw, ph, pw);
+    };
+    int rc = checked();
+    const auto into_vector = [&] {
+        const ConvRow<UpDgrad>* taker = uocr_conv_taker(ctx, UP_DGRAD_ROWS, up);
+        return taker && taker->run == up_dgrad_vector;
+    };
+    if (rc != UOCR_OK || !uocr_held_matches(ctx, dtype, dy, up.call.d) || !into_vector()) {
+        const int held_rc = uocr_held_launch_alone(ctx);
+        if (rc == UOCR_OK) rc = held_rc;
+    }
     if (rc != UOCR_OK) return rc;
-    const ActMask mask{act == UOCR_ACT_NONE ? nullptr : x_act, act, act_alpha};
-    const ConvDgrad call{dtype, up_dims(n, hl, wl, cin, cout), dy, w, dx_low, mask};
-    return uocr_conv_dispatch(ctx, 1, UP_DGRAD_ROWS, UpDgrad{call, weff_in});
+    return uocr_conv_dispatch(ctx, 1, UP_DGRAD_ROWS, up);
 }
 
 extern "C" int uocr_upconv2x_bwd_weight(uocr_ctx* ctx, int dtype, const void* x_low, const void* dy, void* dw, void* db,
diff --git a/univer-ocr_amd/csrc/ctx.hip b/univer-ocr_amd/csrc/ctx.hip
--- a/univer-ocr_amd/csrc/ctx.hip
+++ b/univer-ocr_amd/csrc/ctx.hip
@@ -114,6 +114,7 @@
     else if (!strcmp(key, "wgrad_bands") && value >= 0) ctx->opt_wgrad_bands = value;
     else if (!strcmp(key, "max_blocks") && value >= 0) ctx->opt_max_blocks = value;
     else if (!strcmp(key, "act_dispatch")) ctx->opt_act_dispatch = value != 0;
+    else if (!strcmp(key, "pair_bwd") && value >= 0 && value <= 2) ctx->opt_pair_bwd = value;
     else if (!strcmp(key, "h3")) {
 #ifndef UOCR_EXPERIMENTS
         if (value) UOCR_FAIL(ctx, UOCR_ERR_UNSUPPORTED, "option h3: this library was built without conv_h3 "
@@ -145,6 +146,10 @@
 
 int uocr_ctx_last_conv(uocr_ctx* ctx, int* entry, int* kernel) {
     return uocr_report_read(ctx, UOCR_REPORT_CONV, entry, kernel);
+}
+
+int uocr_ctx_pair_bwd_launches(uocr_ctx* ctx, long long* launches, int* w_blocks, int* d_blocks) {
+    return uocr_report_read(ctx, UOCR_REPORT_PAIR_BWD, launches, w_blocks, d_blocks);
 }
 
 void* uocr_ctx_get_stream(uocr_ctx* ctx) { return ctx ? (void*)ctx->stream : nullptr; }
diff --git a/univer-ocr_amd/csrc/gemm_mfma.hip b/univer-ocr_amd/csrc/gemm_mfma.hip
--- a/univer-ocr_amd/csrc/gemm_mfma.hip
+++ b/univer-ocr_amd/csrc/gemm_mfma.hip
@@ -30,22 +30,6 @@
     for (int q = 1; q < 4; ++q) r.v[q] = code == LD_KEEP ? v.v[q] : rest;
     return r;
 }
-
-struct FastDiv {
-    unsigned mul, shift;
-    int d;
-    FastDiv() = default;
-    explicit FastDiv(int divisor) : mul(0), shift(0), d(divisor) {
-        if (divisor > 1) {
-            int lg = 0;
-            while ((1ll << lg) < divisor) ++lg;
-            const int p = 31 + lg;
-            mul = (unsigned)(((1ull << p) + (unsigned)divisor - 1) / (unsigned)divisor);
-            shift = (unsigned)(p - 32);
-        }
-    }
-    __device__ __forceinline__ int div(int n) const { return d == 1 ? n : (int)(__umulhi((unsigned)n, mul) >> shift); }
-};
 
 struct Epilogue {
     float* c;
diff --git a/univer-ocr_amd/csrc/pair_bwd.h b/univer-ocr_amd/csrc/pair_bwd.h
--- /dev/null
+++ b/univer-ocr_amd/csrc/pair_bwd.h
@@ -0,0 +1,90 @@
+#pragma once
+#include "conv_dims.h"
+
+struct BlockAt {
+    unsigned bx, by, bz, gx, gy, tx, ty, tid;
+};
+__device__ __forceinline__ BlockAt block_at_launch() {
+    return BlockAt{blockIdx.x, blockIdx.y, blockIdx.z, gridDim.x, gridDim.y, threadIdx.x, threadIdx.y, threadIdx.x};
+}
+
+struct PairSide {
+    unsigned gx, gy, blocks;
+    FastDiv by_gx, by_gy;
+};
+struct PairPlan {
+    PairSide w, d;
+    int w_first;
+};
+inline PairSide pair_side(dim3 grid) {
+    return PairSide{grid.x, grid.y, grid.x * grid.y * grid.z, FastDiv((int)grid.x), FastDiv((int)grid.y)};
+}
+__device__ __forceinline__ BlockAt pair_block_at(const PairSide& s, unsigned id) {
+    const unsigned r = (unsigned)s.by_gx.div((int)id), z = (unsigned)s.by_gy.div((int)r);
+    return BlockAt{id - r * s.gx, r - z * s.gy, z, s.gx, s.gy, threadIdx.x, threadIdx.y, threadIdx.y * 64 + threadIdx.x};
+}
+
+template <class W, class D>
+__global__ __launch_bounds__(256) void pair_bwd_kernel(typename W::Args wa, typename D::Args da, PairPlan plan) {
+    constexpr size_t BYTES = W::LDS > D::LDS ? W::LDS : D::LDS;
+    __shared__ __attribute__((aligned(16))) unsigned char lds[BYTES > 0 ? BYTES : 16];
+    const unsigned first = plan.w_first ? plan.w.blocks : plan.d.blocks;
+    const bool low = blockIdx.x < first;
+    const unsigned id = low ? blockIdx.x : blockIdx.x - first;
+    if (low == (plan.w_first != 0)) W::run(pair_block_at(plan.w, id), lds, wa);
+    else D::run(pair_block_at(plan.d, id), lds, da);
+}
+
+static_assert(sizeof(ConvDims) == sizeof(uocr_held_wgrad::dims), "uocr_held_wgrad keeps a ConvDims");
+
+inline bool uocr_held_matches(const uocr_ctx* ctx, int dtype, const void* dy, const ConvDims& d) {
+    const uocr_held_wgrad& h = ctx->held;
+    return h.alone && h.dy == dy && UOCR_DTYPE_BASE(h.dtype) == UOCR_DTYPE_BASE(dtype) && !memcmp(h.dims, &d, sizeof(d));
+}
+inline int uocr_held_launch_alone(uocr_ctx* ctx) { return ctx->held.alone ? ctx->held.alone(ctx) : UOCR_OK; }
+
+template <class Args>
+void uocr_hold_wgrad(uocr_ctx* ctx, int (*alone)(uocr_ctx*), int kind, const ConvWgrad& c, dim3 grid, const Args& args) {
+    static_assert(sizeof(Args) <= sizeof(uocr_held_wgrad::args) && std::is_trivially_copyable_v<Args>);
+    uocr_held_wgrad& h = ctx->held;
+    h.alone = alone;
+    h.kind = kind;
+    h.dtype = c.dtype;
+    h.dy = c.dy;
+    memcpy(h.dims, &c.d, sizeof(c.d));
+    h.grid[0] = grid.x, h.grid[1] = grid.y, h.grid[2] = grid.z;
+    memcpy(h.args, &args, sizeof(args));
+}
+template <class Args>
+Args uocr_held_args(const uocr_held_wgrad& h) {
+    Args a;
+    memcpy(&a, h.args, sizeof(a));
+    return a;
+}
+inline dim3 uocr_held_grid(const uocr_held_wgrad& h) { return dim3(h.grid[0], h.grid[1], h.grid[2]); }
+
+template <class W>
+int uocr_held_alone(uocr_ctx* ctx) {
+    const uocr_held_wgrad h = ctx->held;
+    ctx->held.alone = nullptr;
+    W::launch(ctx->stream, uocr_held_grid(h), uocr_held_args<typename W::Args>(h));
+    UOCR_LAUNCH_CHECK(ctx);
+    return UOCR_OK;
+}
+
+inline unsigned long long pair_blocks(dim3 g) { return (unsigned long long)g.x * g.y * g.z; }
+inline bool uocr_pair_fits(const uocr_ctx* ctx, dim3 dgrid) {
+    return pair_blocks(uocr_held_grid(ctx->held)) + pair_blocks(dgrid) < (1ull << 31);
+}
+template <class W, class D>
+int uocr_launch_pair(uocr_ctx* ctx, const typename D::Args& da, dim3 dgrid) {
+    UOCR_REQUIRE(ctx, ctx->held.alone && uocr_pair_fits(ctx, dgrid));
+    const uocr_held_wgrad h = ctx->held;
+    ctx->held.alone = nullptr;
+    const PairPlan plan{pair_side(uocr_held_grid(h)), pair_side(dgrid), ctx->opt_pair_bwd != 2};
+    hipLaunchKernelGGL((pair_bwd_kernel<W, D>), dim3(plan.w.blocks + plan.d.blocks), dim3(64, 4), 0, ctx->stream,
+                       uocr_held_args<typename W::Args>(h), da, plan);
+    UOCR_LAUNCH_CHECK(ctx);
+    uocr_note(ctx, UOCR_REPORT_PAIR_BWD, ctx->report[UOCR_REPORT_PAIR_BWD][0] + 1, plan.w.blocks, plan.d.blocks);
+    return UOCR_OK;
+}
diff --git a/univer-ocr_amd/csrc/uocr_common.h b/univer-ocr_amd/csrc/uocr_common.h
--- a/univer-ocr_amd/csrc/uocr_common.h
+++ b/univer-ocr_amd/csrc/uocr_common.h
@@ -24,9 +24,21 @@
     UOCR_REPORT_PRED_TO_TEXT,
     UOCR_REPORT_PACK_LINES,
     UOCR_REPORT_PAGE_GEN,
+    UOCR_REPORT_PAIR_BWD,
     UOCR_REPORT_COUNT
 };
 constexpr int UOCR_REPORT_VALUES = 8;
+
+struct uocr_ctx;
+struct uocr_held_wgrad {
+    int (*alone)(uocr_ctx*) = nullptr;
+    int kind = 0;
+    int dtype = 0;
+    const void* dy = nullptr;
+    int dims[13] = {};
+    unsigned grid[3] = {};
+    alignas(8) unsigned char args[96] = {};
+};
 
 struct uocr_ctx {
     int device = 0;
@@ -60,6 +72,8 @@
     int opt_pair_g = 4;
     int opt_act_dispatch = 1;
     int opt_max_blocks = 0;
+    int opt_pair_bwd = 1;
+    uocr_held_wgrad held;
     long long report[UOCR_REPORT_COUNT][UOCR_REPORT_VALUES] = {};
     char err[512] = {};
 };
@@ -97,9 +111,17 @@
         if (!(cond)) UOCR_FAIL(ctx, UOCR_ERR_ARG, "bad argument: %s (%s:%d)", #cond, __FILE__, __LINE__); \
     } while (0)
 
-#define UOCR_CHECK_CTX(ctx) \
-    do {                    \
+#define UOCR_CHECK_CTX_KEEP(ctx) \
+    do {                         \
         if (!(ctx)) return UOCR_ERR_ARG; \
+    } while (0)
+#define UOCR_CHECK_CTX(ctx)                          \
+    do {                                             \
+        UOCR_CHECK_CTX_KEEP(ctx);                    \
+        if ((ctx)->held.alone) {                     \
+            const int held_rc_ = (ctx)->held.alone(ctx); \
+            if (held_rc_ != UOCR_OK) return held_rc_; \
+        }                                            \
     } while (0)
 
 template <typename... V>
@@ -436,6 +458,22 @@
             }
     }
 }
+
+struct FastDiv {
+    unsigned mul, shift;
+    int d;
+    FastDiv() = default;
+    explicit FastDiv(int divisor) : mul(0), shift(0), d(divisor) {
+        if (divisor > 1) {
+            int lg = 0;
+            while ((1ll << lg) < divisor) ++lg;
+            const int p = 31 + lg;
+            mul = (unsigned)(((1ull << p) + (unsigned)divisor - 1) / (unsigned)divisor);
+            shift = (unsigned)(p - 32);
+        }
+    }
+    __device__ __forceinline__ int div(int n) const { return d == 1 ? n : (int)(__umulhi((unsigned)n, mul) >> shift); }
+};
 
 struct TileWalk {
     int strip, trow, img;
diff --git a/univer-ocr_amd/hip/lib.py b/univer-ocr_amd/hip/lib.py
--- a/univer-ocr_amd/hip/lib.py
+++ b/univer-ocr_amd/hip/lib.py
@@ -53,6 +53,7 @@
     'uocr_ctx_last_gemm_group': [_ctx, C.POINTER(_i), C.POINTER(_i)],
     'uocr_ctx_last_pair': [_ctx] + [C.POINTER(_i)] * 8,
     'uocr_ctx_last_conv': [_ctx, C.POINTER(_i), C.POINTER(_i)],
+    'uocr_ctx_pair_bwd_launches': [_ctx, C.POINTER(C.c_longlong), C.POINTER(_i), C.POINTER(_i)],
     'uocr_malloc': [_ctx, _sz, C.POINTER(_vp)],
     'uocr_free': [_ctx, _vp],
     'uocr_memset_zero': [_ctx, _vp, _sz],
diff --git a/univer-ocr_amd/nn/gpu.py b/univer-ocr_amd/nn/gpu.py
--- a/univer-ocr_amd/nn/gpu.py
+++ b/univer-ocr_amd/nn/gpu.py
@@ -157,6 +157,9 @@
     def last_conv(self):
         return self._report('uocr_ctx_last_conv')
 
+    def pair_bwd_launches(self):
+        return self._report('uocr_ctx_pair_bwd_launches')
+
     def last_label(self):
         return self._report('uocr_ctx_last_label')
 
```
